# kepengxu/RealCamNet

Hardware: AMD Instinct MI355X
Metric: megapixels/sec RAW->sRGB at 4K (higher is better)
Workload: dtype bf16; 1 GPU; cfg3: 3840x2160 Bayer mosaic -> unshuffle+pad16 -> LiteISPNet_GFM_LSC_GMA -> sRGB 3840x2160, 8 frames/GPU, bf16 storage / fp32 accumulate; frames_per_gpu=8, global_frames=8, parallelism=frame-shard x1, collective=none

## Files before the change

### include/realcam_hip.h

```cpp
#ifndef REALCAM_HIP_H
#define REALCAM_HIP_H

#include <stddef.h>
#include <stdint.h>

#ifdef __cplusplus
extern "C" {
#endif

#define RC_ABI_VERSION 15

typedef enum rc_status {
    RC_OK = 0,
    RC_ERR_INVALID = -1,
    RC_ERR_HIP = -2,
    RC_ERR_UNSUPPORTED = -3
} rc_status;

typedef enum rc_dtype { RC_F32 = 0, RC_BF16 = 1, RC_U16 = 2 ,
                        RC_F16 = 3  } rc_dtype;

typedef enum rc_act { RC_ACT_NONE = 0, RC_ACT_RELU = 1, RC_ACT_LEAKY = 2 ,
                      RC_ACT_GELU = 3 ,
                      RC_ACT_RELU_POST = 4  } rc_act;

typedef enum rc_out_mode {
    RC_OUT_NHWC = 0,
    RC_OUT_PIXEL_SHUFFLE2 = 1,
    RC_OUT_NCHW = 2,
    RC_OUT_PIXEL_SHUFFLE2_NCHW = 3,
    RC_OUT_NHWC_DWT = 4
} rc_out_mode;

int rc_abi_version(void);
const char* rc_last_error(void);
const char* rc_build_info(void);
int rc_device_arch(char* buf, size_t buflen);

int rc_bayer_unshuffle(const void* d_mosaic, int in_dtype, void* d_packed, int out_dtype,
                       int batch, int h, int w, int hp, int wp, void* stream);

int rc_raw_ingest(const void* d_mosaic, int in_dtype, void* d_packed, void* d_cond, int out_dtype, int batch, int h, int w,
                  int hp, int wp, int cond_h, int cond_w, float black_level, float white_level, void* stream);

typedef enum rc_raw_storage {
    RC_RAW_F32 = 0, RC_RAW_BF16 = 1, RC_RAW_U16 = 2, RC_RAW_F16 = 3,
    RC_RAW_U8 = 4,
    RC_RAW_MIPI10 = 5,
    RC_RAW_MIPI12 = 6
} rc_raw_storage;

typedef enum rc_cfa { RC_CFA_RGGB = 0, RC_CFA_BGGR = 1, RC_CFA_GRBG = 2, RC_CFA_GBRG = 3 } rc_cfa;

typedef struct rc_raw_format {
    int storage;
    int cfa;
    int line_bytes;
    int width;
    float black[4];
    float white;
    int reserved[4];
} rc_raw_format;
size_t rc_raw_format_size(void);

int rc_raw_ingest_fmt(const void* d_src, const rc_raw_format* fmt, void* d_packed, void* d_cond, int out_dtype, int batch, int h, int w,
                      int hp, int wp, int cond_h, int cond_w, void* stream);

int rc_rgb_encode(const void* d_src, int src_dtype, void* d_dst, int out_bits, int batch, int H, int W, int h, int w, void* stream);

typedef enum rc_yuv_layout {
    RC_YUV_NV12 = 0,
    RC_YUV_P010 = 1,
    RC_YUV_I420 = 2
} rc_yuv_layout;
typedef enum rc_yuv_matrix { RC_MATRIX_BT601 = 0, RC_MATRIX_BT709 = 1, RC_MATRIX_BT2020 = 2  } rc_yuv_matrix;
typedef enum rc_yuv_range { RC_RANGE_LIMITED = 0, RC_RANGE_FULL = 1 } rc_yuv_range;
typedef enum rc_chroma_siting { RC_SITING_LEFT = 0 ,
                                RC_SITING_CENTER = 1  } rc_chroma_siting;

#define RC_YUV_KR_KB {{0.299, 0.114}, {0.2126, 0.0722}, {0.2627, 0.0593}}

typedef struct rc_out_format {
    int layout;
    int matrix;
    int range;
    int siting;
    int pitch;
    int rows;
    int chroma_offset[2];
    int reserved[4];
} rc_out_format;
size_t rc_out_format_size(void);

size_t rc_yuv_frame_bytes(const rc_out_format* fmt, int h, int w);

int rc_yuv_encode(const void* d_src, int src_dtype, const rc_out_format* fmt, void* d_dst, int batch, int H, int W, int h, int w, void* stream);

typedef enum rc_resize_filter {
    RC_FILTER_AREA = 0,
    RC_FILTER_BILINEAR = 1
} rc_resize_filter;
#define RC_RESIZE_MAX_TAPS 20
#define RC_RESIZE_MAX_RATIO 8

int rc_resize_taps(int filter, int n, int off, int m, int* first, float* weights, int* taps);

int rc_resize(const void* d_src, int src_dtype, void* d_dst, int dst_dtype, int batch, int H, int W, int h, int w, const int* d_first_y,
              const float* d_wy, int taps_y, const int* d_first_x, const float* d_wx, int taps_x, void* stream);

#define RC_LUT3D_MIN_SIZE 2
#define RC_LUT3D_MAX_SIZE 65

int rc_lut3d(const void* d_src, int src_dtype, void* d_dst, int dst_dtype, const float* d_lut, int n, int batch, int H, int W, int h, int w, void* stream);

typedef enum rc_warp_interp {
    RC_WARP_BILINEAR = 0,
    RC_WARP_BICUBIC = 1
} rc_warp_interp;
typedef enum rc_warp_border {
    RC_WARP_CLAMP = 0,
    RC_WARP_CONSTANT = 1
} rc_warp_border;
#define RC_WARP_MIN_CELL_LOG2 3
#define RC_WARP_MAX_CELL_LOG2 6
#define RC_WARP_MAX_DIM 8388608

int rc_warp(const void* d_src, int src_dtype, void* d_dst, int dst_dtype, const float* d_mesh, int mesh_batch, int cell_log2, int interp,
            int border, float fill_r, float fill_g, float fill_b, int batch, int H, int W, int h, int w, int oh, int ow, void* stream);

int rc_nchw_to_nhwc(const void* d_src, int src_dtype, void* d_dst, int dst_dtype,
                    int batch, int c, int h, int w, int hp, int wp, void* stream);
int rc_nhwc_to_nchw(const void* d_src, int src_dtype, void* d_dst, int dst_dtype,
                    int batch, int c, int H, int W, int h, int w, void* stream);

typedef struct rc_conv_desc {
    int32_t batch, height, width;
    int32_t cin, cout, ksize;
    int32_t dtype;
    const void* in0;
    const void* in1;
    const float* in_gate;
    void* in_store;
    const void* wpacked;
    const float* bias;
    const float* film_scale;
    const float* film_shift;
    int32_t act;
    float act_slope;
    const void* mul_plus1;
    const void* residual;
    void* out;
    int32_t out_mode;
    int32_t out_dtype;
    int32_t out_h, out_w;
    float* chan_sums;
    int32_t src_h, src_w;
    const float* out_scale;
    int32_t chan_sums_slots;
    int32_t cout_tile;
    int32_t algo;
} rc_conv_desc;

size_t rc_conv_packed_bytes(int cin, int cout, int ksize, int dtype, int out_mode);
int rc_conv_pack_weights(const float* w_oihw_host, int cin, int cout, int ksize, int dtype,
                         int out_mode, void* dst_host);
int rc_conv_packed_cout(int cin, int cout, int ksize, int dtype, int out_mode);
int rc_conv_pack_bias(const float* bias_host, int cin, int cout, int ksize, int dtype, int out_mode,
                      float* dst_host);
size_t rc_conv_packed_bytes_ct(int cin, int cout, int ksize, int dtype, int out_mode, int cout_tile);
int rc_conv_packed_cout_ct(int cin, int cout, int ksize, int dtype, int out_mode, int cout_tile);
int rc_conv_pack_weights_ct(const float* w_oihw_host, int cin, int cout, int ksize, int dtype, int out_mode, int cout_tile, void* dst_host);
int rc_conv_pack_bias_ct(const float* bias_host, int cin, int cout, int ksize, int dtype, int out_mode, int cout_tile, float* dst_host);
size_t rc_wino_packed_bytes(int cin, int cout, int dtype);
int rc_wino_pack_weights(const float* w_oihw_host, int cin, int cout, int dtype, void* dst_host);
int rc_conv_sum_tiles(int height, int width);
int rc_conv_sum_slots(const rc_conv_desc* d);
int rc_conv2d(const rc_conv_desc* desc, void* stream);
size_t rc_conv_desc_size(void);

int rc_tail_fold_weights(const float* w1_host, const float* b1_host, const float* w2_host, const float* b2_host, int c, int o,
                         float* wc_host, float* bc_host);
int rc_tail_ring_gather(const void* d_x, void* d_rows, void* d_cols, int dtype, int batch, int H, int W, int c, void* stream);
int rc_tail_ring_scatter(const void* d_rows_out, const void* d_cols_out, void* d_out, int dtype, int batch, int c_out, int H, int W,
                         int out_h, int out_w, void* stream);

typedef struct rc_conv_pair_desc {
    int32_t batch, height, width, channels;
    int32_t dtype;
    const void* in0;
    const void* in1;
    const float* in_gate;
    void* in_store;
    const void* w1; const float* b1;
    const float* film_scale;
    const float* film_shift;
    int32_t act1;
    float act1_slope;
    const void* w2; const float* b2;
    const void* residual;
    void* out;
    float* chan_sums;
} rc_conv_pair_desc;
int rc_conv_pair(const rc_conv_pair_desc* desc, void* stream);
int rc_conv_pair_sum_slots(int height, int width);
size_t rc_conv_pair_desc_size(void);

int rc_pointwise_chain48(const void* d_x, int cin0, const void* d_w0packed, const float* d_b0, const void* const* d_wpacked,
                         const float* const* d_bias, int n_mid, float slope, void* d_out, int dtype, long long pixels,
                         void* stream);

size_t rc_lsc_packed_bytes(int c, int n_mid, int has_head);
int rc_lsc_pack(const float* w0, const float* b0, int cin0, const float* const* wmid, const float* const* bmid, int n_mid,
                const float* whead, const float* bhead, int raw_c, int c, void* dst);
int rc_lsc_chain(const void* d_x, int cin0, const void* d_blob, int c, int n_mid, float slope, const void* d_raw, int raw_c,
                 void* d_out, int batch, int H, int W, void* stream);

int rc_ca_gate(float* d_sums, int batch, int n_tiles, int c, int cr, float inv_hw,
               const float* d_w0, const float* d_b0, const float* d_w1, const float* d_b1,
               float* d_gate, void* stream);

size_t rc_ca_gate_ahead_scratch_floats(int batch, int c);
int rc_ca_gate_ahead(float* d_sums, int batch, int n_tiles, int c, int cr, const void* d_t, int dtype, int H, int W,
                     const float* d_w2t, const float* d_b2, const float* d_w0, const float* d_b0, const float* d_w1, const float* d_b1,
                     float* d_scratch, float* d_gate, void* stream);

int rc_channel_sums_slots(int n_pix);
int rc_channel_sums(const void* d_x, int dtype, int batch, int n_pix, int c, float* d_sums, void* stream);

int rc_gate_residual(const void* d_r, const float* d_gate, const void* d_x, void* d_y, int dtype,
                     int batch, int n_pix, int c, void* stream);

int rc_film_apply(const void* d_x, const float* d_scale, const float* d_shift, void* d_y, int dtype, int batch, int n_pix, int c, void* stream);

int rc_sigmoid_gate_add(const void* d_a, const void* d_b, const void* d_identity, void* d_y, int dtype, long long n_elems,
                        void* stream);

int rc_subsample2(const void* d_src, void* d_dst, int dtype, int batch, int H, int W, int c, void* stream);
int rc_upsample_bilinear2(const void* d_src, void* d_dst, int dtype, int batch, int H, int W, int c, void* stream);
int rc_sft_apply(const void* d_x, const void* d_scale, const void* d_shift, const void* d_identity, void* d_y, int dtype,
                 long long n_elems, void* stream);
int rc_space_to_depth2(const void* d_src, void* d_dst, int dtype, int batch, int H, int W, int c, void* stream);
int rc_pixel_shuffle2(const void* d_src, void* d_dst, int dtype, int batch, int H, int W, int c_out, void* stream);
int rc_pixel_shuffle2_nchw(const void* d_src, void* d_dst, int dtype, int batch, int H, int W, int c_out, void* stream);
int rc_square(const void* d_x, void* d_y, int dtype, long long n_elems, void* stream);
int rc_gdn_apply(const void* d_x, const void* d_norm, const void* d_identity, void* d_y, int dtype, int inverse, long long n_elems,
                 void* stream);

int rc_entropy_bottleneck(const void* d_z, const float* d_params, const float* d_medians, void* d_z_hat, float* d_likelihood,
                          int dtype, long long n_pix, int channels, float likelihood_bound, void* stream);
int rc_gaussian_conditional(const void* d_y, const void* d_scale, const void* d_mu, void* d_y_hat, float* d_likelihood, int dtype,
                            long long n_elems, float scale_bound, float likelihood_bound, void* stream);
// ... 139 lines not shown
```

### realcamnet_amd/LiteISP.py

```python
from __future__ import annotations

from typing import Optional, Sequence

import torch
import torch.nn as nn

from . import networks as N
from . import ops
from .groupmix import GMA_Block, SUPPORTED_DTYPES
from ._lib import RC_OUT_NCHW, RC_OUT_PIXEL_SHUFFLE2
from .out_format import OutFormat
from .resize import Output


def color_block(in_filters, out_filters, normalization=False):
    layers = [N.Conv2d(in_filters, out_filters, 1, stride=1, padding=0),
              nn.AvgPool2d(3, stride=2, padding=1, count_include_pad=True),
              nn.LeakyReLU(0.2)]
    if normalization:
        layers.append(nn.InstanceNorm2d(out_filters, affine=True))
    return layers


def pad_to_multiple_of_16(x):
# ... 256 lines not shown
def _emit(y, bits, outs):
    if outs is None:
        return _encode(y, bits)
    res = []
    for o in outs:
        t = y if o.warp is None else ops.warp(y, o.warp)
        t = t if o.resize is None else ops.resize(t, o.resize)
        if o.look is not None:
            t = ops.lut3d(t, o.look)
        res.append(_encode(t, _out_bits(o.format)))
    return res


class _DwtUNet(nn.Module):

    output_dtype: Optional[torch.dtype] = None
    cond_from_raw = False

    def _build(self, ch_1, ch_2, ch_3, cond_c=None, lsc=False, nf=None, n_blocks=4):
        if cond_c is not None:
            self.classifier = Color_Condition_GFM(in_channels=4, out_c=cond_c)
        self.head = N.seq(N.conv(4, ch_1, mode='C'))
        if lsc:
            self.lsc = Lens_Shading_Correction(in_channels=2, out_c=ch_1, nf=ch_1)

        def gfm(i, c):
            if cond_c is not None:
                setattr(self, f"encoder_modulation{i}", N.seq(Res_GFM(in_nc=c, chan=c, cond_c=cond_c, out_nc=c, nf=nf[i - 1])))

        gfm(1, ch_1)
        self.down1 = N.seq(N.conv(ch_1, ch_1, mode='C'), N.RCAGroup(in_channels=ch_1, out_channels=ch_1, nb=n_blocks),
                           N.conv(ch_1, ch_1, mode='C'), N.DWTForward(ch_1))
        gfm(2, ch_1 * 4)
        self.down2 = N.seq(N.conv(ch_1 * 4, ch_1, mode='C'), N.RCAGroup(in_channels=ch_1, out_channels=ch_1, nb=n_blocks),
                           N.DWTForward(ch_1))
        gfm(3, ch_1 * 4)
        self.down3 = N.seq(N.conv(ch_1 * 4, ch_2, mode='C'), N.RCAGroup(in_channels=ch_2, out_channels=ch_2, nb=n_blocks),
                           N.DWTForward(ch_2))
        gfm(4, ch_2 * 4)
        self.middle = N.seq(N.conv(ch_2 * 4, ch_3, mode='C'), N.RCAGroup(in_channels=ch_3, out_channels=ch_3, nb=n_blocks),
                            N.RCAGroup(in_channels=ch_3, out_channels=ch_3, nb=n_blocks), N.conv(ch_3, ch_2 * 4, mode='C'))
        self.up3 = N.seq(N.DWTInverse(ch_2 * 4), N.RCAGroup(in_channels=ch_2, out_channels=ch_2, nb=n_blocks),
                         N.conv(ch_2, ch_1 * 4, mode='C'))
        self.up2 = N.seq(N.DWTInverse(ch_1 * 4), N.RCAGroup(in_channels=ch_1, out_channels=ch_1, nb=n_blocks),
                         N.conv(ch_1, ch_1 * 4, mode='C'))
        self.up1 = N.seq(N.DWTInverse(ch_1 * 4), N.RCAGroup(in_channels=ch_1, out_channels=ch_1, nb=n_blocks),
                         N.conv(ch_1, ch_1, mode='C'))
        self.tail = N.seq(N.conv(ch_1, ch_1 * 4, mode='C'), nn.PixelShuffle(upscale_factor=2), N.conv(ch_1, 3, mode='C'))

    def _act_dtype(self) -> torch.dtype:
        return self.head.weight.dtype

    def _refine_d1(self, d1):
        return d1

    def _check(self, raw):
        if self.training:
            raise RuntimeError("realcamnet_amd is an inference path: call .eval() first")
        if raw.dim() != 4 or raw.shape[1] != 4:
            raise ValueError(f"raw must be (B,4,H,W), got {tuple(raw.shape)}")
        if raw.shape[2] % 8 or raw.shape[3] % 8:
            raise ValueError(f"packed RAW H,W must be multiples of 8 (3 Haar levels), got {raw.shape[2]}x{raw.shape[3]}; "
                             "use forward_mosaic()/pad_to_multiple_of_16 for other sizes")

    def _front(self, a, cond, coord_nhwc):
        def head():
            if not hasattr(self, "lsc"):
                return self.head._nhwc(a)
            h = ops.lsc_chain(self.lsc, coord_nhwc, self.head, a)
            return h if h is not None else self.head._nhwc(a, mul_plus1=self.lsc._nhwc(coord_nhwc))

        if not hasattr(self, "classifier"):
            return head(), None
        cond = ops._req(cond, "cond")
        vec, h = ops.fork_join(lambda: self.classifier._vec(cond), head, [cond])
        return h, vec

    def _trunk(self, h, vec, crop_hw=None):
        mod = (lambda i, t: getattr(self, f"encoder_modulation{i}")._nhwc((t, vec))[0]) if vec is not None else (lambda i, t: t)
        h = mod(1, h)
        d1 = self._refine_d1(self.down1._nhwc(h))
        d2 = self.down2._nhwc(mod(2, d1))
        d3 = self.down3._nhwc(mod(3, d2))
        m = self.middle._nhwc(mod(4, d3), residual=d3)
        u3 = self.up3._nhwc(m, residual=d2)
        u2 = self.up2._nhwc(u3, residual=d1)
        u1 = self.up1._nhwc(u2, residual=h)
        if ops.tail_fold_ok(u1, self.tail[0], self.tail[2]):
            return ops.tail_fold(u1, self.tail[0], self.tail[2], crop_hw=crop_hw, out_dtype=self.output_dtype)
        t = self.tail[0]._nhwc(u1, out_mode=RC_OUT_PIXEL_SHUFFLE2)
        return self.tail[2]._nhwc(t, out_mode=RC_OUT_NCHW, crop_hw=crop_hw, out_dtype=self.output_dtype)

    def forward(self, x: Sequence[torch.Tensor]):
        raw = x if isinstance(x, torch.Tensor) else x[0]
        self._check(raw)
        dt = self._act_dtype()
        coord_nhwc = None
        if hasattr(self, "lsc"):
            coord = x[2]
            if coord.shape[0] != raw.shape[0] or coord.shape[1] != 2 or coord.shape[2:] != raw.shape[2:]:
                raise ValueError(f"coord must be (B,2,H,W) matching raw, got {tuple(coord.shape)}")
            coord_nhwc = ops.to_nhwc(coord, dtype=dt)
        cond = (raw if self.cond_from_raw else x[1]) if hasattr(self, "classifier") else None
        h, vec = self._front(ops.to_nhwc(raw, dtype=dt), cond, coord_nhwc)
        return self._trunk(h, vec)

    def forward_mosaic(self, mosaic, cond=None, coord=None, pad_to: int = 16, black_level: float = 0.0, white_level: float = 1.0,
                       cond_hw=(256, 256), raw_format=None, out_format=None, outputs=None):
        if self.training:
            raise RuntimeError("realcamnet_amd is an inference path: call .eval() first")
        bits = _out_bits(out_format)
        dt = self._act_dtype()
        mh, mw = _mosaic_hw(mosaic, raw_format)
        outs = _plan_outputs(outputs, out_format, (mh, mw))
        a, cond = _ingest(self, mosaic, cond, dt, pad_to, black_level, white_level, cond_hw, raw_format)
        b, hp, wp, _ = a.shape
        co = None
        if hasattr(self, "lsc"):
            if coord is None or coord.shape[-2:] != (mh // 2, mw // 2):
                raise ValueError("coord must be at packed resolution (h, w)")
            co = ops.to_nhwc(coord, dtype=dt, pad_hw=(hp, wp))
        if hasattr(self, "classifier") and self.cond_from_raw:
            cond = ops.to_nchw(a)
        h, vec = self._front(a, cond, co)
        return _emit(self._trunk(h, vec, crop_hw=(mh, mw)), bits, outs)


class LiteISPNet(_DwtUNet):

    def __init__(self):
        super().__init__()
        self._build(64, 128, 128)


class LiteISPNet_GFM_LSC(_DwtUNet):

    def __init__(self):
        super().__init__()
        self._build(48, 128, 128, cond_c=32, lsc=True, nf=(48, 48, 48, 128))


class LiteISPNet_LSC(_DwtUNet):

    def __init__(self):
        super().__init__()
        self._build(48, 128, 128, lsc=True)


class LiteISPNet_GFM(_DwtUNet):

    def __init__(self):
        super().__init__()
        self._build(64, 128, 128, cond_c=64, nf=(64, 64, 64, 128))


class LiteISPNet_GFMresize(_DwtUNet):
    cond_from_raw = True

    def __init__(self):
        super().__init__()
        self._build(64, 128, 128, cond_c=32, nf=(128, 256, 256, 512))


class _StridedUNet(nn.Module):

    output_dtype: Optional[torch.dtype] = None

    cond_from_raw = False
    coord_in_intro = False
    skips = True
# ... 270 lines not shown
```

### realcamnet_amd/_lib.py

```python
from __future__ import annotations

import ctypes as C
import os
import re
from pathlib import Path

PKG = Path(__file__).resolve().parent
LIB_PATH = Path(os.environ["RC_HIP_LIB"]) if os.environ.get("RC_HIP_LIB") else PKG / "librealcam_hip.so"
HEADER = PKG.parent / "include" / "realcam_hip.h"

RC_F32, RC_BF16, RC_U16, RC_F16 = 0, 1, 2, 3
RC_ACT_NONE, RC_ACT_RELU, RC_ACT_LEAKY, RC_ACT_GELU, RC_ACT_RELU_POST = 0, 1, 2, 3, 4
RC_OUT_NHWC, RC_OUT_PIXEL_SHUFFLE2, RC_OUT_NCHW, RC_OUT_PIXEL_SHUFFLE2_NCHW, RC_OUT_NHWC_DWT = 0, 1, 2, 3, 4
ABI_VERSION = 15
RC_RAW_F32, RC_RAW_BF16, RC_RAW_U16, RC_RAW_F16, RC_RAW_U8, RC_RAW_MIPI10, RC_RAW_MIPI12 = 0, 1, 2, 3, 4, 5, 6
RC_CFA_RGGB, RC_CFA_BGGR, RC_CFA_GRBG, RC_CFA_GBRG = 0, 1, 2, 3
RC_YUV_NV12, RC_YUV_P010, RC_YUV_I420 = 0, 1, 2
RC_MATRIX_BT601, RC_MATRIX_BT709, RC_MATRIX_BT2020 = 0, 1, 2
RC_RANGE_LIMITED, RC_RANGE_FULL = 0, 1
RC_SITING_LEFT, RC_SITING_CENTER = 0, 1
RC_FILTER_AREA, RC_FILTER_BILINEAR = 0, 1
RC_RESIZE_MAX_TAPS, RC_RESIZE_MAX_RATIO = 20, 8
RC_LUT3D_MIN_SIZE, RC_LUT3D_MAX_SIZE = 2, 65
RC_WARP_BILINEAR, RC_WARP_BICUBIC = 0, 1
RC_WARP_CLAMP, RC_WARP_CONSTANT = 0, 1
RC_WARP_MIN_CELL_LOG2, RC_WARP_MAX_CELL_LOG2, RC_WARP_MAX_DIM = 3, 6, 1 << 23


class ConvDesc(C.Structure):
    _fields_ = [
        ("batch", C.c_int32), ("height", C.c_int32), ("width", C.c_int32),
        ("cin", C.c_int32), ("cout", C.c_int32), ("ksize", C.c_int32),
        ("dtype", C.c_int32),
        ("in0", C.c_void_p), ("in1", C.c_void_p), ("in_gate", C.c_void_p), ("in_store", C.c_void_p),
        ("wpacked", C.c_void_p), ("bias", C.c_void_p),
        ("film_scale", C.c_void_p), ("film_shift", C.c_void_p),
        ("act", C.c_int32), ("act_slope", C.c_float),
        ("mul_plus1", C.c_void_p), ("residual", C.c_void_p),
        ("out", C.c_void_p), ("out_mode", C.c_int32), ("out_dtype", C.c_int32),
        ("out_h", C.c_int32), ("out_w", C.c_int32),
        ("chan_sums", C.c_void_p),
        ("src_h", C.c_int32), ("src_w", C.c_int32),
        ("out_scale", C.c_void_p),
        ("chan_sums_slots", C.c_int32), ("cout_tile", C.c_int32),
        ("algo", C.c_int32),
    ]


class ConvPairDesc(C.Structure):
    _fields_ = [
        ("batch", C.c_int32), ("height", C.c_int32), ("width", C.c_int32), ("channels", C.c_int32),
        ("dtype", C.c_int32),
        ("in0", C.c_void_p), ("in1", C.c_void_p), ("in_gate", C.c_void_p), ("in_store", C.c_void_p),
        ("w1", C.c_void_p), ("b1", C.c_void_p),
        ("film_scale", C.c_void_p), ("film_shift", C.c_void_p),
        ("act1", C.c_int32), ("act1_slope", C.c_float),
        ("w2", C.c_void_p), ("b2", C.c_void_p),
        ("residual", C.c_void_p), ("out", C.c_void_p), ("chan_sums", C.c_void_p),
    ]


class RawFormatDesc(C.Structure):
    _fields_ = [
        ("storage", C.c_int32), ("cfa", C.c_int32), ("line_bytes", C.c_int32), ("width", C.c_int32),
        ("black", C.c_float * 4), ("white", C.c_float), ("reserved", C.c_int32 * 4),
    ]


class OutFormatDesc(C.Structure):
    _fields_ = [
        ("layout", C.c_int32), ("matrix", C.c_int32), ("range", C.c_int32), ("siting", C.c_int32),
        ("pitch", C.c_int32), ("rows", C.c_int32), ("chroma_offset", C.c_int32 * 2), ("reserved", C.c_int32 * 4),
    ]


def declared_symbols() -> list[str]:
    text = HEADER.read_text()
    text = re.sub(r"/\*.*?\*/", "", text, flags=re.S)
    return sorted(set(re.findall(r"\b(rc_[a-z0-9_]+)\s*\(", text)))


_P, _I, _F, _SZ = C.c_void_p, C.c_int, C.c_float, C.c_size_t
_SIGS = {
    "rc_abi_version": (C.c_int, []),
    "rc_last_error": (C.c_char_p, []),
    "rc_build_info": (C.c_char_p, []),
    "rc_device_arch": (C.c_int, [C.c_char_p, _SZ]),
    "rc_bayer_unshuffle": (C.c_int, [_P, _I, _P, _I, _I, _I, _I, _I, _I, _P]),
    "rc_raw_ingest": (C.c_int, [_P, _I, _P, _P, _I, _I, _I, _I, _I, _I, _I, _I, _F, _F, _P]),
    "rc_raw_format_size": (_SZ, []),
    "rc_raw_ingest_fmt": (C.c_int, [_P, C.POINTER(RawFormatDesc), _P, _P, _I, _I, _I, _I, _I, _I, _I, _I, _P]),
    "rc_rgb_encode": (C.c_int, [_P, _I, _P, _I, _I, _I, _I, _I, _I, _P]),
    "rc_out_format_size": (_SZ, []),
    "rc_yuv_frame_bytes": (_SZ, [C.POINTER(OutFormatDesc), _I, _I]),
    "rc_yuv_encode": (C.c_int, [_P, _I, C.POINTER(OutFormatDesc), _P, _I, _I, _I, _I, _I, _P]),
    "rc_resize_taps": (C.c_int, [_I, _I, _I, _I, _P, _P, C.POINTER(C.c_int)]),
    "rc_resize": (C.c_int, [_P, _I, _P, _I, _I, _I, _I, _I, _I, _P, _P, _I, _P, _P, _I, _P]),
    "rc_lut3d": (C.c_int, [_P, _I, _P, _I, _P, _I, _I, _I, _I, _I, _I, _P]),
    "rc_warp": (C.c_int, [_P, _I, _P, _I, _P, _I, _I, _I, _I, _F, _F, _F, _I, _I, _I, _I, _I, _I, _I, _P]),
    "rc_nchw_to_nhwc": (C.c_int, [_P, _I, _P, _I, _I, _I, _I, _I, _I, _I, _P]),
    "rc_nhwc_to_nchw": (C.c_int, [_P, _I, _P, _I, _I, _I, _I, _I, _I, _I, _P]),
    "rc_conv_packed_bytes": (_SZ, [_I, _I, _I, _I, _I]),
    "rc_conv_pack_weights": (C.c_int, [_P, _I, _I, _I, _I, _I, _P]),
    "rc_conv_packed_cout": (C.c_int, [_I, _I, _I, _I, _I]),
    "rc_conv_pack_bias": (C.c_int, [_P, _I, _I, _I, _I, _I, _P]),
    "rc_conv_packed_bytes_ct": (_SZ, [_I, _I, _I, _I, _I, _I]),
    "rc_wino_packed_bytes": (_SZ, [_I, _I, _I]),
    "rc_wino_pack_weights": (C.c_int, [_P, _I, _I, _I, _P]),
    "rc_conv_packed_cout_ct": (C.c_int, [_I, _I, _I, _I, _I, _I]),
    "rc_conv_pack_weights_ct": (C.c_int, [_P, _I, _I, _I, _I, _I, _I, _P]),
    "rc_conv_pack_bias_ct": (C.c_int, [_P, _I, _I, _I, _I, _I, _I, _P]),
    "rc_conv_sum_tiles": (C.c_int, [_I, _I]),
    "rc_conv_sum_slots": (C.c_int, [_P]),
    "rc_conv2d": (C.c_int, [C.POINTER(ConvDesc), _P]),
    "rc_conv_desc_size": (_SZ, []),
    "rc_tail_fold_weights": (C.c_int, [_P, _P, _P, _P, _I, _I, _P, _P]),
    "rc_tail_ring_gather": (C.c_int, [_P, _P, _P, _I, _I, _I, _I, _I, _P]),
    "rc_tail_ring_scatter": (C.c_int, [_P, _P, _P, _I, _I, _I, _I, _I, _I, _I, _P]),
    "rc_debug_stream_create_masked": (C.c_int, [_I, C.POINTER(C.c_void_p)]),
    "rc_debug_hbm_probe": (C.c_int, [_P, _P, C.c_size_t, _I, _I, _I, _I, _I, C.POINTER(C.c_double)]),
    "rc_debug_mfma_peak": (C.c_int, [_I, _I, C.POINTER(C.c_double), C.POINTER(C.c_double)]),
    "rc_debug_mfma_peak32": (C.c_int, [_I, _I, C.POINTER(C.c_double), C.POINTER(C.c_double)]),
    "rc_debug_poison_lds": (C.c_int, [C.c_uint, _P]),
    "rc_pointwise_chain48": (C.c_int, [_P, _I, _P, _P, C.POINTER(C.c_void_p), C.POINTER(C.c_void_p), _I, _F, _P, _I, C.c_longlong, _P]),
    "rc_lsc_packed_bytes": (C.c_size_t, [_I, _I, _I]),
    "rc_lsc_pack": (C.c_int, [_P, _P, _I, C.POINTER(C.c_void_p), C.POINTER(C.c_void_p), _I, _P, _P, _I, _I, _P]),
    "rc_lsc_chain": (C.c_int, [_P, _I, _P, _I, _I, _F, _P, _I, _P, _I, _I, _I, _P]),
    "rc_film_apply": (C.c_int, [_P, _P, _P, _P, _I, _I, _I, _I, _P]),
    "rc_sigmoid_gate_add": (C.c_int, [_P, _P, _P, _P, _I, C.c_longlong, _P]),
    "rc_subsample2": (C.c_int, [_P, _P, _I, _I, _I, _I, _I, _P]),
    "rc_entropy_bottleneck": (C.c_int, [_P, _P, _P, _P, _P, _I, C.c_longlong, _I, C.c_float, _P]),
    "rc_gaussian_conditional": (C.c_int, [_P, _P, _P, _P, _P, _I, C.c_longlong, C.c_float, C.c_float, _P]),
    "rc_tanh_half_add": (C.c_int, [_P, _P, _P, _I, C.c_longlong, _P]),
    "rc_upsample_bilinear2": (C.c_int, [_P, _P, _I, _I, _I, _I, _I, _P]),
    "rc_sft_apply": (C.c_int, [_P, _P, _P, _P, _P, _I, C.c_longlong, _P]),
    "rc_space_to_depth2": (C.c_int, [_P, _P, _I, _I, _I, _I, _I, _P]),
    "rc_pixel_shuffle2": (C.c_int, [_P, _P, _I, _I, _I, _I, _I, _P]),
    "rc_pixel_shuffle2_nchw": (C.c_int, [_P, _P, _I, _I, _I, _I, _I, _P]),
    "rc_square": (C.c_int, [_P, _P, _I, C.c_longlong, _P]),
    "rc_gdn_apply": (C.c_int, [_P, _P, _P, _P, _I, _I, C.c_longlong, _P]),
    "rc_channel_copy": (C.c_int, [_P, _I, _I, _P, _I, _I, _I, C.c_longlong, _I, _P]),
    "rc_channel_concat": (C.c_int, [C.POINTER(C.c_void_p), C.POINTER(C.c_int), _I, _P, C.c_longlong, _I, _P]),
    "rc_window_attention": (C.c_int, [_P, _P, _P, _I, _I, _I, _I, _I, _I, _I, _I, _P]),
    "rc_window_attention_planar8": (C.c_int, [_P, _P, _P, _I, _I, _I, _I, _I, _I, _I, _I, _P]),
    "rc_window_attention_planar8_ok": (C.c_int, [_I, _I, _I, _I, _I, _I]),
    "rc_conv_pair": (C.c_int, [C.POINTER(ConvPairDesc), _P]),
    "rc_conv_pair_sum_slots": (C.c_int, [_I, _I]),
    "rc_conv_pair_desc_size": (_SZ, []),
    "rc_ca_gate": (C.c_int, [_P, _I, _I, _I, _I, _F, _P, _P, _P, _P, _P, _P]),
    "rc_ca_gate_ahead_scratch_floats": (_SZ, [_I, _I]),
    "rc_ca_gate_ahead": (C.c_int, [_P, _I, _I, _I, _I, _P, _I, _I, _I, _P, _P, _P, _P, _P, _P, _P, _P, _P]),
    "rc_gate_residual": (C.c_int, [_P, _P, _P, _P, _I, _I, _I, _I, _P]),
    "rc_channel_sums_slots": (C.c_int, [_I]),
    "rc_channel_sums": (C.c_int, [_P, _I, _I, _I, _I, _P, _P]),
    "rc_dwt_forward": (C.c_int, [_P, _P, _P, _I, _I, _I, _I, _I, _I, _P]),
    "rc_dwt_inverse": (C.c_int, [_P, _P, _P, _I, _I, _I, _I, _I, _I, _P]),
    "rc_color_block": (C.c_int, [_P, _I, _P, _I, _I, _I, _I, _I, _P, _P, _P, _P, _P, _P, _P]),
    "rc_instance_stats": (C.c_int, [_P, _P, _P, _I, _I, _I, _F, _P]),
    "rc_instance_norm": (C.c_int, [_P, _P, _P, _P, _P, _P, _I, _I, _I, _P]),
    "rc_color_head": (C.c_int, [_P, _P, _I, _I, _I, _I, _P, _P, _P]),
    "rc_gfm_vector": (C.c_int, [_P, _I, _I, _I, _I, _P, _P, _P, _P, _P, _P]),
    "rc_dwconv2d": (C.c_int, [_P, _I, _I, _P, _I, _I, _I, _I, _I, _I, _I, _I, _P, _I, _P, _I, _I, _I, _I, _I, _P, _P]),
    "rc_layernorm": (C.c_int, [_P, _P, _I, C.c_longlong, _I, _P, _P, _F, _P]),
    "rc_gma_pointwise": (C.c_int, [_P, _P, _P, _I, _I, _I, _I, _P, _P, _I, C.c_longlong, _I, _P, _P, _P, _P, _P, _P, _P]),
    "rc_chain_packed_bytes": (_SZ, [_I, _I]),
    "rc_chain_packed_rows": (C.c_int, [_I]),
    "rc_chain_pack_weights": (C.c_int, [_P, _I, _I, _P]),
    "rc_chain_pack_bias": (C.c_int, [_P, _I, _P]),
    "rc_gma_ln_qkv": (C.c_int, [_P, _P, C.c_longlong, _P, _P, _P, _P, _F, _P]),
    "rc_gma_tail": (C.c_int, [_P, _P, _P, _P, _P, _P, _I, _I, _P, _P, _P, _P, _F, _P, _P, _P, _P, _P, _P, _P, _I, _P, _P]),
    "rc_gma_aggregate": (C.c_int, [_P, _P, _P, _I, _I, _I, _P, _P, _P, _P, _P, _P, _P, _P, _P, _P, _P, _P]),
    "rc_chain_pack_weights_natural": (C.c_int, [_P, _I, _I, _P]),
    "rc_gma_toeplitz_bytes": (_SZ, []),
    "rc_gma_toeplitz_pack": (C.c_int, [_P, _P, _P, _P, _P]),
    "rc_dw_toeplitz_pack": (C.c_int, [_P, _I, _I, _P]),
    "rc_gma_in_cpe": (C.c_int, [_P, _P, _P, _P, _P, _P, _I, _I, _I, _P]),
    "rc_gma_qkv_aggregate": (C.c_int, [_P, _P, _P, _P, _P, _F, _P, _P, _I, _I, _I, _P, _P, _P, _P, _P, _P, _P, _P, _P]),
    "rc_cat_linear": (C.c_int, [_P, _P, _P, _P, _P, C.c_longlong, _I, _P, _P, _P]),
    "rc_gdn_chain": (C.c_int, [_P, _P, _P, C.c_longlong, _I, _P, _P, _I, _P]),
    "rc_ln_linear": (C.c_int, [_P, _P, C.c_longlong, _I, _I, _P, _P, _P, _P, _F, _P]),
    "rc_ln_linear_planar8": (C.c_int, [_P, _P, C.c_longlong, _I, _I, _P, _P, _P, _P, _F, _P]),
    "rc_ln_mlp": (C.c_int, [_P, _P, C.c_longlong, _I, _P, _P, _P, _P, _P, _P, _F, _P]),
    "rc_gma_kv_mfma_blocks": (C.c_int, [_I]),
    "rc_gma_kv_mfma_scratch_bytes": (C.c_size_t, [_I, _I]),
    "rc_gma_kv_mfma": (C.c_int, [_P, _I, _I, _F, _P, _P, _P, _P]),
    "rc_gma_crpe": (C.c_int, [_P, _P, _I, _I, _I, _P, _P, _P, _P, _P, _P]),
    "rc_gma_kv_blocks": (C.c_int, [_I]),
    "rc_gma_kv_scratch_bytes": (_SZ, [_I, _I, _I, _I]),
# ... 74 lines not shown
```

### realcamnet_amd/csrc/conv.hip

```cpp
#include <mutex>
#include <vector>

#include "conv32_kernel.hpp"

namespace rc {

struct ConvPlan {
    int ck = 0, nt = 0, unit = 0, upt = 0, nu = 0, steps = 0;
    int n_chunks = 0, n_ct = 0, cout_packed = 0;
    int m32 = 0;
};

static int g_persist_on = 1;
extern int g_dw3_seg16;
extern int g_dec_lds;
extern int g_pw_grid_cap;
static int g_pss = 0;
static int g_poison = 0;
static int g_thin = 2;
static int g_auto = 1;
static int g_sums_compact = 1;
static int g_conv32 = 0;

static bool make_plan(int cin, int cout, int ksize, int dtype, int out_mode, ConvPlan* p, int cout_tile = 0) {
    if (cin < 1 || cout < 1 || (ksize != 1 && ksize != 3 && ksize != 2 && ksize != 5)) return false;
    if (dtype != RC_F32 && dtype != RC_BF16 && dtype != RC_F16) return false;
    const bool h16 = dtype != RC_F32;
    if (ksize == 5 && (cout > 16 || out_mode == RC_OUT_PIXEL_SHUFFLE2 || (h16 ? (cin % 48 != 0 && cin % 32 != 0) : cin % 16 != 0))) return false;
    if (out_mode == RC_OUT_PIXEL_SHUFFLE2_NCHW && cout % 4 != 0) return false;
    if (ksize == 2 && (dtype != RC_BF16 || cin % 16 != 0 || out_mode != RC_OUT_NHWC || (cin % 48 == 0 && cin % 64 != 0))) return false;
    p->unit = dtype == RC_F32 ? 4 : 8;
    if (ksize == 5) p->ck = h16 ? (cin % 48 == 0 ? 48 : 32) : 16;
    else if (h16) {
        if (cin <= 8) p->ck = 8;
        else if (ksize == 1 && cin % 80 == 0 && cin % 64 != 0) p->ck = 80;
        else if (ksize >= 2 && cin % 64 == 0 && cin > 64) p->ck = 32;
        else if (cin % 64 == 0) p->ck = 64;
        else if (cin % 48 == 0) p->ck = 48;
        else if (ksize == 3 && cin == 32) p->ck = 32;
        else if (ksize == 3 && cin % 32 == 0 && cin > 64) p->ck = 32;
        else p->ck = 16;
    } else {
        p->ck = cin <= 4 ? 4 : 16;
    }
    if (out_mode == RC_OUT_PIXEL_SHUFFLE2) {
        if (cout % 4 != 0) return false;
        const int cps = cout / 4;
        if (cps % 64 == 0 && !(cps % 48 == 0 && h16 && cin == 48)) p->nt = 4;
        else if (cps % 48 == 0) p->nt = 3;
        else if (cps % 64 == 0) p->nt = 4;
        else if (cps % 16 == 0) p->nt = 1;
        else return false;
    } else if (cout % 48 == 0 && h16 && cin == 48) p->nt = 3;
    else if (h16 && ksize == 3 && cin == 32 && cout == 32) p->nt = 2;
    else if (ksize == 1 && cout % 80 == 0) p->nt = 5;
    else if (cout % 64 == 0) p->nt = 4;
    else if (cout % 48 == 0) p->nt = 3;
    else if (h16 && ksize == 3 && p->ck == 32 && cout % 32 == 0) p->nt = 2;
    else p->nt = 1;
    if (cout_tile != 0) {
        if (cout_tile < 16 || cout_tile > 80 || cout_tile % 16 != 0 || ksize == 5 || ksize == 2 || out_mode == RC_OUT_PIXEL_SHUFFLE2 || out_mode == RC_OUT_PIXEL_SHUFFLE2_NCHW) return false;
        p->nt = cout_tile / 16;
    }
    p->m32 = 0;
    if (cout_tile == 0 && dtype == RC_BF16 && ksize == 3 && g_conv32 != 0 && cout <= kPersistMaxCout && out_mode != RC_OUT_NCHW && out_mode != RC_OUT_PIXEL_SHUFFLE2_NCHW) {
        const int cw = out_mode == RC_OUT_PIXEL_SHUFFLE2 ? cout / 4 : cout;
        const bool all = g_conv32 != 4;
        if (all && p->ck == 32 && cin % 32 == 0 && (out_mode == RC_OUT_PIXEL_SHUFFLE2 ? cw % 32 == 0 : cw % 64 == 0)) { p->m32 = 1; p->nt = 2; p->ck = (g_conv32 == 1 && out_mode == RC_OUT_NHWC) ? 16 : 32; }
        else if (cin == 48 && (out_mode == RC_OUT_PIXEL_SHUFFLE2 ? (all && cw % 48 == 0) : cw % 96 == 0)) { p->m32 = 1; p->nt = 3; p->ck = 48; }
    }
    if (p->m32) {
        p->upt = p->ck / p->unit;
        p->nu = 9 * p->upt;
        p->steps = 9 * (p->ck / 16);
        p->n_chunks = cin / p->ck;
        p->n_ct = cout / (32 * p->nt);
        p->cout_packed = cout;
        return true;
    }
    p->upt = p->ck / p->unit;
    p->nu = ksize * ksize * p->upt;
    p->steps = unit_map_steps(p->upt, ksize * ksize);
    p->n_chunks = ceil_div(cin, p->ck);
    p->n_ct = ceil_div(cout, 16 * p->nt);
    p->cout_packed = p->n_ct * 16 * p->nt;
    return true;
}

static int packed_to_cout(const ConvPlan& p, int cout, int out_mode, int j) {
    if (p.m32) return c32_packed_to_cout(p.nt, out_mode, j);
    if (out_mode == RC_OUT_PIXEL_SHUFFLE2) {
        const int tile = 16 * p.nt;
        const int ct = j / tile, within = j % tile;
        const int cb = ct >> 2, sub = ct & 3;
        return 4 * (cb * tile + within) + sub;
    }
    return j < cout ? j : -1;
}

int wino_conv(const rc_conv_desc* d, hipStream_t stream);
int wino_sum_slots(int H, int W, int cout);
void wino_set_nnt(int v);
int wino_get_nnt();
bool wino_supported(const rc_conv_desc* d, std::string* why);

static int g_dbg_flags = 0;
static int g_pair_impl = 0;
static long long* g_dbg_ptr = nullptr;
static std::mutex g_prof_mu;
static bool g_prof_on = false;
struct ProfRec { hipEvent_t e0, e1; double flops, bytes; int cin, cout, ksize; };
static std::vector<ProfRec> g_prof;

long long* conv_dbg_ptr() { return g_dbg_ptr; }
int conv_pair_impl() { return g_pair_impl; }

void conv_prof_begin(double flops, hipStream_t stream, void** token, double bytes, int cin, int cout, int ksize) {
    *token = nullptr;
    { std::lock_guard<std::mutex> lk(g_prof_mu); if (!g_prof_on) return; }
    ProfRec* rec = new ProfRec{};
    rec->flops = flops; rec->bytes = bytes; rec->cin = cin; rec->cout = cout; rec->ksize = ksize;
    if (hipEventCreate(&rec->e0) != hipSuccess || hipEventCreate(&rec->e1) != hipSuccess) { delete rec; return; }
    (void)hipEventRecord(rec->e0, stream);
    *token = rec;
}
void conv_prof_end(void* token, hipStream_t stream) {
    if (!token) return;
    ProfRec* rec = static_cast<ProfRec*>(token);
    (void)hipEventRecord(rec->e1, stream);
    std::lock_guard<std::mutex> lk(g_prof_mu);
    g_prof.push_back(*rec);
    delete rec;
}

}

using namespace rc;

extern "C" {

size_t rc_conv_packed_bytes_ct(int cin, int cout, int ksize, int dtype, int out_mode, int cout_tile) {
    ConvPlan p;
    if (!make_plan(cin, cout, ksize, dtype, out_mode, &p, cout_tile)) { set_error("rc_conv_packed_bytes: bad shape"); return 0; }
    return (size_t)p.n_ct * p.n_chunks * p.steps * p.nt * 1024;
}
size_t rc_conv_packed_bytes(int cin, int cout, int ksize, int dtype, int out_mode) { return rc_conv_packed_bytes_ct(cin, cout, ksize, dtype, out_mode, 0); }

int rc_conv_packed_cout_ct(int cin, int cout, int ksize, int dtype, int out_mode, int cout_tile) {
    ConvPlan p;
    if (!make_plan(cin, cout, ksize, dtype, out_mode, &p, cout_tile)) return fail(RC_ERR_INVALID, "rc_conv_packed_cout: bad shape");
    return p.cout_packed;
}
int rc_conv_packed_cout(int cin, int cout, int ksize, int dtype, int out_mode) { return rc_conv_packed_cout_ct(cin, cout, ksize, dtype, out_mode, 0); }

int rc_conv_pack_weights(const float* w, int cin, int cout, int ksize, int dtype, int out_mode, void* dst) {
    return rc_conv_pack_weights_ct(w, cin, cout, ksize, dtype, out_mode, 0, dst);
}
int rc_conv_pack_bias(const float* bias, int cin, int cout, int ksize, int dtype, int out_mode, float* dst) {
    return rc_conv_pack_bias_ct(bias, cin, cout, ksize, dtype, out_mode, 0, dst);
}

int rc_conv_pack_weights_ct(const float* w, int cin, int cout, int ksize, int dtype, int out_mode, int cout_tile, void* dst) {
    ConvPlan p;
    RC_REQUIRE(w && dst, "rc_conv_pack_weights: null pointer");
    RC_REQUIRE(make_plan(cin, cout, ksize, dtype, out_mode, &p, cout_tile), "rc_conv_pack_weights: bad shape");
    const int kk = ksize * ksize;
    char* out = static_cast<char*>(dst);
    if (p.m32) {
        const int spt = p.ck / 16;
        for (int ct = 0; ct < p.n_ct; ++ct)
            for (int chunk = 0; chunk < p.n_chunks; ++chunk)
                for (int s = 0; s < p.steps; ++s)
                    for (int t = 0; t < p.nt; ++t)
                        for (int lane = 0; lane < 64; ++lane) {
                            const int m = lane & 31, kg = lane >> 5;
                            const int c = 16 * ((m >> 2) & 1) + (m & 3) + 4 * (m >> 3);
                            const int co = packed_to_cout(p, cout, out_mode, ct * 32 * p.nt + 32 * t + c);
                            const int tap = s / spt, ci0 = chunk * p.ck + (2 * (s % spt) + kg) * 8;
                            for (int e = 0; e < 8; ++e) {
                                *reinterpret_cast<uint16_t*>(out) = host_f32_to_bf16(w[((size_t)co * cin + ci0 + e) * kk + tap]);
                                out += 2;
                            }
                        }
        return RC_OK;
    }
    for (int ct = 0; ct < p.n_ct; ++ct)
        for (int chunk = 0; chunk < p.n_chunks; ++chunk)
            for (int s = 0; s < p.steps; ++s)
                for (int nt = 0; nt < p.nt; ++nt)
                    for (int lane = 0; lane < 64; ++lane) {
                        const int m = lane & 15, qk = lane >> 4;
                        int tap = 0, cu = 0;
                        const bool live = unit_map(p.upt, kk, s, qk, tap, cu);
                        const int j = ct * 16 * p.nt + (m >> 2) * (4 * p.nt) + nt * 4 + (m & 3);
                        const int co = packed_to_cout(p, cout, out_mode, j);
                        for (int e = 0; e < p.unit; ++e) {
                            float val = 0.f;
                            if (live && co >= 0 && co < cout) {
                                const int ci = chunk * p.ck + cu * p.unit + e;
                                if (ci < cin) val = w[((size_t)co * cin + ci) * kk + tap];
                            }
                            if (dtype == RC_F32) {
                                *reinterpret_cast<float*>(out) = val; out += 4;
                            } else {
                                *reinterpret_cast<uint16_t*>(out) = host_f32_to_h16(val, dtype); out += 2;
                            }
                        }
                    }
    return RC_OK;
}

int rc_conv_pack_bias_ct(const float* bias, int cin, int cout, int ksize, int dtype, int out_mode, int cout_tile, float* dst) {
    ConvPlan p;
    RC_REQUIRE(dst, "rc_conv_pack_bias: null pointer");
    RC_REQUIRE(make_plan(cin, cout, ksize, dtype, out_mode, &p, cout_tile), "rc_conv_pack_bias: bad shape");
    for (int j = 0; j < p.cout_packed; ++j) {
        const int co = packed_to_cout(p, cout, out_mode, j);
        dst[j] = (bias && co >= 0 && co < cout) ? bias[co] : 0.f;
    }
    return RC_OK;
}

size_t rc_conv_desc_size(void) { return sizeof(rc_conv_desc); }

int rc_tail_fold_weights(const float* w1, const float* b1, const float* w2, const float* b2, int c, int o, float* wc, float* bc) {
    RC_REQUIRE(w1 && w2 && wc && bc && c >= 1 && o >= 1, "rc_tail_fold_weights: bad arguments");
    std::vector<double> acc((size_t)4 * o * c * 25, 0.0), bacc((size_t)4 * o, 0.0);
    for (int oo = 0; oo < o; ++oo)
        for (int i = 0; i < 2; ++i)
            for (int j = 0; j < 2; ++j) {
                const int row = oo * 4 + 2 * i + j;
                bacc[row] = b2 ? (double)b2[oo] : 0.0;
                for (int dy = 0; dy < 3; ++dy)
                    for (int dx = 0; dx < 3; ++dx) {
                        const int a = i + dy - 1, b = j + dx - 1;
                        const int fy = a < 0 ? -1 : a >> 1, ii = a & 1, fx = b < 0 ? -1 : b >> 1, jj = b & 1;
                        for (int cc = 0; cc < c; ++cc) {
                            const int m = 4 * cc + 2 * ii + jj;
                            const double v2 = w2[(((size_t)oo * c + cc) * 3 + dy) * 3 + dx];
                            if (b1) bacc[row] += v2 * (double)b1[m];
                            for (int k = 0; k < c; ++k)
                                for (int ey = 0; ey < 3; ++ey)
                                    for (int ex = 0; ex < 3; ++ex)
                                        acc[(((size_t)row * c + k) * 5 + (fy + ey + 1)) * 5 + (fx + ex + 1)] += v2 * (double)w1[(((size_t)m * c + k) * 3 + ey) * 3 + ex];
                        }
                    }
            }
    for (size_t n = 0; n < acc.size(); ++n) wc[n] = (float)acc[n];
    for (size_t n = 0; n < bacc.size(); ++n) bc[n] = (float)bacc[n];
    return RC_OK;
}

int rc_conv_sum_tiles(int height, int width) { return 4 * ceil_div(height, kTH) * ceil_div(width, kTW); }

int rc_debug_set(const char* key, int value) {
    RC_REQUIRE(key != nullptr, "rc_debug_set: null key");
    if (std::string(key) == "persist") { g_persist_on = value < 0 ? 0 : (value > 3 ? 3 : value); return RC_OK; }
    if (std::string(key) == "conv_flags") { g_dbg_flags = value; return RC_OK; }
    if (std::string(key) == "pair_impl") { g_pair_impl = value < 0 || value > 2 ? 0 : value; return RC_OK; }
    if (std::string(key) == "dec_lds") { g_dec_lds = value != 0; return RC_OK; }
    if (std::string(key) == "dw3_seg16") { g_dw3_seg16 = value != 0; return RC_OK; }
    if (std::string(key) == "pss") { g_pss = value != 0; return RC_OK; }
    if (std::string(key) == "sums_compact") { g_sums_compact = value != 0; return RC_OK; }
    if (std::string(key) == "persist_auto") { g_auto = value < 0 ? 0 : (value > 2 ? 2 : value); return RC_OK; }
    if (std::string(key) == "thin") { g_thin = value < 0 ? 0 : (value > 2 ? 2 : value); return RC_OK; }
    if (std::string(key) == "lds_poison") { g_poison = value != 0; return RC_OK; }
    if (std::string(key) == "conv32") { g_conv32 = value < 0 ? 0 : (value > 4 ? 4 : value); return RC_OK; }
    if (std::string(key) == "wino_nnt") { wino_set_nnt(value); return RC_OK; }
    if (std::string(key) == "pw_grid_cap") { g_pw_grid_cap = value <= 0 || value > (1 << 22) ? (1 << 22) : value; return RC_OK; }
    return fail(RC_ERR_INVALID, std::string("rc_debug_set: unknown key ") + key);
}

int rc_debug_get(const char* key) {
    if (key == nullptr) return -1;
    if (std::string(key) == "persist") return g_persist_on;
    if (std::string(key) == "conv32") return g_conv32;
    if (std::string(key) == "conv_flags") return g_dbg_flags;
    if (std::string(key) == "pss") return g_pss;
    if (std::string(key) == "sums_compact") return g_sums_compact;
    if (std::string(key) == "persist_auto") return g_auto;
    if (std::string(key) == "thin") return g_thin;
    if (std::string(key) == "lds_poison") return g_poison;
    if (std::string(key) == "wino_nnt") return wino_get_nnt();
    if (std::string(key) == "pw_grid_cap") return g_pw_grid_cap;
    return -1;
}

int rc_debug_set_ptr(const char* key, void* p) {
    RC_REQUIRE(key != nullptr, "rc_debug_set_ptr: null key");
    if (std::string(key) == "conv_phase_timing") { g_dbg_ptr = static_cast<long long*>(p); return RC_OK; }
    return fail(RC_ERR_INVALID, std::string("rc_debug_set_ptr: unknown key ") + key);
}

int rc_prof_enable(int on) {
    std::lock_guard<std::mutex> lk(g_prof_mu);
    for (auto& r : g_prof) { (void)hipEventDestroy(r.e0); (void)hipEventDestroy(r.e1); }
    g_prof.clear();
    g_prof_on = on != 0;
    return RC_OK;
}

int rc_prof_collect(int64_t* n_launches, double* total_ms, double* total_flops) {
    std::lock_guard<std::mutex> lk(g_prof_mu);
    double ms = 0.0, fl = 0.0;
    for (auto& r : g_prof) {
        RC_HIP_CHECK(hipEventSynchronize(r.e1));
        float t = 0.f;
        RC_HIP_CHECK(hipEventElapsedTime(&t, r.e0, r.e1));
        ms += t; fl += r.flops;
    }
    if (n_launches) *n_launches = (int64_t)g_prof.size();
    if (total_ms) *total_ms = ms;
    if (total_flops) *total_flops = fl;
    return RC_OK;
}

int rc_prof_collect_rows(rc_prof_row* rows, int max_rows, int* n_rows) {
    RC_REQUIRE(rows != nullptr && n_rows != nullptr && max_rows >= 1, "rc_prof_collect_rows: bad arguments");
    std::lock_guard<std::mutex> lk(g_prof_mu);
    int n = 0;
    for (auto& r : g_prof) {
        RC_HIP_CHECK(hipEventSynchronize(r.e1));
        float t = 0.f;
        RC_HIP_CHECK(hipEventElapsedTime(&t, r.e0, r.e1));
        int i = 0;
        while (i < n && !(rows[i].cin == r.cin && rows[i].cout == r.cout && rows[i].ksize == r.ksize)) ++i;
        if (i == n) {
            if (n == max_rows) continue;
            rows[n] = rc_prof_row{r.cin, r.cout, r.ksize, 0, 0.0, 0.0, 0.0};
            ++n;
        }
        rows[i].launches += 1; rows[i].ms += t; rows[i].flops += r.flops; rows[i].bytes += r.bytes;
    }
    *n_rows = n;
    return RC_OK;
}

static int conv_build_args(const rc_conv_desc* d, ConvPlan& p, ConvArgs& a, size_t& es_out) {
    RC_REQUIRE(d != nullptr, "rc_conv2d: null desc");
    const bool dwt = d->out_mode == RC_OUT_NHWC_DWT;
    RC_REQUIRE(make_plan(d->cin, d->cout, d->ksize, d->dtype, dwt ? (int)RC_OUT_NHWC : d->out_mode, &p, d->cout_tile), "rc_conv2d: unsupported cin/cout/ksize/dtype/cout_tile");
    RC_REQUIRE(d->batch >= 1 && d->height >= 1 && d->width >= 1, "rc_conv2d: empty tensor");
    RC_REQUIRE(d->batch <= 65535, "rc_conv2d: batch > 65535");
    RC_REQUIRE(d->in0 && d->wpacked && d->out, "rc_conv2d: null in0/wpacked/out");
    RC_REQUIRE(d->out_mode >= RC_OUT_NHWC && d->out_mode <= RC_OUT_NHWC_DWT, "rc_conv2d: bad out_mode");
    if (dwt) {
        RC_REQUIRE(d->height % 2 == 0 && d->width % 2 == 0, "rc_conv2d: RC_OUT_NHWC_DWT needs even height and width");
        RC_REQUIRE(d->out_dtype == d->dtype && reinterpret_cast<uintptr_t>(d->out) % 16 == 0, "rc_conv2d: RC_OUT_NHWC_DWT: out_dtype must equal dtype, out 16-byte aligned");
        RC_REQUIRE(!d->mul_plus1 && !d->film_scale && !d->out_scale && !d->chan_sums && !d->in_gate && !d->in1 && !d->in_store && !d->src_h && !d->src_w && !d->cout_tile,
                   "rc_conv2d: RC_OUT_NHWC_DWT excludes mul_plus1 / film / out_scale / chan_sums / gated input / src_h / cout_tile");
        if (d->dtype == RC_F32 || d->ksize != 3 || p.m32 || !(d->act == RC_ACT_NONE || ((d->act == RC_ACT_RELU || d->act == RC_ACT_LEAKY) && !d->residual)))
            return fail(RC_ERR_UNSUPPORTED, "rc_conv2d: RC_OUT_NHWC_DWT is a bf16 / fp16 3x3 form with act NONE / RELU / LEAKY, or act NONE + residual");
    }
    RC_REQUIRE(d->act >= RC_ACT_NONE && d->act <= RC_ACT_RELU_POST, "rc_conv2d: bad act");
    RC_REQUIRE(d->act != RC_ACT_RELU_POST || (d->residual != nullptr && d->mul_plus1 == nullptr && d->film_scale == nullptr && d->chan_sums == nullptr),
               "rc_conv2d: RC_ACT_RELU_POST is relu(conv + residual): needs residual, excludes film / mul_plus1 / chan_sums");
    if (d->in_gate) RC_REQUIRE(d->in1 != nullptr, "rc_conv2d: in_gate needs in1 (the skip tensor)");
    RC_REQUIRE((d->film_scale == nullptr) == (d->film_shift == nullptr), "rc_conv2d: film_scale/film_shift must come together");
    const bool full_tiles = d->cout == p.cout_packed;
    if (d->mul_plus1 || d->residual)
        RC_REQUIRE((full_tiles || d->cout % 4 == 0) && (d->out_mode == RC_OUT_NHWC || (dwt && !d->mul_plus1)), "rc_conv2d: mul_plus1/residual need cout % 4 == 0 and RC_OUT_NHWC (residual: or RC_OUT_NHWC_DWT)");
    if (d->chan_sums) RC_REQUIRE(d->out_mode == RC_OUT_NHWC, "rc_conv2d: chan_sums needs RC_OUT_NHWC");
    if (d->out_scale) {
        RC_REQUIRE(d->out_mode == RC_OUT_NHWC && !p.m32, "rc_conv2d: out_scale needs RC_OUT_NHWC and a layer outside the 32x32x16 forms");
        RC_REQUIRE(reinterpret_cast<uintptr_t>(d->out_scale) % 4 == 0, "rc_conv2d: out_scale must be 4-byte aligned");
    }
    const size_t es = dtype_size(d->dtype);
    const int planar16 = d->dtype == RC_F16 ? RC_F16 : RC_BF16;
    if (dwt) {
    } else if (d->out_mode == RC_OUT_NHWC) {
        RC_REQUIRE(d->out_dtype == d->dtype, "rc_conv2d: out_dtype must equal dtype for RC_OUT_NHWC");
        RC_REQUIRE(!full_tiles || (d->cout * es) % 8 == 0, "rc_conv2d: cout*elem_size must be a multiple of 8 bytes for RC_OUT_NHWC");
        RC_REQUIRE(reinterpret_cast<uintptr_t>(d->out) % 16 == 0, "rc_conv2d: out must be 16-byte aligned");
        if (p.nt == 4 && d->dtype != RC_F32) RC_REQUIRE(d->cout % 8 == 0, "rc_conv2d: cout % 8");
    } else if (d->out_mode == RC_OUT_PIXEL_SHUFFLE2) {
        RC_REQUIRE(d->out_dtype == d->dtype, "rc_conv2d: out_dtype must equal dtype for RC_OUT_PIXEL_SHUFFLE2");
        RC_REQUIRE(full_tiles && ((d->cout / 4) * es) % 8 == 0, "rc_conv2d: pixel-shuffle store needs (cout/4)*elem_size % 8 == 0");
        RC_REQUIRE(!d->film_scale, "rc_conv2d: film not supported with pixel-shuffle store");
        RC_REQUIRE(reinterpret_cast<uintptr_t>(d->out) % 16 == 0, "rc_conv2d: out must be 16-byte aligned");
    } else if (d->out_mode == RC_OUT_PIXEL_SHUFFLE2_NCHW) {
        RC_REQUIRE(d->out_h >= 1 && d->out_h <= 2 * d->height && d->out_w >= 1 && d->out_w <= 2 * d->width, "rc_conv2d: bad pixel-shuffle NCHW crop");
        RC_REQUIRE(d->out_dtype == RC_F32 || d->out_dtype == planar16, "rc_conv2d: bad out_dtype");
        RC_REQUIRE(!d->chan_sums, "rc_conv2d: chan_sums needs RC_OUT_NHWC");
        RC_REQUIRE((double)d->out_h * d->out_w * (d->cout / 4) * 4.0 < 2147483647.0, "rc_conv2d: one output image must be < 2 GiB");
    } else {
        RC_REQUIRE(d->out_h >= 1 && d->out_h <= d->height && d->out_w >= 1 && d->out_w <= d->width, "rc_conv2d: bad NCHW crop");
        RC_REQUIRE(d->out_dtype == RC_F32 || d->out_dtype == planar16, "rc_conv2d: bad out_dtype");
    }
    {
        const double lim = 2147483647.0;
        RC_REQUIRE((double)d->height * d->width * d->cin * es < lim, "rc_conv2d: one input image must be < 2 GiB");
        RC_REQUIRE((double)d->height * d->width * d->cout * 4.0 < lim, "rc_conv2d: one output image must be < 2 GiB");
    }
    const bool fold = d->src_h != 0 || d->src_w != 0;
    if (fold) {
        RC_REQUIRE(d->ksize == 2 && d->cin % 4 == 0 && (d->cin / 4) % p.ck == 0, "rc_conv2d: src_h/src_w need ksize 2 and cin / 4 a whole number of Cin chunks");
        RC_REQUIRE(d->src_h >= 1 && d->src_w >= 1 && d->height == (d->src_h + 1) / 2 && d->width == (d->src_w + 1) / 2,
                   "rc_conv2d: height/width must be ceil(src_h / 2), ceil(src_w / 2)");
        RC_REQUIRE(d->in_gate == nullptr && d->in1 == nullptr && d->in_store == nullptr, "rc_conv2d: src_h/src_w exclude the gated input");
        RC_REQUIRE(reinterpret_cast<uintptr_t>(d->in0) % 16 == 0, "rc_conv2d: src_h/src_w need a 16-byte aligned in0 (the scalar staging path does not gather)");
        RC_REQUIRE((double)d->src_h * d->src_w * (d->cin / 4) * es < 2147483647.0, "rc_conv2d: one input image must be < 2 GiB");
    }
    if (d->residual) RC_REQUIRE(reinterpret_cast<uintptr_t>(d->residual) % 16 == 0, "rc_conv2d: residual must be 16-byte aligned");
    if (d->mul_plus1) RC_REQUIRE(reinterpret_cast<uintptr_t>(d->mul_plus1) % 16 == 0, "rc_conv2d: mul_plus1 must be 16-byte aligned");

    a = ConvArgs{};
    a.batch = d->batch; a.H = d->height; a.W = d->width; a.cin = d->cin; a.cout = d->cout;
    a.n_chunks = p.n_chunks; a.n_ct = p.n_ct;
    a.tiles_x = ceil_div(d->width, kTW); a.tiles_y = ceil_div(d->height, kTH);
    if (p.m32) RC_REQUIRE(!d->film_scale || (reinterpret_cast<uintptr_t>(d->film_scale) % 16 == 0 && reinterpret_cast<uintptr_t>(d->film_shift) % 16 == 0),
                          "rc_conv2d: film vectors must be 16-byte aligned");
    auto aligned16 = [](const void* q) { return q == nullptr || reinterpret_cast<uintptr_t>(q) % 16 == 0; };
    a.cin_vec_ok = (d->cin % p.unit == 0) && aligned16(d->in0) && aligned16(d->in1) && aligned16(d->in_store) &&
                   (d->in_gate == nullptr || reinterpret_cast<uintptr_t>(d->in_gate) % 4 == 0);
    a.cin_chunk_ok = d->cin % p.ck == 0;
    a.fold2 = fold ? 1 : 0; a.src_H = d->src_h; a.src_W = d->src_w; a.cfold = d->cin / 4;
    a.in0 = d->in0; a.in1 = d->in1; a.in_gate = d->in_gate; a.in_store = d->in_store;
    a.wpacked = d->wpacked; a.bias = d->bias;
    a.film_scale = d->film_scale; a.film_shift = d->film_shift;
    a.act = d->act; a.act_slope = d->act_slope;
    a.mul_plus1 = d->mul_plus1; a.residual = d->residual; a.out_scale = d->out_scale;
    a.out = d->out; a.out_mode = d->out_mode; a.out_dtype = d->out_dtype; a.out_h = d->out_h; a.out_w = d->out_w;
    a.chan_sums = d->chan_sums; a.cout_packed = p.cout_packed;
    a.sum_slots = d->chan_sums_slots > 0 ? d->chan_sums_slots : 4 * ceil_div(d->height, kTH) * ceil_div(d->width, kTW);
    a.sums_compact = 0; a.query = nullptr; a.sums_compact_ok = g_sums_compact;
    {
        int key = (d->act == RC_ACT_RELU ? 1 : 0) | (d->act == RC_ACT_LEAKY ? 2 : 0) | (d->film_scale ? 4 : 0) |
                  (d->mul_plus1 ? 8 : 0) | (d->residual ? 16 : 0) | (d->chan_sums ? 32 : 0) | (d->out_scale ? 64 : 0);
        bool fast = full_tiles && d->out_mode != RC_OUT_NCHW && d->out_mode != RC_OUT_PIXEL_SHUFFLE2_NCHW && d->act != RC_ACT_GELU && d->act != RC_ACT_RELU_POST;
        if (d->act == RC_ACT_LEAKY) fast = fast && d->act_slope >= 0.f && d->act_slope <= 1.f;
        if (d->film_scale)
            fast = fast && d->cout % 4 == 0 && reinterpret_cast<uintptr_t>(d->film_scale) % 16 == 0 && reinterpret_cast<uintptr_t>(d->film_shift) % 16 == 0;
        if (d->out_scale) fast = fast && d->cout % 4 == 0 && reinterpret_cast<uintptr_t>(d->out_scale) % 16 == 0;
        switch (key) { case 0: case 1: case 2: case 16: case 32: case 8: case 6: case 33: case 34: case 80: break; default: fast = false; }
        a.ep_key = fast ? key : -1;
        a.pss = g_pss && d->out_mode == RC_OUT_PIXEL_SHUFFLE2 && !p.m32 && p.n_chunks == 1 && p.n_ct == 4 && d->cout == 4 * 16 * p.nt &&
                d->dtype == RC_BF16 && d->in_gate == nullptr && fast && (key == 0 || key == 1 || key == 2);
    }
    {
        const int num_cus = device_cu_count();
        a.num_cus = num_cus;
        a.persist_ok = g_persist_on;
        a.auto_impl = g_auto;
        a.thin = g_thin;
        a.dbg = g_dbg_ptr;
        a.dbg_flags = g_dbg_flags;
        a.td = make_tile_decode(a.tiles_x, a.tiles_y, kBandRows);
        a.td_wsm = make_tile_decode(a.tiles_x, (a.H + kWsmTH - 1) / kWsmTH, kBandRows);
        a.div_n_ct = make_magic(a.n_ct);
    }
    es_out = es;
    return RC_OK;
// ... 44 lines not shown
```

### realcamnet_amd/csrc/conv_dispatch.hip

```cpp
#include "conv_kernel.hpp"
namespace rc {
int conv_bf16_k3_ck8(int nt, const ConvArgs& a, hipStream_t s);
int conv_bf16_k3_ck16(int nt, const ConvArgs& a, hipStream_t s);
int conv_bf16_k3_ck32(int nt, const ConvArgs& a, hipStream_t s);
int conv_bf16_k3_ck48(int nt, const ConvArgs& a, hipStream_t s);
int conv_bf16_k3_ck64(int nt, const ConvArgs& a, hipStream_t s);
int conv_bf16_k5_ck48(int nt, const ConvArgs& a, hipStream_t s);
int conv_bf16_k5_ck32(int nt, const ConvArgs& a, hipStream_t s);
int conv_f32_k5_ck16(int nt, const ConvArgs& a, hipStream_t s);
int conv_bf16_k2_ck16(int nt, const ConvArgs& a, hipStream_t s);
int conv_bf16_k2_ck32(int nt, const ConvArgs& a, hipStream_t s);
int conv_bf16_k2_ck64(int nt, const ConvArgs& a, hipStream_t s);
int conv_bf16_k1_ck8(int nt, const ConvArgs& a, hipStream_t s);
int conv_bf16_k1_ck16(int nt, const ConvArgs& a, hipStream_t s);
int conv_bf16_k1_ck48(int nt, const ConvArgs& a, hipStream_t s);
int conv_bf16_k1_ck64(int nt, const ConvArgs& a, hipStream_t s);
int conv_bf16_k1_ck80(int nt, const ConvArgs& a, hipStream_t s);
int conv_f32_k3_ck4(int nt, const ConvArgs& a, hipStream_t s);
int conv_f32_k3_ck16(int nt, const ConvArgs& a, hipStream_t s);
int conv_f32_k1_ck4(int nt, const ConvArgs& a, hipStream_t s);
int conv_f32_k1_ck16(int nt, const ConvArgs& a, hipStream_t s);
int conv_f16_k3_ck8(int nt, const ConvArgs& a, hipStream_t s);
int conv_f16_k3_ck16(int nt, const ConvArgs& a, hipStream_t s);
int conv_f16_k3_ck32(int nt, const ConvArgs& a, hipStream_t s);
int conv_f16_k3_ck48(int nt, const ConvArgs& a, hipStream_t s);
int conv_f16_k3_ck64(int nt, const ConvArgs& a, hipStream_t s);
int conv_f16_k5_ck48(int nt, const ConvArgs& a, hipStream_t s);
int conv_f16_k5_ck32(int nt, const ConvArgs& a, hipStream_t s);
int conv_f16_k1_ck8(int nt, const ConvArgs& a, hipStream_t s);
int conv_f16_k1_ck16(int nt, const ConvArgs& a, hipStream_t s);
int conv_f16_k1_ck48(int nt, const ConvArgs& a, hipStream_t s);
int conv_f16_k1_ck64(int nt, const ConvArgs& a, hipStream_t s);

int dispatch_conv(int dtype, int ksize, int ck, int nt, const ConvArgs& a, hipStream_t s) {
    if (dtype == RC_F16) {
        if (ksize == 3 && ck == 8) return conv_f16_k3_ck8(nt, a, s);
        if (ksize == 3 && ck == 16) return conv_f16_k3_ck16(nt, a, s);
        if (ksize == 3 && ck == 32) return conv_f16_k3_ck32(nt, a, s);
        if (ksize == 3 && ck == 48) return conv_f16_k3_ck48(nt, a, s);
        if (ksize == 3 && ck == 64) return conv_f16_k3_ck64(nt, a, s);
        if (ksize == 5 && ck == 48) return conv_f16_k5_ck48(nt, a, s);
        if (ksize == 5 && ck == 32) return conv_f16_k5_ck32(nt, a, s);
        if (ksize == 1 && ck == 8) return conv_f16_k1_ck8(nt, a, s);
        if (ksize == 1 && ck == 16) return conv_f16_k1_ck16(nt, a, s);
        if (ksize == 1 && ck == 48) return conv_f16_k1_ck48(nt, a, s);
        if (ksize == 1 && ck == 64) return conv_f16_k1_ck64(nt, a, s);
        return fail(RC_ERR_UNSUPPORTED, "conv: no fp16 kernel instantiation for this (ksize, chunk width)");
    }
    const bool bf16 = dtype == RC_BF16;
    if (bf16 && ksize == 3 && ck == 8) return conv_bf16_k3_ck8(nt, a, s);
    if (bf16 && ksize == 3 && ck == 16) return conv_bf16_k3_ck16(nt, a, s);
    if (bf16 && ksize == 3 && ck == 32) return conv_bf16_k3_ck32(nt, a, s);
    if (bf16 && ksize == 3 && ck == 48) return conv_bf16_k3_ck48(nt, a, s);
    if (bf16 && ksize == 3 && ck == 64) return conv_bf16_k3_ck64(nt, a, s);
    if (bf16 && ksize == 5 && ck == 48) return conv_bf16_k5_ck48(nt, a, s);
    if (bf16 && ksize == 5 && ck == 32) return conv_bf16_k5_ck32(nt, a, s);
    if (!bf16 && ksize == 5 && ck == 16) return conv_f32_k5_ck16(nt, a, s);
    if (bf16 && ksize == 2 && ck == 16) return conv_bf16_k2_ck16(nt, a, s);
    if (bf16 && ksize == 2 && ck == 32) return conv_bf16_k2_ck32(nt, a, s);
    if (bf16 && ksize == 2 && ck == 64) return conv_bf16_k2_ck64(nt, a, s);
    if (bf16 && ksize == 1 && ck == 8) return conv_bf16_k1_ck8(nt, a, s);
    if (bf16 && ksize == 1 && ck == 16) return conv_bf16_k1_ck16(nt, a, s);
    if (bf16 && ksize == 1 && ck == 48) return conv_bf16_k1_ck48(nt, a, s);
    if (bf16 && ksize == 1 && ck == 64) return conv_bf16_k1_ck64(nt, a, s);
    if (bf16 && ksize == 1 && ck == 80) return conv_bf16_k1_ck80(nt, a, s);
    if (!bf16 && ksize == 3 && ck == 4) return conv_f32_k3_ck4(nt, a, s);
    if (!bf16 && ksize == 3 && ck == 16) return conv_f32_k3_ck16(nt, a, s);
    if (!bf16 && ksize == 1 && ck == 4) return conv_f32_k1_ck4(nt, a, s);
    if (!bf16 && ksize == 1 && ck == 16) return conv_f32_k1_ck16(nt, a, s);
    return fail(RC_ERR_UNSUPPORTED, "conv: no kernel instantiation for this (dtype, ksize, chunk width)");
}
}
```

### realcamnet_amd/csrc/conv_kernel.hpp

```cpp
#pragma once
#include "common.hpp"

namespace rc {

struct MagicDiv { unsigned m, sh; };
inline MagicDiv make_magic(int d) {
    if (d <= 1) return MagicDiv{0u, 0u};
    int L = 0;
    while ((2 << L) <= d) ++L;
    const unsigned long long m = ((1ull << (31 + L)) + (unsigned long long)d - 1) / (unsigned long long)d;
    return MagicDiv{(unsigned)m, (unsigned)(L - 1)};
}
__device__ __forceinline__ int magic_div(int n, const MagicDiv& d) {
    return d.m ? (int)(__umulhi((unsigned)n, d.m) >> d.sh) : n;
}
struct TileDecode { MagicDiv sp_total, band, last_rows; };
inline TileDecode make_tile_decode(int tiles_x, int tiles_y, int band_rows) {
    return TileDecode{make_magic(tiles_x * tiles_y), make_magic(band_rows * tiles_x), make_magic(tiles_y % band_rows ? tiles_y % band_rows : 1)};
}

struct ConvArgs {
    int batch, H, W, cin, cout;
    int n_chunks, n_ct, tiles_x, tiles_y;
    int cin_vec_ok;
    int cin_chunk_ok;
    const void* in0; const void* in1; const float* in_gate; void* in_store;
    const void* wpacked; const float* bias;
    const float* film_scale; const float* film_shift;
    int act; float act_slope;
    const void* mul_plus1; const void* residual;
    const float* out_scale;
    void* out; int out_mode; int out_dtype; int out_h, out_w;
    float* chan_sums; int cout_packed;
    int sum_slots;
    int sums_compact_ok;
    int sums_compact;
    int* query;
    int num_cus; int persist_ok;
    int ep_key;
    TileDecode td, td_wsm;
    MagicDiv div_n_ct;
    int w_resident;
    int pss;
    int auto_impl;
    int thin;
    int fold2, src_H, src_W, cfold;
    long long* dbg;
    int dbg_flags;
};

constexpr int kTH = 8, kTW = 32, kThreads = 256;

constexpr int pix_stride_bytes(int ck_bytes) {
    int s = (ck_bytes + 15) / 16 * 16;
    while (s % 64 != 32) s += 16;
    return s;
}

__host__ __device__ constexpr int unit_map_steps(int upt, int taps) {
    return upt == 6 ? taps + (taps + 1) / 2 : (taps * upt + 3) / 4;
}
__host__ __device__ constexpr bool unit_map(int upt, int taps, int s, int q, int& tap, int& cu) {
    if (upt == 6) {
        if (s < taps) { tap = s; cu = q; return true; }
        tap = 2 * (s - taps) + (q >> 1); cu = 4 + (q & 1);
        return tap < taps;
    }
    const int u = 4 * s + q;
    tap = u / upt; cu = u % upt;
    return u < taps * upt;
}

template <typename T, int CK_, int NT_, int KS_, int TH_ = kTH>
struct ConvCfg {
    using elem = T;
    static constexpr int CK = CK_, NT = NT_, KS = KS_, TH = TH_;
    static constexpr int UNIT = 16 / (int)sizeof(T);
    static_assert(CK % UNIT == 0, "CK must be a whole number of 16-byte units");
    static constexpr int UPT = CK / UNIT;
    static constexpr int TAPS = KS * KS;
    static constexpr int STEPS = unit_map_steps(UPT, TAPS);
    static constexpr int HALO = KS / 2;
    static constexpr int THH = TH + 2 * HALO, TWH = kTW + 2 * HALO;
    static constexpr int SPIX = pix_stride_bytes(CK * (int)sizeof(T));
    static constexpr int IN_BYTES = THH * TWH * SPIX;
    static constexpr int G_RAW = (80 * 1024 - IN_BYTES) / (NT * 1024);
    static constexpr int G_CAP = G_RAW < 1 ? 1 : (G_RAW > STEPS ? STEPS : G_RAW);
    static constexpr int NSUB = (STEPS + G_CAP - 1) / G_CAP;
    static constexpr int G = (STEPS + NSUB - 1) / NSUB;
    static constexpr int W_BYTES = G * NT * 1024;
    static constexpr int COUT_TILE = 16 * NT;
    static constexpr int LDS_BYTES = IN_BYTES + W_BYTES;
    static constexpr size_t CHUNK_W_BYTES = (size_t)STEPS * NT * 1024;
};

constexpr int kOOB = (int)0x80000000;

typedef unsigned int u32x4_t __attribute__((ext_vector_type(4)));
typedef unsigned int u32x2_t __attribute__((ext_vector_type(2)));

__device__ __forceinline__ __amdgpu_buffer_rsrc_t make_rsrc(const void* p, unsigned bytes) {
    return __builtin_amdgcn_make_buffer_rsrc(const_cast<void*>(p), 0, (int)bytes, 0x00020000);
}
__device__ __forceinline__ uint4 buf_load16(__amdgpu_buffer_rsrc_t r, int voff, int soff) {
    const u32x4_t v = __builtin_amdgcn_raw_buffer_load_b128(r, voff, soff, 0);
    return make_uint4(v.x, v.y, v.z, v.w);
}
__device__ __forceinline__ void buf_store16(__amdgpu_buffer_rsrc_t r, int voff, int soff, const uint4& v) {
    __builtin_amdgcn_raw_buffer_store_b128(u32x4_t{v.x, v.y, v.z, v.w}, r, voff, soff, 0);
}

template <typename T> struct Mma;
template <> struct Mma<bf16_t> {
    __device__ static __forceinline__ void run(const uint4& w, const uint4& x, f32x4& acc) {
        acc = __builtin_amdgcn_mfma_f32_16x16x32_bf16(__builtin_bit_cast(bf16x8, w), __builtin_bit_cast(bf16x8, x), acc, 0, 0, 0);
    }
};
template <> struct Mma<f16_t> {
    __device__ static __forceinline__ void run(const uint4& w, const uint4& x, f32x4& acc) {
        acc = __builtin_amdgcn_mfma_f32_16x16x32_f16(__builtin_bit_cast(f16x8, w), __builtin_bit_cast(f16x8, x), acc, 0, 0, 0);
    }
};
template <> struct Mma<float> {
    __device__ static __forceinline__ void run(const uint4& w, const uint4& x, f32x4& acc) {
        acc = __builtin_amdgcn_mfma_f32_16x16x4f32(__uint_as_float(w.x), __uint_as_float(x.x), acc, 0, 0, 0);
        acc = __builtin_amdgcn_mfma_f32_16x16x4f32(__uint_as_float(w.y), __uint_as_float(x.y), acc, 0, 0, 0);
        acc = __builtin_amdgcn_mfma_f32_16x16x4f32(__uint_as_float(w.z), __uint_as_float(x.z), acc, 0, 0, 0);
        acc = __builtin_amdgcn_mfma_f32_16x16x4f32(__uint_as_float(w.w), __uint_as_float(x.w), acc, 0, 0, 0);
    }
};

__device__ __forceinline__ unsigned pack_bf16x2(float lo, float hi) {
    return Vec16<bf16_t>::rne2(lo, hi);
}
template <typename T> __device__ __forceinline__ unsigned pack16x2(float lo, float hi) {
    return Vec16<T>::rne2(lo, hi);
}

template <typename TT, int NV, bool PK_RELU>
__device__ __forceinline__ void buf_store_row(__amdgpu_buffer_rsrc_t r, int voff, const float* v) {
    if constexpr (sizeof(TT) == 4) {
        static_assert(!PK_RELU, "packed ReLU is a bf16 form");
#pragma unroll
        for (int i = 0; i < NV; i += 4)
            __builtin_amdgcn_raw_buffer_store_b128(u32x4_t{__float_as_uint(v[i]), __float_as_uint(v[i + 1]), __float_as_uint(v[i + 2]), __float_as_uint(v[i + 3])},
                                                   r, voff + 4 * i, 0, 0);
    } else {
        unsigned w[NV / 2];
#pragma unroll
        for (int i = 0; i < NV / 2; ++i) {
            w[i] = pack16x2<TT>(v[2 * i], v[2 * i + 1]);
            if constexpr (PK_RELU) {
                typedef short s16x2 __attribute__((ext_vector_type(2)));
                const s16x2 z = {0, 0};
                w[i] = __builtin_bit_cast(unsigned, __builtin_elementwise_max(__builtin_bit_cast(s16x2, w[i]), z));
            }
        }
        constexpr int NQ = NV / 8;
#pragma unroll
        for (int i = 0; i < NQ; ++i)
            __builtin_amdgcn_raw_buffer_store_b128(u32x4_t{w[4 * i], w[4 * i + 1], w[4 * i + 2], w[4 * i + 3]}, r, voff + 16 * i, 0, 0);
        if constexpr (NV % 8 != 0)
            __builtin_amdgcn_raw_buffer_store_b64(u32x2_t{w[4 * NQ], w[4 * NQ + 1]}, r, voff + 16 * NQ, 0, 0);
    }
}

template <typename TT, int NV>
__device__ __forceinline__ void buf_load_row(__amdgpu_buffer_rsrc_t r, int voff, float* v) {
    if constexpr (sizeof(TT) == 4) {
#pragma unroll
        for (int i = 0; i < NV; i += 4) {
            const u32x4_t t = __builtin_amdgcn_raw_buffer_load_b128(r, voff + 4 * i, 0, 0);
            v[i] = __uint_as_float(t.x); v[i + 1] = __uint_as_float(t.y); v[i + 2] = __uint_as_float(t.z); v[i + 3] = __uint_as_float(t.w);
        }
    } else {
#pragma unroll
        for (int i = 0; i < NV; i += 4) {
            const u32x2_t p = __builtin_amdgcn_raw_buffer_load_b64(r, voff + 2 * i, 0, 0);
            v[i] = lo16<TT>(p.x); v[i + 1] = hi16<TT>(p.x);
            v[i + 2] = lo16<TT>(p.y); v[i + 3] = hi16<TT>(p.y);
        }
    }
// ... 662 lines not shown
                }
            }
            if constexpr ((F & EP_SUMS) != 0) {
#pragma unroll
                for (int e = 0; e < NV; ++e) run[e] += valid ? v[e] : 0.f;
            }
            const int oo = (valid && !(a.dbg_flags & 1)) ? (((gy + p) * a.W + gx) * a.cout + jbase) * ES : kOOB;
            buf_store_row<T, NV, PK_RELU>(r_out, oo, v);
        }
        if constexpr ((F & EP_SUMS) != 0) {
            if (flush) {
                write_chan_sums(a, b, slot, n, jbase, run, false);
#pragma unroll
                for (int e = 0; e < NV; ++e) run[e] = 0.f;
            }
        }
    }

    template <int F>
    __device__ static __forceinline__ void epilogue_dwt(const ConvArgs& a, int b, int y0, int x0, int tid, f32x4 (&acc)[4][NT], char* st,
                                                        const unsigned (&rp)[(F & EP_RES) ? 4 : 1][(F & EP_RES) ? NV / 2 : 1]) {
        static_assert(ES == 2 && NV % 4 == 0 && (F == 0 || F == EP_RELU || F == EP_LEAKY || F == EP_RES), "bf16; plain / ReLU / LeakyReLU / + residual");
        typedef float f32x2 __attribute__((ext_vector_type(2)));
        const int lane = tid & 63, wave = tid >> 6, q = lane >> 4, n = lane & 15;
        constexpr int REC = Cfg::COUT_TILE * 2 + 8, ROW = kTW * REC;
        const float inf = __builtin_inff();
#pragma unroll
        for (int pt = 0; pt < 4; ++pt) {
            float v[NV];
#pragma unroll
            for (int nt = 0; nt < NT; ++nt)
#pragma unroll
                for (int r = 0; r < 4; ++r) v[nt * 4 + r] = acc[pt][nt][r];
            if constexpr ((F & EP_RELU) != 0) {
#pragma unroll
                for (int e = 0; e < NV; ++e) v[e] = __builtin_amdgcn_fmed3f(v[e], 0.f, inf);
            }
            if constexpr ((F & EP_LEAKY) != 0) {
#pragma unroll
                for (int e = 0; e < NV; ++e) v[e] = __builtin_amdgcn_fmed3f(v[e], v[e] * a.act_slope, inf);
            }
            if constexpr ((F & EP_RES) != 0) {
#pragma unroll
                for (int i = 0; i < NV / 2; ++i) {
                    v[2 * i] += lo16<T>(rp[pt][i]);
                    v[2 * i + 1] += hi16<T>(rp[pt][i]);
                }
            }
            char* dst = st + (pt >> 1) * ROW + (16 * (pt & 1) + n) * REC + q * (NV * 2);
#pragma unroll
            for (int i = 0; i < NV / 4; ++i)
                *reinterpret_cast<uint2*>(dst + 8 * i) = make_uint2(pack16x2<T>(v[4 * i], v[4 * i + 1]), pack16x2<T>(v[4 * i + 2], v[4 * i + 3]));
        }
        __builtin_amdgcn_fence(__ATOMIC_RELEASE, "wavefront");
        __builtin_amdgcn_wave_barrier();
        f32x2 in[4][NV / 2];
        const char* src = st + (2 * n) * REC + q * (NV * 2);
#pragma unroll
        for (int t = 0; t < 4; ++t)
#pragma unroll
            for (int i = 0; i < NV / 4; ++i) {
                const uint2 w = *reinterpret_cast<const uint2*>(src + (t >> 1) * ROW + (t & 1) * REC + 8 * i);
                in[t][2 * i] = f32x2{lo16<T>(w.x), hi16<T>(w.x)} * 0.5f;
                in[t][2 * i + 1] = f32x2{lo16<T>(w.y), hi16<T>(w.y)} * 0.5f;
            }
        __builtin_amdgcn_fence(__ATOMIC_RELEASE, "wavefront");
        __builtin_amdgcn_wave_barrier();
        unsigned o[2 * NV];
#pragma unroll
        for (int p = 0; p < NV / 2; ++p) {
            const f32x2 sab = in[0][p] + in[1][p], dab = in[0][p] - in[1][p];
            const f32x2 k0 = (sab + in[2][p]) + in[3][p], k1 = (sab - in[2][p]) - in[3][p];
            const f32x2 k2 = (dab + in[2][p]) - in[3][p], k3 = (dab - in[2][p]) + in[3][p];
            o[4 * p] = pack16x2<T>(k0.x, k1.x); o[4 * p + 1] = pack16x2<T>(k2.x, k3.x);
            o[4 * p + 2] = pack16x2<T>(k0.y, k1.y); o[4 * p + 3] = pack16x2<T>(k2.y, k3.y);
        }
        const int Hh = a.H >> 1, Wh = a.W >> 1, oy = (y0 >> 1) + wave, ox = (x0 >> 1) + n;
        const size_t img_out = (size_t)a.H * a.W * a.cout;
        const __amdgpu_buffer_rsrc_t r_out = make_rsrc(static_cast<T*>(a.out) + (size_t)b * img_out, (unsigned)(img_out * ES));
        const int oo = (oy < Hh && ox < Wh && !(a.dbg_flags & 1)) ? ((oy * Wh + ox) * (4 * a.cout) + 4 * q * NV) * ES : kOOB;
#pragma unroll
        for (int i = 0; i < NV / 2; ++i)
            __builtin_amdgcn_raw_buffer_store_b128(u32x4_t{o[4 * i], o[4 * i + 1], o[4 * i + 2], o[4 * i + 3]}, r_out, oo, 16 * i, 0);
    }

    __device__ static __forceinline__ void epilogue_generic(const ConvArgs& a, int b, int y0, int x0, int sp, int ct, int tid,
                                                            f32x4 (&acc)[4][NT]) {
        const int lane = tid & 63, wave = tid >> 6, q = lane >> 4, n = lane & 15;
        const int jbase = ct * Cfg::COUT_TILE + q * NV;
        float fs[NV], ft[NV];
        const bool film = a.film_scale != nullptr;
        if (film) {
#pragma unroll
            for (int e = 0; e < NV; ++e) {
                const bool in = jbase + e < a.cout;
                fs[e] = in ? a.film_scale[(size_t)b * a.cout + jbase + e] : 0.f;
                ft[e] = in ? a.film_shift[(size_t)b * a.cout + jbase + e] : 0.f;
            }
        }
        const int gy_w = y0 + 2 * wave, gx_l = x0 + n;
        float csum[NV];
#pragma unroll
        for (int e = 0; e < NV; ++e) csum[e] = 0.f;

        const size_t img_out = (size_t)a.H * a.W * a.cout;
        const unsigned img_bytes_out = (unsigned)(img_out * ES);
        __amdgpu_buffer_rsrc_t r_out;
        if (a.out_mode == RC_OUT_NCHW || a.out_mode == RC_OUT_PIXEL_SHUFFLE2_NCHW) {
            const size_t plane = (size_t)a.out_h * a.out_w;
            const int osz = a.out_dtype == RC_F32 ? 4 : 2;
            const int planes = a.out_mode == RC_OUT_NCHW ? a.cout : a.cout >> 2;
            r_out = make_rsrc(static_cast<char*>(a.out) + (size_t)b * planes * plane * osz, (unsigned)(planes * plane * osz));
        } else {
            r_out = make_rsrc(static_cast<T*>(a.out) + (size_t)b * img_out, img_bytes_out);
        }
        const bool full = a.cout == a.cout_packed;

#pragma unroll
        for (int pt = 0; pt < 4; ++pt) {
            const int gy = gy_w + (pt >> 1);
            const int gx = gx_l + (pt & 1) * 16;
            const bool valid = gy < a.H && gx < a.W;
            float v[NV];
#pragma unroll
            for (int nt = 0; nt < NT; ++nt)
#pragma unroll
                for (int r = 0; r < 4; ++r) v[nt * 4 + r] = acc[pt][nt][r];
            if (film) {
#pragma unroll
                for (int e = 0; e < NV; ++e) v[e] = v[e] * fs[e] + ft[e] + v[e];
            }
            if (a.act == RC_ACT_RELU) {
#pragma unroll
                for (int e = 0; e < NV; ++e) v[e] = __builtin_amdgcn_fmed3f(v[e], 0.f, __builtin_inff());
            } else if (a.act == RC_ACT_LEAKY) {
#pragma unroll
                for (int e = 0; e < NV; ++e) v[e] = v[e] > 0.f ? v[e] : v[e] * a.act_slope;
            } else if (a.act == RC_ACT_GELU) {
#pragma unroll
                for (int e = 0; e < NV; ++e) v[e] = gelu_erf_f32(v[e]);
            }
            const int pix_off = valid ? ((gy * a.W + gx) * a.cout + jbase) * ES : kOOB;
            if (a.mul_plus1 != nullptr) {
                float m[NV];
                const __amdgpu_buffer_rsrc_t r_mul = make_rsrc(static_cast<const T*>(a.mul_plus1) + (size_t)b * img_out, img_bytes_out);
                buf_load_row<T, NV>(r_mul, pix_off, m);
#pragma unroll
                for (int e = 0; e < NV; ++e) v[e] = v[e] * (m[e] + 1.f);
            }
            if (a.out_scale != nullptr) {
#pragma unroll
                for (int e = 0; e < NV; ++e) v[e] *= (jbase + e < a.cout) ? a.out_scale[(size_t)b * a.cout + jbase + e] : 0.f;
            }
            if (a.residual != nullptr) {
                float m[NV];
                const __amdgpu_buffer_rsrc_t r_res = make_rsrc(static_cast<const T*>(a.residual) + (size_t)b * img_out, img_bytes_out);
                buf_load_row<T, NV>(r_res, pix_off, m);
#pragma unroll
                for (int e = 0; e < NV; ++e) v[e] += m[e];
                if (a.act == RC_ACT_RELU_POST) {
#pragma unroll
                    for (int e = 0; e < NV; ++e) v[e] = __builtin_amdgcn_fmed3f(v[e], 0.f, __builtin_inff());
                }
            }
            if (a.chan_sums != nullptr) {
#pragma unroll
// ... 60 lines not shown

template <class Cfg, bool GATED, bool FAST>
__global__ __launch_bounds__(kThreads, 2) void conv_mfma_kernel(const ConvArgs a) {
    using D = ConvDev<Cfg>;
    using T = typename Cfg::elem;
    constexpr int NT = Cfg::NT, STEPS = Cfg::STEPS, G = Cfg::G, NSUB = Cfg::NSUB, NV = 4 * NT;

    extern __shared__ __attribute__((aligned(16))) char smem[];
    char* s_w = smem;
    char* s_in = smem + Cfg::W_BYTES;

    const int tid = threadIdx.x, lane = tid & 63, wave = tid >> 6;
    const int q = lane >> 4, n = lane & 15;
    const int ct = blockIdx.x % a.n_ct;
    const int sp = blockIdx.x / a.n_ct;
    const int tx = sp % a.tiles_x, ty = sp / a.tiles_x;
    const int b = blockIdx.y;
    const int y0 = ty * kTH, x0 = tx * kTW;

    typename D::LaneOff lo;
    D::lane_offsets(q, lo);
    const int lane_x = ((2 * wave) * D::TWH + n) * D::SPIX;
    const int lane_w = lane * 16;

    f32x4 acc[4][NT];
#pragma unroll
    for (int nt = 0; nt < NT; ++nt) {
        f32x4 bv = f32x4{0.f, 0.f, 0.f, 0.f};
        if (a.bias) {
            const float4 t4 = *reinterpret_cast<const float4*>(a.bias + ct * Cfg::COUT_TILE + q * NV + nt * 4);
            bv = f32x4{t4.x, t4.y, t4.z, t4.w};
        }
#pragma unroll
        for (int pt = 0; pt < 4; ++pt) acc[pt][nt] = bv;
    }

    ConvArgs aa = a;
    if (ct != 0) aa.in_store = nullptr;
    const typename D::TileSrc ts = D::tile_src(aa, b, y0, x0);
    typename D::TileOffs to;
    D::tile_offsets(aa, tid, to);
    const char* wbase = static_cast<const char*>(a.wpacked) + (size_t)ct * a.n_chunks * Cfg::CHUNK_W_BYTES;

    for (int chunk = 0; chunk < a.n_chunks; ++chunk) {
        if (chunk > 0) __syncthreads();
        const char* wchunk = wbase + (size_t)chunk * Cfg::CHUNK_W_BYTES;
        D::dma_weights(wchunk, s_w, (STEPS < G ? STEPS : G) * NT, wave, lane_w);
        if (a.cin_vec_ok) {
            uint4 r0[D::NI], r1[GATED ? D::NI : 1];
            float gv[GATED ? D::UNIT : 1];
            D::template load_tile<GATED>(aa, ts, to, b, chunk, tid, r0, r1, gv);
            D::template commit_tile<GATED>(aa, ts, to, chunk, tid, r0, r1, gv, s_in);
        } else {
            D::stage_tile_scalar(aa, b, y0, x0, chunk, tid, s_in, static_cast<T*>(aa.in_store));
        }
        __syncthreads();
        D::template mma_steps<0, G, 0>(s_in, s_w, lane_x, lane_w, q, lo, acc);
        if constexpr (NSUB > 1) {
            __syncthreads();
            D::dma_weights(wchunk + (size_t)G * NT * 1024, s_w, ((STEPS - G) < G ? (STEPS - G) : G) * NT, wave, lane_w);
            __syncthreads();
            D::template mma_steps<G, G, G>(s_in, s_w, lane_x, lane_w, q, lo, acc);
        }
        if constexpr (NSUB > 2) {
            __syncthreads();
            D::dma_weights(wchunk + (size_t)2 * G * NT * 1024, s_w, ((STEPS - 2 * G) < G ? (STEPS - 2 * G) : G) * NT, wave, lane_w);
            __syncthreads();
            D::template mma_steps<2 * G, G, 2 * G>(s_in, s_w, lane_x, lane_w, q, lo, acc);
        }
        static_assert(NSUB <= 3, "add another weight sub-stage");
    }
    D::template epilogue<FAST>(a, b, y0, x0, sp, ct, tid, acc);
}

constexpr int kPersistMaxCout = 512;
template <class Cfg>
constexpr int persist_bias_slots() { return Cfg::KS == 5 ? 64 : kPersistMaxCout; }
template <class Cfg>
constexpr int persist_lds_bytes_c() { return Cfg::IN_BYTES + (int)Cfg::CHUNK_W_BYTES + persist_bias_slots<Cfg>() * 4; }

template <class Cfg>
constexpr int persist_blocks_per_cu() { return Cfg::NT <= 2 && persist_lds_bytes_c<Cfg>() * 3 <= 160 * 1024 ? 3 : 2; }

template <class Cfg, bool GATED, bool FAST>
__global__ __launch_bounds__(kThreads, persist_blocks_per_cu<Cfg>()) void conv_mfma_persist_kernel(const ConvArgs a) {
    using D = ConvDev<Cfg>;
    constexpr int NT = Cfg::NT, STEPS = Cfg::STEPS, NV = 4 * NT;

    const int w_copies = a.w_resident ? a.n_ct : 1;
    extern __shared__ __attribute__((aligned(16))) char smem[];
    char* s_w = smem;
    float* s_bias = reinterpret_cast<float*>(smem + w_copies * Cfg::CHUNK_W_BYTES);
    char* s_in = smem + w_copies * Cfg::CHUNK_W_BYTES + persist_bias_slots<Cfg>() * 4;

    const int tid = threadIdx.x, lane = tid & 63, wave = tid >> 6;
    const int q = lane >> 4, n = lane & 15;
    typename D::LaneOff lo;
    D::lane_offsets(q, lo);
    const int lane_x = ((2 * wave) * D::TWH + n) * D::SPIX;
    const int lane_w = lane * 16;

    const int sp_total = a.tiles_x * a.tiles_y;
    const int n_tiles = sp_total * a.batch;
    const int n_ct = a.n_ct;
    const int slots = gridDim.x >> 3;
    const int pos = (blockIdx.x & 7) * slots + (blockIdx.x >> 3);

    if (n_ct == 1 || a.w_resident) D::dma_weights(static_cast<const char*>(a.wpacked), s_w, STEPS * NT * w_copies, wave, lane_w);
    for (int i = tid; i < a.cout_packed; i += kThreads) s_bias[i] = a.bias ? a.bias[i] : 0.f;

    uint4 r0[D::NI], r1[GATED ? D::NI : 1];
    float gv[GATED ? D::UNIT : 1];
    typename D::TileOffs to;
    D::tile_offsets(a, tid, to);
    int tile = pos < n_tiles ? pos : -1;
    int b = 0, sp = 0, y0 = 0, x0 = 0;
    typename D::TileSrc ts;
    if (tile >= 0) {
        b = magic_div(tile, a.td.sp_total);
        int ty, tx;
        band_decode(tile - b * sp_total, a.tiles_x, a.tiles_y, a.td, ty, tx);
        sp = ty * a.tiles_x + tx; y0 = ty * kTH; x0 = tx * kTW;
        ts = D::tile_src(a, b, y0, x0);
        if (a.cin_vec_ok) {
            D::template load_gate<GATED>(a, b, 0, tid, gv);
            if (ts.interior) D::template load_tile_interior<GATED>(a, ts, to, 0, r0, r1);
        }
    }
    float run[NV];
#pragma unroll
    for (int e = 0; e < NV; ++e) run[e] = 0.f;
    int covered = 0;
    constexpr bool BORDER_PRE = !GATED && Cfg::KS == 3 && (NT == 3 || NT == 4) && sizeof(typename Cfg::elem) == 2;
    bool first_tile = true;
    while (tile >= 0) {
        __syncthreads();
        if (a.cin_vec_ok && !ts.interior && (!BORDER_PRE || first_tile || (a.dbg_flags & 16))) D::template load_tile_border<GATED>(a, ts, 0, tid, r0, r1);
        first_tile = false;
        if (a.cin_vec_ok) D::template commit_tile<GATED>(a, ts, to, 0, tid, r0, r1, gv, s_in);
        else D::stage_tile_scalar(a, b, y0, x0, 0, tid, s_in, static_cast<typename Cfg::elem*>(a.in_store));
        constexpr bool RUN_SUMS = FAST && sizeof(typename Cfg::elem) == 2 && NT >= 3;
        const int cb = b, csp = sp, cy0 = y0, cx0 = x0;
        const int next = tile + (int)gridDim.x;
        tile = next < n_tiles ? next : -1;
        if constexpr (RUN_SUMS) {
            const bool will_flush = tile < 0 || magic_div(tile, a.td.sp_total) != cb;
            if ((a.ep_key == D::EP_SUMS || a.ep_key == (D::EP_RELU | D::EP_SUMS)) && n_ct == 1) {
                if (!a.sums_compact) { if (!will_flush) D::zero_sum_slots(a, cb, csp, tid); }
                else if (will_flush) {
                    for (int bb = covered; bb < cb; ++bb) D::zero_slots4(a, bb, 4 * D::compact_residue(pos, bb, sp_total, (int)gridDim.x), tid);
                    covered = cb + 1;
                }
            }
        }

        for (int ct = 0; ct < n_ct; ++ct) {
            if (n_ct > 1 && !a.w_resident) {
                if (ct > 0) __syncthreads();
                D::dma_weights(static_cast<const char*>(a.wpacked) + (size_t)ct * Cfg::CHUNK_W_BYTES, s_w, STEPS * NT, wave, lane_w);
            }
            if (ct == 0 || !a.w_resident) __syncthreads();
            if (ct == n_ct - 1 && tile >= 0) {
                b = magic_div(tile, a.td.sp_total);
                int ty, tx;
                band_decode(tile - b * sp_total, a.tiles_x, a.tiles_y, a.td, ty, tx);
                sp = ty * a.tiles_x + tx; y0 = ty * kTH; x0 = tx * kTW;
                ts = D::tile_src(a, b, y0, x0);
                if (a.cin_vec_ok) {
                    D::template load_gate<GATED>(a, b, 0, tid, gv);
                    if (ts.interior) D::template load_tile_interior<GATED>(a, ts, to, 0, r0, r1);
                    else if constexpr (BORDER_PRE) { if (!(a.dbg_flags & 16)) D::template load_tile_border<GATED>(a, ts, 0, tid, r0, r1); }
                }
            }
            f32x4 acc[4][NT];
#pragma unroll
            for (int nt = 0; nt < NT; ++nt) {
                const float4 t4 = *reinterpret_cast<const float4*>(s_bias + ct * Cfg::COUT_TILE + q * NV + nt * 4);
#pragma unroll
                for (int pt = 0; pt < 4; ++pt) acc[pt][nt] = f32x4{t4.x, t4.y, t4.z, t4.w};
            }
            constexpr bool RESPRE = FAST && !GATED && sizeof(typename Cfg::elem) == 2 && NT <= 3;
            [[maybe_unused]] unsigned rpre[RESPRE ? 4 : 1][RESPRE ? D::NRH : 1];
            bool res_pre = false;
            if constexpr (RESPRE) {
                if ((a.ep_key == D::EP_RES || a.ep_key == (D::EP_GATE | D::EP_RES)) && a.out_mode == RC_OUT_NHWC) {
                    res_pre = true;
                    D::res_prefetch(a, cb, cy0, cx0, ct, tid, rpre);
                }
            }
            D::template mma_steps<0, STEPS, 0, (!GATED && NT < 5)>(s_in, a.w_resident ? s_w + ct * (int)Cfg::CHUNK_W_BYTES : s_w, lane_x, lane_w, q, lo, acc);
            if constexpr (FAST && sizeof(typename Cfg::elem) == 2) {
                const int rslot = a.sums_compact ? 4 * D::compact_residue(pos, cb, sp_total, (int)gridDim.x) : -1;
                if (RUN_SUMS && a.ep_key == D::EP_SUMS && n_ct == 1)
                    D::template epilogue_fast_impl<D::EP_SUMS, RUN_SUMS>(a, cb, cy0, cx0, csp, ct, tid, acc, run, tile < 0 || b != cb, rslot);
                else if (RUN_SUMS && a.ep_key == (D::EP_RELU | D::EP_SUMS) && n_ct == 1)
                    D::template epilogue_fast_impl<D::EP_RELU | D::EP_SUMS, RUN_SUMS>(a, cb, cy0, cx0, csp, ct, tid, acc, run, tile < 0 || b != cb, rslot);
                else if (res_pre) {
                    if constexpr (RESPRE) {
                        D::epilogue_res_pre(a, cb, cy0, cx0, ct, tid, acc, rpre, a.ep_key == (D::EP_GATE | D::EP_RES) ? a.out_scale + (size_t)cb * a.cout : nullptr);
                    }
                } else D::template epilogue<FAST>(a, cb, cy0, cx0, csp, ct, tid, acc);
            } else D::template epilogue<FAST>(a, cb, cy0, cx0, csp, ct, tid, acc);
        }
    }
    if constexpr (FAST && sizeof(typename Cfg::elem) == 2 && NT >= 3) {
        if (a.sums_compact && (a.ep_key == D::EP_SUMS || a.ep_key == (D::EP_RELU | D::EP_SUMS)) && n_ct == 1)
            for (int bb = covered; bb < a.batch; ++bb) D::zero_slots4(a, bb, 4 * D::compact_residue(pos, bb, sp_total, (int)gridDim.x), tid);
    }
}

constexpr int kWsThreads = 512;

template <class Cfg, bool GATED, bool FAST>
__global__ __launch_bounds__(kWsThreads) void conv_mfma_ws_kernel(const ConvArgs a) {
    using D = ConvDev<Cfg>;
    constexpr int NT = Cfg::NT, STEPS = Cfg::STEPS, NV = 4 * NT;

    extern __shared__ __attribute__((aligned(16))) char smem[];
    char* s_w = smem;
    float* s_bias = reinterpret_cast<float*>(smem + Cfg::CHUNK_W_BYTES);
    char* s_buf0 = smem + Cfg::CHUNK_W_BYTES + 16 * Cfg::NT * 4;
    char* s_buf1 = s_buf0 + Cfg::IN_BYTES;

    const int tid = threadIdx.x, lane = tid & 63;
    const int wave8 = __builtin_amdgcn_readfirstlane(tid >> 6);
    const bool loader = wave8 >= 4;
    const int rtid = tid & 255, wave = wave8 & 3;
    const int q = lane >> 4, n = lane & 15;

    const int sp_total = a.tiles_x * a.tiles_y;
    const int n_tiles = sp_total * a.batch;
    const int slots = gridDim.x >> 3;
    const int pos = (blockIdx.x & 7) * slots + (blockIdx.x >> 3);
    const int stride = (int)gridDim.x;
    const int my_tiles = pos < n_tiles ? (n_tiles - pos + stride - 1) / stride : 0;

    for (int kb = wave8; kb < STEPS * NT; kb += kWsThreads / 64)
        __builtin_amdgcn_global_load_lds((const __attribute__((address_space(1))) void*)(static_cast<const char*>(a.wpacked) + kb * 1024 + lane * 16),
                                         (__attribute__((address_space(3))) void*)(s_w + kb * 1024), 16, 0, 0);
    for (int i = tid; i < a.cout_packed; i += kWsThreads) s_bias[i] = a.bias ? a.bias[i] : 0.f;

    auto decode = [&](int tile, int& b, int& sp, int& y0, int& x0) {
        b = magic_div(tile, a.td.sp_total);
        int ty, tx;
        band_decode(tile - b * sp_total, a.tiles_x, a.tiles_y, a.td, ty, tx);
        sp = ty * a.tiles_x + tx; y0 = ty * kTH; x0 = tx * kTW;
    };

    if (loader) {
        uint4 r0[D::NI], r1[GATED ? D::NI : 1];
        float gv[GATED ? D::UNIT : 1];
        typename D::TileSrc ts;
        typename D::TileOffs to;
        D::tile_offsets(a, rtid, to);
        int b, sp, y0, x0;
        if (my_tiles > 0) {
            decode(pos, b, sp, y0, x0);
            ts = D::tile_src(a, b, y0, x0);
            D::template load_tile<GATED>(a, ts, to, b, 0, rtid, r0, r1, gv);
            D::template commit_tile<GATED>(a, ts, to, 0, rtid, r0, r1, gv, s_buf0);
        }
        if (my_tiles > 1) {
            decode(pos + stride, b, sp, y0, x0);
            ts = D::tile_src(a, b, y0, x0);
            D::template load_tile<GATED>(a, ts, to, b, 0, rtid, r0, r1, gv);
        }
        __syncthreads();
        const bool rec = a.dbg != nullptr && blockIdx.x == 8 && wave8 == 4 && lane == 0;
        for (int k = 0; k < my_tiles; ++k) {
            const long long tl0 = rec ? (long long)__builtin_amdgcn_s_memtime() : 0;
            if (k + 1 < my_tiles) {
                D::template commit_tile<GATED>(a, ts, to, 0, rtid, r0, r1, gv, ((k + 1) & 1) ? s_buf1 : s_buf0);
                if (k + 2 < my_tiles) {
                    decode(pos + (k + 2) * stride, b, sp, y0, x0);
// ... 128 lines not shown
        __syncthreads();
        for (int g = 0; g < my_stages; ++g) {
            const int wsoff_g = wsoff;
            dma(WA, WB, wsoff_g);
            if (g + 1 < my_stages) issue_a();
            __syncthreads();
            if (g + 1 < my_stages) {
                if (need_wa()) dma(0, WA, wsoff);
                commit_a();
            }
            __syncthreads();
        }
    } else {
        const int wave = wave12;
        typename D::LaneOff lo;
        D::lane_offsets(q, lo);
        const int lane_x = ((2 * wave) * D::TWH + n) * D::SPIX;
        const int lane_w = lane * 16;
        __syncthreads();
        int g = 0;
        for (int k = 0; k < my_units; ++k) {
            int b, ty, tx, ct0;
            decode(pos + k * stride, b, ty, tx, ct0);
            const int ty8 = 2 * ty + (wave >> 2);
            for (int ct = ct0; ct < ct0 + cts_per_unit; ++ct) {
                f32x4 acc[4][NT];
#pragma unroll
                for (int nt = 0; nt < NT; ++nt) {
                    const float4 t4 = *reinterpret_cast<const float4*>(s_bias + ct * Cfg::COUT_TILE + q * NV + nt * 4);
#pragma unroll
                    for (int pt = 0; pt < 4; ++pt) acc[pt][nt] = f32x4{t4.x, t4.y, t4.z, t4.w};
                }
                auto run_chunks = [&](auto PH, int c0, int c1) {
                    constexpr int ph = decltype(PH)::value;
                    for (int c = c0; c < c1; ++c, ++g) {
                        const char* s_in = s_in0 + (one_chunk ? (k & 1) : (g & 1)) * Cfg::IN_BYTES;
                        if constexpr (ph == 3) { if (!(a.dbg_flags & 2)) D::template mma_steps<0, SA, 0, true>(s_in, s_w, lane_x, lane_w, q, lo, acc); }
                        else if constexpr (ph == 2) D::template mma_steps<1, 1, 0, false>(s_in, s_w, lane_x, lane_w, q, lo, acc);
                        __syncthreads();
                        if constexpr ((ph & 1) != 0) { if (!(a.dbg_flags & 2)) D::template mma_steps<SA, STEPS - SA, 0, true>(s_in, s_w, lane_x, lane_w, q, lo, acc); }
                        else D::template mma_steps<3, 1, 0, false>(s_in, s_w, lane_x, lane_w, q, lo, acc);
                        if (c + 1 < n_chunks) __syncthreads();
                    }
                };
                if constexpr (FOLD_SKIP) {
                    const int cpp = D::folded(a) ? n_chunks >> 2 : 0;
                    run_chunks(std::integral_constant<int, 0>{}, 0, cpp);
                    run_chunks(std::integral_constant<int, 1>{}, cpp, 2 * cpp);
                    run_chunks(std::integral_constant<int, 2>{}, 2 * cpp, 3 * cpp);
                    run_chunks(std::integral_constant<int, 3>{}, 3 * cpp, n_chunks);
                } else {
                    run_chunks(std::integral_constant<int, 3>{}, 0, n_chunks);
                }
                if (ty8 < a.tiles_y)
                    D8::template epilogue<FAST>(a, b, ty8 * kTH, tx * kTW, ty8 * a.tiles_x + tx, ct, tid & 255, acc);
                __syncthreads();
            }
        }
    }
}

template <class Cfg8>
struct WstCfg : WsmCfg<Cfg8> {
    using B = WsmCfg<Cfg8>;
    static constexpr int SPIX = B::CK * (int)sizeof(typename B::elem);
    static constexpr int N_PIECES = B::THH * B::TWH * B::UPT;
    static constexpr int N_DMA = (N_PIECES + 63) / 64;
    static constexpr int IN_BYTES = N_DMA * 1024;
};
template <class Cfg>
constexpr int wst_form() {
    if (!(sizeof(typename Cfg::elem) == 2 && (Cfg::KS == 2 || Cfg::KS == 3) && (Cfg::UPT == 2 || Cfg::UPT == 4) && Cfg::STEPS >= 2)) return 0;
    const int w = (int)Cfg::CHUNK_W_BYTES, in = WstCfg<Cfg>::IN_BYTES, fixed = 2 * w + kPersistMaxCout * 4;
    if (w <= 20 * 1024 && fixed + 3 * in <= 160 * 1024) return 3;
    if (w <= 36 * 1024 && fixed + 2 * in <= 160 * 1024) return 2;
    return 0;
}
template <class Cfg>
constexpr int wst_lds_bytes() { return 2 * (int)Cfg::CHUNK_W_BYTES + kPersistMaxCout * 4 + (wst_form<Cfg>() == 3 ? 3 : 2) * WstCfg<Cfg>::IN_BYTES; }
template <class Cfg>
constexpr bool wst_eligible() { return wst_form<Cfg>() != 0; }
constexpr int waitcnt_vm(int n) { return (n & 15) | ((n >> 4) << 14) | 0x0F70; }

template <class Cfg8, bool FAST>
__global__ __launch_bounds__(kWsmThreads) void conv_mfma_wst_kernel(const ConvArgs a) {
#if defined(__HIP_DEVICE_COMPILE__)
    using Cfg = WstCfg<Cfg8>;
    using D = ConvDev<Cfg>;
    using D8 = ConvDev<Cfg8>;
    constexpr int NT = Cfg::NT, STEPS = Cfg::STEPS, NV = 4 * NT, WALL = (int)Cfg::CHUNK_W_BYTES, UPT = Cfg::UPT, TWH = Cfg::TWH, ES = 2;
    constexpr int N_DMA = Cfg::N_DMA, NDW = (N_DMA + 3) / 4;
    constexpr int NBUF = wst_form<Cfg8>() == 3 ? 3 : 2;
    constexpr bool FOLD_SKIP = Cfg::KS == 2 && UPT == 4 && STEPS == 4;

    extern __shared__ __attribute__((aligned(16))) char smem[];
    char* s_w = smem;
    float* s_bias = reinterpret_cast<float*>(smem + 2 * WALL);
    char* s_in0 = smem + 2 * WALL + kPersistMaxCout * 4;

    const int tid = threadIdx.x, lane = tid & 63;
    const int wave12 = __builtin_amdgcn_readfirstlane(tid >> 6);
    const bool loader = wave12 >= 8;
    const int q = lane >> 4, n = lane & 15;

    const int tiles_y = (a.H + kWsmTH - 1) / kWsmTH;
    const int sp_total = a.tiles_x * tiles_y;
    const int n_tiles = sp_total * a.batch;
    const int n_chunks = a.n_chunks, n_ct = a.n_ct;
    const bool one_chunk = n_chunks == 1;
    const int n_units = one_chunk ? n_tiles : n_tiles * n_ct;
    const int cts_per_unit = one_chunk ? n_ct : 1;
    const int slots = gridDim.x >> 3;
    const int pos = (blockIdx.x & 7) * slots + (blockIdx.x >> 3);
    const int stride = (int)gridDim.x;
    const int my_units = pos < n_units ? (n_units - pos + stride - 1) / stride : 0;
    const int my_stages = my_units * cts_per_unit * n_chunks;

    for (int i = tid; i < a.cout_packed; i += kWsmThreads) s_bias[i] = a.bias ? a.bias[i] : 0.f;

    auto decode = [&](int unit, int& b, int& ty, int& tx, int& ct0) {
        int tile = unit;
        ct0 = 0;
        if (!one_chunk) { tile = magic_div(unit, a.div_n_ct); ct0 = unit - tile * n_ct; }
        b = magic_div(tile, a.td_wsm.sp_total);
        band_decode(tile - b * sp_total, a.tiles_x, tiles_y, a.td_wsm, ty, tx);
    };

    if (loader && NBUF == 2) {
        if constexpr (NBUF == 2) {
            const int rtid = tid - kWsmCompute, w4 = wave12 - 8;
            uint4 r0[D::NI], r1[1];
            float gv[1];
            typename D::TileSrc ts;
            typename D::TileOffs to;
            D::tile_offsets(a, rtid, to);
            int k_unit = 0, cti = 0, chunk = 0, gi = 0, ct = 0;
            int b = 0, ty = 0, tx = 0, ct0 = 0;
            auto fetch = [&]() {
                if (gi < my_stages) {
                    if (chunk == 0) {
                        if (cti == 0) decode(pos + k_unit * stride, b, ty, tx, ct0);
                        ct = ct0 + cti;
                        ts = D::tile_src(a, b, ty * kWsmTH, tx * kTW);
                    }
                    const int goff = (ct * n_chunks + chunk) * WALL;
                    for (int kb = w4; kb < WALL / 1024; kb += 4)
                        __builtin_amdgcn_global_load_lds((const __attribute__((address_space(1))) void*)(static_cast<const char*>(a.wpacked) + goff + kb * 1024 + lane * 16),
                                                         (__attribute__((address_space(3))) void*)(s_w + (gi & 1) * WALL + kb * 1024), 16, 0, 0);
                    if (!one_chunk || cti == 0) {
                        D::template load_tile<false>(a, ts, to, b, chunk, rtid, r0, r1, gv);
                        D::template commit_tile<false>(a, ts, to, chunk, rtid, r0, r1, gv, s_in0 + (one_chunk ? (k_unit & 1) : (gi & 1)) * Cfg::IN_BYTES);
                    }
                }
                ++gi;
                if (++chunk == n_chunks) { chunk = 0; if (++cti == cts_per_unit) { cti = 0; ++k_unit; } }
            };
            fetch();
            __syncthreads();
            for (int g = 0; g < my_stages; ++g) {
                fetch();
                __syncthreads();
            }
        }
    } else if (loader) {
        const int w4 = wave12 - 8;
        int lc[NDW];
#pragma unroll
        for (int r = 0; r < NDW; ++r) {
            const int P = (w4 + 4 * r) * 64 + lane, pix = P / UPT, v = P - pix * UPT, py = pix / TWH, px = pix - py * TWH;
            const int o = D::folded(a) ? ((2 * py * a.src_W + 2 * px) * a.cfold + v * Cfg::UNIT) * ES : ((py * a.W + px) * a.cin + v * Cfg::UNIT) * ES;
            lc[r] = P < Cfg::N_PIECES ? o : kOOB;
        }
        typename D::TileSrc ts;
        int k_unit = 0, cti = 0, chunk = 0, gi = 0, gb3 = 0, kb3 = 0;
        int b = 0, ty = 0, tx = 0, ct0 = 0;
        const int n_mine = (N_DMA - w4 + 3) / 4;
        auto issue = [&]() -> int {
            const bool tile = gi < my_stages && (!one_chunk || cti == 0);
            char* dst = s_in0 + (one_chunk ? kb3 : gb3) * Cfg::IN_BYTES;
            int in_flight = 0;
            if (tile && chunk == 0) {
                decode(pos + k_unit * stride, b, ty, tx, ct0);
                ts = D::tile_src(a, b, ty * kWsmTH, tx * kTW);
            }
            if (tile && ts.interior) {
                const int soff = ts.soff + D::chunk_soff(a, chunk);
#pragma unroll
                for (int r = 0; r < NDW; ++r) {
                    const int inst = w4 + 4 * r;
                    if (inst < N_DMA)
                        __builtin_amdgcn_raw_ptr_buffer_load_lds(ts.r0, (__attribute__((address_space(3))) void*)(dst + inst * 1024), 16, lc[r], soff, 0, 0);
                }
                in_flight = n_mine;
            } else if (tile) {
                int ln = lane;
                asm volatile("" : "+v"(ln));
#pragma unroll
                for (int r = 0; r < NDW; ++r) {
                    const int inst = w4 + 4 * r, P = inst * 64 + ln, pix = P / UPT, v = P - pix * UPT;
                    if (inst < N_DMA) {
                        bool center;
// ... 2 lines not shown
                    }
                }
            }
            ++gi; gb3 = gb3 == 2 ? 0 : gb3 + 1;
            if (++chunk == n_chunks) { chunk = 0; if (++cti == cts_per_unit) { cti = 0; ++k_unit; kb3 = kb3 == 2 ? 0 : kb3 + 1; } }
            return in_flight;
        };
        int wi = 0, wk = 0, wcti = 0, wchunk = 0, wct0 = 0;
        auto issue_w = [&]() {
            if (wi < my_stages) {
                if (wchunk == 0 && wcti == 0) { int b_, ty_, tx_; decode(pos + wk * stride, b_, ty_, tx_, wct0); }
                const int goff = ((wct0 + wcti) * n_chunks + wchunk) * WALL;
                int ph = 3;
                if constexpr (FOLD_SKIP) ph = D::folded(a) ? D::fold_phase(a, wchunk * Cfg::CK) : 3;
                for (int kb = w4; kb < WALL / 1024; kb += 4) {
                    if constexpr (FOLD_SKIP) {
                        const int st = kb / NT;
                        if (!(st == 3 || ph == 3 || (ph == 1 && st == 2) || (ph == 2 && st == 1))) continue;
                    }
                    __builtin_amdgcn_global_load_lds((const __attribute__((address_space(1))) void*)(static_cast<const char*>(a.wpacked) + goff + kb * 1024 + lane * 16),
                                                     (__attribute__((address_space(3))) void*)(s_w + (wi & 1) * WALL + kb * 1024), 16, 0, 0);
                }
            }
            ++wi;
            if (++wchunk == n_chunks) { wchunk = 0; if (++wcti == cts_per_unit) { wcti = 0; ++wk; } }
        };
        issue_w();
        issue();
        issue();
        __syncthreads();
        for (int g = 0; g < my_stages; ++g) {
            issue_w();
            const int nfl = issue();
            if (nfl == NDW) __builtin_amdgcn_s_waitcnt(waitcnt_vm(NDW));
            else if (NDW > 1 && nfl == NDW - 1) __builtin_amdgcn_s_waitcnt(waitcnt_vm(NDW > 1 ? NDW - 1 : 0));
            else __builtin_amdgcn_s_waitcnt(waitcnt_vm(0));
            __builtin_amdgcn_s_barrier();
        }
        __builtin_amdgcn_s_waitcnt(waitcnt_vm(0));
    } else {
        const int wave = wave12;
        typename D::LaneOff lo;
        D::lane_offsets(q, lo);
        const int lane_x = ((2 * wave) * D::TWH + n) * D::SPIX;
        const int lane_w = lane * 16;
        __syncthreads();
        int g = 0, gb3 = 0, kb3 = 0;
        for (int k = 0; k < my_units; ++k) {
            int b, ty, tx, ct0;
            decode(pos + k * stride, b, ty, tx, ct0);
            const int ty8 = 2 * ty + (wave >> 2);
            for (int ct = ct0; ct < ct0 + cts_per_unit; ++ct) {
                f32x4 acc[4][NT];
#pragma unroll
                for (int nt = 0; nt < NT; ++nt) {
                    const float4 t4 = *reinterpret_cast<const float4*>(s_bias + ct * Cfg::COUT_TILE + q * NV + nt * 4);
#pragma unroll
                    for (int pt = 0; pt < 4; ++pt) acc[pt][nt] = f32x4{t4.x, t4.y, t4.z, t4.w};
                }
                auto run_chunks = [&](auto PH, int c0, int c1) {
                    constexpr int ph = decltype(PH)::value;
                    for (int c = c0; c < c1; ++c, ++g) {
                        const char* s_in = s_in0 + (one_chunk ? kb3 : gb3) * Cfg::IN_BYTES;
                        const char* s_wg = s_w + (g & 1) * WALL;
                        if constexpr (ph == 3) D::template mma_steps<0, STEPS, 0, true>(s_in, s_wg, lane_x, lane_w, q, lo, acc);
                        else if constexpr (ph == 1) D::template mma_steps<2, 2, 0, true>(s_in, s_wg, lane_x, lane_w, q, lo, acc);
                        else {
                            if constexpr (ph == 2) D::template mma_steps<1, 1, 0, false>(s_in, s_wg, lane_x, lane_w, q, lo, acc);
                            D::template mma_steps<3, 1, 0, false>(s_in, s_wg, lane_x, lane_w, q, lo, acc);
                        }
                        gb3 = gb3 == NBUF - 1 ? 0 : gb3 + 1;
                        if (c + 1 < n_chunks) __syncthreads();
                    }
                };
                if constexpr (FOLD_SKIP) {
                    const int cpp = D::folded(a) ? n_chunks >> 2 : 0;
                    run_chunks(std::integral_constant<int, 0>{}, 0, cpp);
                    run_chunks(std::integral_constant<int, 1>{}, cpp, 2 * cpp);
                    run_chunks(std::integral_constant<int, 2>{}, 2 * cpp, 3 * cpp);
                    run_chunks(std::integral_constant<int, 3>{}, 3 * cpp, n_chunks);
                } else {
                    run_chunks(std::integral_constant<int, 3>{}, 0, n_chunks);
                }
                if (ty8 < a.tiles_y)
                    D8::template epilogue<FAST>(a, b, ty8 * kTH, tx * kTW, ty8 * a.tiles_x + tx, ct, tid & 255, acc);
                __syncthreads();
            }
            kb3 = kb3 == NBUF - 1 ? 0 : kb3 + 1;
        }
    }
#endif
}

template <class Cfg>
constexpr int pss_lds_bytes() { return (int)Cfg::CHUNK_W_BYTES + kPersistMaxCout * 4 + WsmCfg<Cfg>::IN_BYTES + kWsmTH * kTW * Cfg::COUT_TILE * 2; }

template <class Cfg8>
__global__ __launch_bounds__(kWsmThreads) void conv_mfma_pss_kernel(const ConvArgs a) {
    using Cfg = WsmCfg<Cfg8>;
    using D = ConvDev<Cfg>;
    using T = typename Cfg::elem;
    static_assert(sizeof(T) == 2, "bf16 form");
    constexpr int NT = Cfg::NT, STEPS = Cfg::STEPS, NV = 4 * NT, NH = NV / 2;
    constexpr int SA = (STEPS + 1) / 2;
    constexpr int WA = SA * NT * 1024, WB = (STEPS - SA) * NT * 1024, WALL = (int)Cfg::CHUNK_W_BYTES;
    constexpr int NWA = (WA / 16 + kThreads - 1) / kThreads, NWB = (WB / 16 + kThreads - 1) / kThreads;
    constexpr int PXB = Cfg::COUT_TILE * 2, ROWB = kTW * PXB, OUTB = kWsmTH * ROWB;
    constexpr int UPP = PXB / 16, UPR = kTW * UPP;
    constexpr int NDR = OUTB / 16 / kThreads;
    static_assert(STEPS >= 2 && WA + WB == WALL && OUTB % (16 * kThreads) == 0 && NDR % 2 == 0 && PXB % 16 == 0, "pss shapes");

    extern __shared__ __attribute__((aligned(16))) char smem[];
    char* s_w = smem;
    float* s_bias = reinterpret_cast<float*>(smem + WALL);
    char* s_in = smem + WALL + kPersistMaxCout * 4;
    char* s_out = s_in + Cfg::IN_BYTES;

    const int tid = threadIdx.x, lane = tid & 63;
    const int wave12 = __builtin_amdgcn_readfirstlane(tid >> 6);
    const bool loader = wave12 >= 8;
    const int q = lane >> 4, n = lane & 15;

    const int tiles_y = (a.H + kWsmTH - 1) / kWsmTH;
    const int sp_total = a.tiles_x * tiles_y;
    const int n_tiles = sp_total * a.batch;
    constexpr int n_ct = 4;
    const int slots = gridDim.x >> 3;
    const int pos = (blockIdx.x & 7) * slots + (blockIdx.x >> 3);
    const int stride = (int)gridDim.x;
    const int my_units = pos < n_tiles ? (n_tiles - pos + stride - 1) / stride : 0;
    const int my_stages = my_units * n_ct;
    const int cps = a.cout >> 2;

    for (int i = tid; i < a.cout_packed; i += kWsmThreads) s_bias[i] = a.bias ? a.bias[i] : 0.f;

    auto decode = [&](int unit, int& b, int& ty, int& tx) {
        b = magic_div(unit, a.td_wsm.sp_total);
        band_decode(unit - b * sp_total, a.tiles_x, tiles_y, a.td_wsm, ty, tx);
    };

    if (loader) {
        const int rtid = tid - kWsmCompute;
        uint4 r0[D::NI], r1[1], wra[NWA], wrb[NWB];
        float gv[1];
        typename D::TileSrc ts;
        typename D::TileOffs to;
        D::tile_offsets(a, rtid, to);
        int lt = rtid;
        auto woa = [&](int k) { return (k * kThreads + lt) * 16 < WA ? (k * kThreads + lt) * 16 : kOOB; };
        auto wob = [&](int k) { return (k * kThreads + lt) * 16 < WB ? WA + (k * kThreads + lt) * 16 : kOOB; };
        const __amdgpu_buffer_rsrc_t r_w = make_rsrc(a.wpacked, (unsigned)((size_t)n_ct * WALL));
        const size_t img_out = (size_t)a.H * a.W * a.cout;

        int b = 0, ty = 0, tx = 0;
        int d_b = 0, d_y0 = 0, d_x0 = 0, d_ct = 0;
        int wsoff = 0;
        auto issue_tile = [&](int k) {
            decode(pos + k * stride, b, ty, tx);
            ts = D::tile_src(a, b, ty * kWsmTH, tx * kTW);
            D::template load_tile<false>(a, ts, to, b, 0, rtid, r0, r1, gv);
        };
        auto issue_wa = [&](int ct) {
            wsoff = ct * WALL;
#pragma unroll
            for (int k = 0; k < NWA; ++k) wra[k] = buf_load16(r_w, woa(k), wsoff);
        };
        auto issue_wb = [&]() {
#pragma unroll
            for (int k = 0; k < NWB; ++k) wrb[k] = buf_load16(r_w, wob(k), wsoff);
        };
        auto commit_tile = [&]() { D::template commit_tile<false>(a, ts, to, 0, rtid, r0, r1, gv, s_in); };
        auto commit_wa = [&]() {
#pragma unroll
            for (int k = 0; k < NWA; ++k)
                if (woa(k) != kOOB) *reinterpret_cast<uint4*>(s_w + woa(k)) = wra[k];
// ... 378 lines not shown
    for (int e = 0; e < (MODE == 1 ? NV : 1); ++e) run[e] = 0.f;
    [[maybe_unused]] int covered = 0;

    while (cu_ >= 0) {
#pragma unroll
        for (int k = 0; k < NI; ++k) {
            const int row0 = (8 * k) / TWH, thr = (row0 + 1) * TWH - 8 * k;
            const int pix = 8 * k + j8;
            const int px = pix - TWH * (row0 + ((thr < 8 && j8 >= thr) ? 1 : 0));
            *reinterpret_cast<uint4*>(s_my + pix * kA64PXB + ((cu ^ (px & 7)) * 16)) = r[k];
        }
        const int gy = cty8 * kTH + 2 * wv, gx0 = ctx * kTW + 16 * chalf, sp = cty8 * a.tiles_x + ctx;
        int nb = cb, nty8 = cty8, ntx = ctx, nu = cu_;
        const int nhalf = chalf ^ 1;
        if (chalf == 1) nu = decode(cu_ + stride, nb, nty8, ntx);
        unsigned rpre[MODE == 2 ? 2 : 1][MODE == 2 ? D::NRH : 1];
        if constexpr (MODE == 2) D::sub_res_prefetch(a, cb, gy, gx0, lane, rpre);
        issue(nu >= 0, nb, nty8, ntx, nhalf);

        f32x4 acc[2][NT];
#pragma unroll
        for (int nt = 0; nt < NT; ++nt) {
            const float4 t4 = *reinterpret_cast<const float4*>(s_bias + q * NV + nt * 4);
            acc[0][nt] = f32x4{t4.x, t4.y, t4.z, t4.w};
            acc[1][nt] = f32x4{t4.x, t4.y, t4.z, t4.w};
        }
        if (!(a.dbg_flags & 2)) {
            uint4 wfa[NT], xfa[2], wfb[NT], xfb[2];
#pragma unroll
            for (int nt = 0; nt < NT; ++nt) wfa[nt] = *reinterpret_cast<const uint4*>(s_w + nt * 1024 + lane_w);
            xfa[0] = *reinterpret_cast<const uint4*>(s_my + xo[0][0]);
            xfa[1] = *reinterpret_cast<const uint4*>(s_my + xo[0][0] + kA64ROWB);
#pragma unroll
            for (int s = 0; s < STEPS; s += 2) {
                a64_step<T, 0, true, NT>(s, s_my, s_w, lane_w, xo, wfa, xfa, wfb, xfb, acc);
                if (s + 2 < STEPS) a64_step<T, 0, true, NT>(s + 1, s_my, s_w, lane_w, xo, wfb, xfb, wfa, xfa, acc);
                else a64_step<T, 0, false, NT>(s + 1, s_my, s_w, lane_w, xo, wfb, xfb, wfa, xfa, acc);
            }
        }

        if constexpr (MODE == 1) {
            const bool last = chalf == 1;
            const bool flush = last && (nu < 0 || nb != cb);
            int slot = 4 * sp + wv;
            if (!a.sums_compact) {
                if (last && !flush) D::zero_slot1(a, cb, slot, lane);
            } else if (flush) {
                for (int bb = covered; bb < cb; ++bb) D::zero_slot1(a, bb, 4 * D::compact_residue(pos, bb, sp_total, stride) + wv, lane);
                covered = cb + 1;
                slot = 4 * D::compact_residue(pos, cb, sp_total, stride) + wv;
            }
            const unsigned none[1][1] = {{0u}};
            if (a.ep_key == EP_SUMS) D::template epilogue_sub<EP_SUMS, 1>(a, cb, gy, gx0, slot, lane, acc, run, flush, none, nullptr);
            else if (a.ep_key == (EP_RELU | EP_SUMS)) D::template epilogue_sub<EP_RELU | EP_SUMS, 1>(a, cb, gy, gx0, slot, lane, acc, run, flush, none, nullptr);
            else D::template epilogue_sub<EP_LEAKY | EP_SUMS, 1>(a, cb, gy, gx0, slot, lane, acc, run, flush, none, nullptr);
        } else if constexpr (MODE == 2) {
            float none[1] = {0.f};
            if (gated_out) D::template epilogue_sub<EP_GATE | EP_RES, 2>(a, cb, gy, gx0, 0, lane, acc, none, false, rpre, s_gate + cb * a.cout);
            else D::template epilogue_sub<EP_RES, 2>(a, cb, gy, gx0, 0, lane, acc, none, false, rpre, nullptr);
        } else {
            float none[1] = {0.f};
            const unsigned nonr[1][1] = {{0u}};
            if (a.ep_key == EP_RELU) D::template epilogue_sub<EP_RELU, 1>(a, cb, gy, gx0, 0, lane, acc, none, false, nonr, nullptr);
            else if (a.ep_key == EP_LEAKY) D::template epilogue_sub<EP_LEAKY, 1>(a, cb, gy, gx0, 0, lane, acc, none, false, nonr, nullptr);
            else D::template epilogue_sub<0, 1>(a, cb, gy, gx0, 0, lane, acc, none, false, nonr, nullptr);
        }
        cu_ = nu; cb = nb; cty8 = nty8; ctx = ntx; chalf = nhalf;
    }
    if constexpr (MODE == 1) {
        if (a.sums_compact)
            for (int bb = covered; bb < a.batch; ++bb) D::zero_slot1(a, bb, 4 * D::compact_residue(pos, bb, sp_total, stride) + wv, lane);
    }
}

template <class Cfg>
constexpr int ws_lds_bytes() { return 2 * Cfg::IN_BYTES + (int)Cfg::CHUNK_W_BYTES + 16 * Cfg::NT * 4; }

template <class Cfg>
constexpr int persist_lds_bytes() { return persist_lds_bytes_c<Cfg>(); }

template <class Cfg, bool FAST>
int launch_wst(const ConvArgs& a, int grid, hipStream_t stream) {
    return launch_lds<&conv_mfma_wst_kernel<Cfg, FAST>>(dim3((unsigned)grid), dim3(kWsmThreads), wst_lds_bytes<Cfg>(), stream, a);
}

template <class Cfg, bool GATED, bool FAST>
int launch_conv_g(const ConvArgs& a, hipStream_t stream) {
    constexpr int P_LDS = persist_lds_bytes<Cfg>();
    constexpr bool P_OK = P_LDS <= 80 * 1024;
    const int n_tiles = a.tiles_x * a.tiles_y * a.batch;
    const int legacy_slots = 4 * a.tiles_x * a.tiles_y;
    auto report = [&](int kind, int slots) -> bool {
        if (a.query == nullptr) return false;
        a.query[0] = kind; a.query[1] = slots;
        return true;
    };
    auto sums_mode = [&](int compact_slots, int& compact) -> int {
        compact = 0;
        if (a.chan_sums == nullptr || a.sum_slots == legacy_slots) return RC_OK;
        if (compact_slots > 0 && a.sum_slots == compact_slots) { compact = 1; return RC_OK; }
        return fail(RC_ERR_INVALID, "rc_conv2d: chan_sums_slots matches neither layout of the kernel this launch takes (ask rc_conv_sum_slots)");
    };
    if (a.out_mode == RC_OUT_NHWC_DWT) {
        if constexpr (!GATED && FAST && auto_eligible<Cfg>()) {
            using DD = ConvDev<Cfg>;
            static_assert(StripCfg<Cfg>::IN_BYTES >= 2 * kTW * (Cfg::COUT_TILE * 2 + 8), "the strip's output fits its own halo strip");
            if ((a.ep_key == 0 || a.ep_key == DD::EP_RELU || a.ep_key == DD::EP_LEAKY || a.ep_key == DD::EP_RES) && a.n_chunks == 1 && a.n_ct == 1 && a.cout == Cfg::COUT_TILE &&
                a.cin_vec_ok && a.cin_chunk_ok && n_tiles < (1 << 24)) {
                if (report(0, legacy_slots)) return RC_OK;
                constexpr int A_LDS = auto_lds_bytes<Cfg>();
                const int n_items = a.tiles_x * ((a.H + kWsmTH - 1) / kWsmTH) * a.batch;
                const dim3 grid((unsigned)persistent_grid(a.num_cus, n_items));
                if (a.ep_key == DD::EP_RES) return launch_lds<&conv_mfma_auto_kernel<Cfg, 2>>(grid, dim3(kAutoThreads), A_LDS, stream, a);
                return launch_lds<&conv_mfma_auto_kernel<Cfg, 0>>(grid, dim3(kAutoThreads), A_LDS, stream, a);
            }
        }
        return fail(RC_ERR_UNSUPPORTED, "rc_conv2d: RC_OUT_NHWC_DWT needs a bf16 / fp16 3x3 layer of one Cin chunk and one 32- or 48-wide cout tile (cin == cout == 32 or 48), 16-byte aligned operands");
    }
    constexpr int WS_LDS = ws_lds_bytes<Cfg>();
    if constexpr (WS_LDS <= 150 * 1024) {
        const bool ws_auto = GATED || Cfg::NT == 5 || Cfg::CK == 80;
        if (a.n_chunks == 1 && a.n_ct == 1 && a.cin_vec_ok && (a.persist_ok == 2 || (a.persist_ok == 1 && ws_auto)) && n_tiles < (1 << 24)) {
            if (report(0, legacy_slots)) return RC_OK;
            { int c_; if (int e_ = sums_mode(0, c_)) return e_; }
            return launch_lds<&conv_mfma_ws_kernel<Cfg, GATED, FAST>>(dim3((unsigned)persistent_grid(a.num_cus, n_tiles)), dim3(kWsThreads), WS_LDS, stream, a);
        }
    }
    if constexpr (!GATED && FAST && dtype_of<typename Cfg::elem>::value == RC_BF16 && Cfg::KS == 3 && Cfg::STEPS >= 2 && pss_lds_bytes<Cfg>() <= 160 * 1024 &&
                  (kWsmTH * kTW * Cfg::COUT_TILE * 2) % (16 * kThreads * 2) == 0) {
        if (a.pss && a.n_chunks == 1 && a.n_ct == 4 && a.cin_vec_ok && a.cin_chunk_ok && a.persist_ok && n_tiles < (1 << 24)) {
            if (report(0, legacy_slots)) return RC_OK;
            constexpr int PSS_LDS = pss_lds_bytes<Cfg>();
            const int n_items = a.tiles_x * ((a.H + kWsmTH - 1) / kWsmTH) * a.batch;
            return launch_lds<&conv_mfma_pss_kernel<Cfg>>(dim3((unsigned)persistent_grid(a.num_cus, n_items)), dim3(kWsmThreads), PSS_LDS, stream, a);
        }
    }
    constexpr int WSM_LDS = wsm_lds_bytes<Cfg>();
    if constexpr (!GATED && WSM_LDS <= 160 * 1024 && Cfg::KS >= 2 && Cfg::STEPS >= 2 && sizeof(typename Cfg::elem) == 2) {
        const bool res_pre_form = FAST && !GATED && sizeof(typename Cfg::elem) == 2 && Cfg::NT <= 3 && a.ep_key == ConvDev<Cfg>::EP_RES && a.out_mode == RC_OUT_NHWC;
        if ((a.n_chunks > 1 || (a.n_ct > 1 && a.persist_ok != 3 && !(P_OK && res_pre_form))) && a.cin_vec_ok && a.cin_chunk_ok && a.persist_ok && a.cout_packed <= kPersistMaxCout &&
            n_tiles < (1 << 24)) {
            if (report(0, legacy_slots)) return RC_OK;
            { int c_; if (int e_ = sums_mode(0, c_)) return e_; }
            const int n_items = a.tiles_x * ((a.H + kWsmTH - 1) / kWsmTH) * a.batch * (a.n_chunks > 1 ? a.n_ct : 1);
            const int grid = persistent_grid(a.num_cus, n_items);
            if constexpr ((FAST || Cfg::NT <= 3) && wst_eligible<Cfg>()) {
                if (a.thin >= (wst_form<Cfg>() == 3 ? 1 : 2)) return launch_wst<Cfg, FAST>(a, grid, stream);
            }
            return launch_lds<&conv_mfma_wsm_kernel<Cfg, GATED, FAST>>(dim3((unsigned)grid), dim3(kWsmThreads), WSM_LDS, stream, a);
        }
    }
    if constexpr (!GATED && FAST && auto64_eligible<Cfg>()) {
        using DD = ConvDev<Cfg>;
        const int k7 = a.ep_key;
        const bool key_ok = k7 == 0 || k7 == DD::EP_RELU || k7 == DD::EP_LEAKY || k7 == DD::EP_SUMS || k7 == (DD::EP_RELU | DD::EP_SUMS) || k7 == (DD::EP_LEAKY | DD::EP_SUMS) ||
                            k7 == DD::EP_RES || (k7 == (DD::EP_GATE | DD::EP_RES) && a.batch * a.cout <= kAutoGate);
        if (a.auto_impl && key_ok && a.n_chunks == 1 && a.n_ct == 1 && a.cout == Cfg::COUT_TILE && a.cin_vec_ok && a.persist_ok && a.out_mode == RC_OUT_NHWC && n_tiles < (1 << 24)) {
            constexpr int A_LDS = auto64_lds_bytes<Cfg>();
            static_assert(A_LDS <= 160 * 1024, "kernel 7 LDS");
            const int grid = persistent_grid(a.num_cus, (n_tiles + 1) / 2);
            const int cslots = ((k7 & DD::EP_SUMS) && a.sums_compact_ok && grid * 8 < legacy_slots) ? grid * 8 : 0;
            if (report(7, cslots ? cslots : legacy_slots)) return RC_OK;
            ConvArgs aa = a;
            if (int e_ = sums_mode(cslots, aa.sums_compact)) return e_;
            if (k7 & DD::EP_SUMS) return launch_lds<&conv_mfma_auto64_kernel<Cfg, 1>>(dim3((unsigned)grid), dim3(kAutoThreads), A_LDS, stream, aa);
            if (k7 & DD::EP_RES) return launch_lds<&conv_mfma_auto64_kernel<Cfg, 2>>(dim3((unsigned)grid), dim3(kAutoThreads), A_LDS, stream, aa);
// ... 56 lines not shown
```

### realcamnet_amd/networks.py

```python
from __future__ import annotations

from collections import OrderedDict

import torch
import torch.nn as nn

from . import ops
from ._lib import RC_OUT_NHWC, RC_OUT_PIXEL_SHUFFLE2


def _is_act(m) -> bool:
    return isinstance(m, (nn.ReLU, nn.LeakyReLU)) or (isinstance(m, nn.GELU) and m.approximate == "none")


def _act_args(m):
    if isinstance(m, nn.ReLU):
        return dict(act="relu")
    if isinstance(m, nn.GELU):
        return dict(act="gelu")
    return dict(act="leaky", slope=float(m.negative_slope))


class HipModule(nn.Module):

    def forward(self, x):
        a = ops.to_nhwc(x)
        return ops.to_nchw(self._nhwc(a))

    def _nhwc(self, a):
        raise NotImplementedError


class Conv2d(nn.Conv2d):

    def forward(self, x):
        return ops.to_nchw(self._nhwc(ops.to_nhwc(x)))

    def _nhwc(self, a, **fuse):
        if ops.is_down2x2(self):
            return ops.conv2x2s2(a, self, **fuse)
        if tuple(self.stride) == (2, 2) and ops.is_stride2(self):
            return ops.conv_stride2(a, self, **fuse)
        return ops.conv2d(a, self, **fuse)


class Sequential(nn.Sequential):

    def forward(self, x):
        if isinstance(x, (tuple, list)):
            a = (ops.to_nhwc(x[0]), *x[1:])
            y = self._nhwc(a)
            return (ops.to_nchw(y[0]), *y[1:])
        return ops.to_nchw(self._nhwc(ops.to_nhwc(x)))

    def _nhwc(self, a, residual=None):
        mods = list(self)
        i, n = 0, len(mods)
        while i < n:
            m = mods[i]
            if isinstance(m, Conv2d):
                kw = {}
                j = i + 1
                if j < n and _is_act(mods[j]):
                    kw.update(_act_args(mods[j]))
                    j += 1
                shuffle_after = False
                if j < n and isinstance(mods[j], nn.PixelShuffle):
                    if mods[j].upscale_factor != 2:
                        raise NotImplementedError("PixelShuffle: only upscale_factor=2 is on the hot path")
                    if (m.out_channels // 4) % 16 == 0:
                        kw["out_mode"] = RC_OUT_PIXEL_SHUFFLE2
                    else:
                        shuffle_after = True
                    j += 1
                if (j < n and isinstance(mods[j], DWTForward) and "out_mode" not in kw and not shuffle_after and
                        ops.conv_dwt_ok(a, m, mods[j], kw.get("act"), kw.get("slope", 0.0))):
                    kw["out_mode"] = ops.RC_OUT_NHWC_DWT
                    j += 1
                if j == n and residual is not None and kw.get("out_mode", RC_OUT_NHWC) == RC_OUT_NHWC and not shuffle_after:
                    kw["residual"], residual = residual, None
                a = m._nhwc(a, **kw)
                if shuffle_after:
                    a = ops.pixel_shuffle2(a)
                i = j
                continue
            if isinstance(m, RCAGroup) and i + 1 < n and isinstance(mods[i + 1], DWTForward) and not isinstance(a, (tuple, list)):
                a = m._nhwc(a, dwt=mods[i + 1])
                i += 2
                continue
            if isinstance(m, (nn.Dropout, nn.Identity)):
                i += 1
                continue
            if not hasattr(m, "_nhwc"):
                raise NotImplementedError(f"{type(m).__name__} has no HIP implementation on this path")
            a = m._nhwc(a)
            i += 1
        if residual is not None:
            raise NotImplementedError("trailing residual could not be fused (sequence does not end in a conv)")
        return a


def seq(*args):
    if len(args) == 1:
        args = args[0]
    if isinstance(args, nn.Module):
        return args
    if isinstance(args, OrderedDict):
        return Sequential(OrderedDict((k, seq(v)) for k, v in args.items()))
    assert isinstance(args, (list, tuple))
    return Sequential(*[seq(i) for i in args])


_UNSUPPORTED = "XTBIiSP34UuMA"


def conv(in_channels=64, out_channels=64, kernel_size=3, stride=1, padding=1, output_padding=0, dilation=1,
         groups=1, bias=True, padding_mode='zeros', mode='CBR'):
    L = []
    for t in mode:
        if t == 'C':
            L.append(Conv2d(in_channels=in_channels, out_channels=out_channels, kernel_size=kernel_size,
                            stride=stride, padding=padding, dilation=dilation, groups=groups, bias=bias,
                            padding_mode=padding_mode))
        elif t == 'R':
            L.append(nn.ReLU(inplace=True))
        elif t == 'r':
            L.append(nn.ReLU(inplace=False))
        elif t == 'L':
            L.append(nn.LeakyReLU(negative_slope=1e-1, inplace=True))
        elif t == 'l':
            L.append(nn.LeakyReLU(negative_slope=1e-1, inplace=False))
        elif t == '2':
            L.append(nn.PixelShuffle(upscale_factor=2))
        elif t in _UNSUPPORTED:
            raise NotImplementedError(f"conv mode '{t}' is not on the RAW->sRGB hot path (SURVEY.md section 8); no HIP kernel")
        else:
            raise NotImplementedError('Undefined type: {}'.format(t))
    return seq(*L)


_HAAR = [[[[0.5, 0.5], [0.5, 0.5]]],
         [[[0.5, 0.5], [-0.5, -0.5]]],
         [[[0.5, -0.5], [0.5, -0.5]]],
         [[[0.5, -0.5], [-0.5, 0.5]]]]


class DWTForward(nn.Conv2d):

    def __init__(self, in_channels=64):
        super().__init__(in_channels, in_channels * 4, 2, 2, groups=in_channels, bias=False)
        w = torch.tensor(_HAAR, dtype=torch.get_default_dtype()).repeat(in_channels, 1, 1, 1)
        self.weight.data.copy_(w)
        self.requires_grad_(False)

    def forward(self, x):
        return ops.to_nchw(self._nhwc(ops.to_nhwc(x)))

    def _nhwc(self, a):
        return ops.dwt_forward(a, self)


class DWTInverse(nn.ConvTranspose2d):

    def __init__(self, in_channels=64):
        super().__init__(in_channels, in_channels // 4, 2, 2, groups=in_channels // 4, bias=False)
        w = torch.tensor(_HAAR, dtype=torch.get_default_dtype()).repeat(in_channels // 4, 1, 1, 1)
        self.weight.data.copy_(w)
        self.requires_grad_(False)

    def forward(self, x, output_size=None):
        return ops.to_nchw(self._nhwc(ops.to_nhwc(x)))

    def _nhwc(self, a):
        return ops.dwt_inverse(a, self)


class DWTForward_(nn.Module):

    def __init__(self):
        super().__init__()
        ll, lh, hl, hh = [[0.5, 0.5], [0.5, 0.5]], [[-0.5, -0.5], [0.5, 0.5]], [[-0.5, 0.5], [-0.5, 0.5]], [[0.5, -0.5], [-0.5, 0.5]]
        flip = lambda f: [row[::-1] for row in f[::-1]]
# ... 140 lines not shown
```

### realcamnet_amd/ops.py

```python
from __future__ import annotations

import ctypes as C
import math
from typing import Optional, Tuple

import numpy as np
import os
import torch
from torch._subclasses.fake_tensor import FakeTensor

from . import _lib
from . import torch_ops as _T
from ._lib import (RC_ACT_GELU, RC_ACT_LEAKY, RC_ACT_NONE, RC_ACT_RELU, RC_ACT_RELU_POST, RC_BF16, RC_F16, RC_F32, RC_OUT_NCHW, RC_OUT_NHWC, RC_OUT_NHWC_DWT,
                   RC_OUT_PIXEL_SHUFFLE2, RC_OUT_PIXEL_SHUFFLE2_NCHW, ConvDesc, ConvPairDesc, check)

_DT = {torch.float32: RC_F32, torch.bfloat16: RC_BF16, torch.float16: RC_F16}
_HALF = (torch.bfloat16, torch.float16)
_R = torch.ops.realcam


def _opt(t: torch.Tensor) -> Optional[torch.Tensor]:
    return t if t.numel() else None

FUSE_GATE = True


def lib():
    return _lib.load()


def _dt(t: torch.Tensor) -> int:
    try:
        return _DT[t.dtype]
    except KeyError:
        raise TypeError(f"realcamnet_amd: unsupported dtype {t.dtype} (fp32 / bf16 / fp16)") from None


def require_dtype(t: torch.Tensor, allowed, what: str) -> None:
    if t.dtype not in allowed:
        names = " / ".join({torch.float32: "fp32", torch.bfloat16: "bf16", torch.float16: "fp16"}.get(d, str(d)) for d in allowed)
        raise TypeError(f"realcamnet_amd: {what} supports {names} only, got {t.dtype}")


def _req(t: torch.Tensor, name: str) -> torch.Tensor:
    if not isinstance(t, torch.Tensor):
        raise TypeError(f"{name}: expected a tensor")
    if not t.is_cuda:
        raise RuntimeError(f"{name}: tensor is on {t.device}; the HIP path has no CPU fallback "
                           "(use oracle/ for CPU reference results)")
    return t if t.is_contiguous() else t.contiguous()


def _stream() -> int:
    return torch.cuda.current_stream().cuda_stream


def _ptr(t: Optional[torch.Tensor]) -> Optional[int]:
    return None if t is None else t.data_ptr()


def derived(mod, slot, params, build, extra=None):
    cache = mod.__dict__.get("_rc_cache")
    if cache is None:
        cache = mod.__dict__["_rc_cache"] = {}
    key = (tuple(None if p is None else (id(p), 0 if isinstance(p, FakeTensor) else p.data_ptr(), p._version, p.dtype, str(p.device)) for p in params), extra)
    hit = cache.get(slot)
    if hit is not None and hit[0] == key:
        return hit[2]
    cache.pop(slot, None)
    value = build()
    cache[slot] = (key, tuple(params), value)
    return value


def drop_derived(mod, *slots) -> None:
    if not slots:
        mod.__dict__.pop("_rc_cache", None)
    for slot in slots:
        mod.__dict__.get("_rc_cache", {}).pop(slot, None)


def invalidate_caches(module) -> None:
    for m in module.modules():
        for k in ("_rc_cache", "_f32_masters", "_f32_verdict", "_graphs"):
            m.__dict__.pop(k, None)


def f32_param(mod, name: str) -> torch.Tensor:
    p = getattr(mod, name)
    if p.dtype == torch.float32 and p.is_contiguous():
        return _req(p.detach(), name)
    return derived(mod, ("f32", name), (p,), lambda: _req(p.detach(), name).float().contiguous())


class PackedConv:
    __slots__ = ("wpacked", "bias", "cin", "cout", "ksize", "dtype", "out_mode")

# ... 543 lines not shown

def conv2d(x: torch.Tensor, mod, *, act: Optional[str] = None, slope: float = 0.0,
           residual: Optional[torch.Tensor] = None, mul_plus1: Optional[torch.Tensor] = None,
           film: Optional[Tuple[torch.Tensor, torch.Tensor]] = None,
           gate: Optional[torch.Tensor] = None, skip: Optional[torch.Tensor] = None, store_input: bool = False,
           out_mode: int = RC_OUT_NHWC, want_sums: bool = False,
           crop_hw: Optional[Tuple[int, int]] = None, out_dtype: Optional[torch.dtype] = None,
           out_scale: Optional[torch.Tensor] = None):
    if mod.weight.dim() == 4:
        check_conv_module(mod)
    x = _req(x, "conv input")
    b, H, W, cin = x.shape
    algo = 1 if mod.weight.dim() == 4 and winograd_ok(x, mod, act=act, gate=gate, skip=skip, mul_plus1=mul_plus1, out_mode=out_mode, store_input=store_input) else 0
    if algo:
        ct = 0
        pc = packed_wino(mod, x.dtype)
    else:
        ct = small_map_cout_tile(x, mod, out_mode)
        pc = packed_conv(mod, x.dtype, RC_OUT_NHWC if out_mode == RC_OUT_NHWC_DWT else out_mode, ct)
    if cin != pc.cin:
        raise ValueError(f"conv expects {pc.cin} input channels, got {cin}")
    if gate is not None:
        if skip is None:
            raise ValueError("gate needs skip")
        skip = _req(skip, "skip")
        gate = _req(gate, "gate")
        if skip.shape != x.shape or skip.dtype != x.dtype or gate.shape != (b, cin) or gate.dtype != torch.float32:
            raise ValueError("gate/skip shape or dtype mismatch")
    fs = ft = None
    if film is not None:
        fs, ft = (_req(t, "film") for t in film)
        if fs.shape != (b, pc.cout) or ft.shape != (b, pc.cout) or fs.dtype != torch.float32 or ft.dtype != torch.float32:
            raise ValueError("film tensors must be fp32 (B, cout)")
    if mul_plus1 is not None:
        mul_plus1 = _req(mul_plus1, "mul_plus1")
    if out_scale is not None:
        out_scale = _req(out_scale, "out_scale")
        if out_scale.shape != (b, pc.cout) or out_scale.dtype != torch.float32 or out_mode != RC_OUT_NHWC:
            raise ValueError("out_scale must be fp32 (B, cout) and needs the NHWC store")
    if residual is not None:
        residual = _req(residual, "residual")
    for name, t in (("mul_plus1", mul_plus1), ("residual", residual)):
        if t is not None and (t.shape != (b, H, W, pc.cout) or t.dtype != x.dtype):
            raise ValueError(f"{name} must be NHWC {(b, H, W, pc.cout)} {x.dtype}, got {tuple(t.shape)} {t.dtype}")
    planar = out_mode in (RC_OUT_NCHW, RC_OUT_PIXEL_SHUFFLE2_NCHW)
    ch, cw = (crop_hw if crop_hw is not None else (0, 0)) if planar else (0, 0)
    if out_dtype is not None:
        _DT[out_dtype]
    out, stored, sums = _R.conv2d(x, pc.wpacked, pc.bias, pc.cout, pc.ksize, _ACT[act], float(slope), residual, mul_plus1, fs, ft, gate, skip,
                                  bool(store_input), int(out_mode), bool(want_sums), int(ch), int(cw),
                                  out_dtype if planar else None, out_scale, ct, algo)
    extras = [t for t in (_opt(stored), _opt(sums)) if t is not None]
    return (out, *extras) if extras else out


FUSE_DWT = os.environ.get("RC_FUSE_DWT", "1") != "0"
_HAAR_TAPS = (0.5, 0.5, 0.5, 0.5, 0.5, 0.5, -0.5, -0.5, 0.5, -0.5, 0.5, -0.5, 0.5, -0.5, -0.5, 0.5)


def conv_dwt_ok(x: torch.Tensor, conv, dwt, act: Optional[str] = None, slope: float = 0.0, residual: bool = False) -> bool:
    if residual and act is not None:
        return False
    if not FUSE_DWT or x.dtype not in _HALF or x.dim() != 4 or conv.weight.dim() != 4:
        return False
    cout, cin, kh, kw = conv.weight.shape
    if not (kh == kw == 3 and cin == cout and cin in (32, 48) and x.shape[3] == cin and x.shape[1] % 2 == 0 and x.shape[2] % 2 == 0):
        return False
    if tuple(conv.stride) != (1, 1) or tuple(conv.padding) != (1, 1) or tuple(conv.dilation) != (1, 1) or conv.groups != 1:
        return False
    if act not in (None, "relu", "leaky") or (act == "leaky" and not (0.0 <= slope <= 1.0)):
        return False
    w = getattr(dwt, "weight", None)
    if w is None or tuple(w.shape) != (4 * cout, 1, 2, 2):
        return False
    if isinstance(w, FakeTensor):
        return True

    def taps_are_haar():
        want = torch.tensor(_HAAR_TAPS, dtype=torch.float32).reshape(4, 1, 2, 2).repeat(cout, 1, 1, 1)
        return bool(torch.equal(w.detach().float().cpu(), want))
    return derived(dwt, "haar_ok", (w,), taps_are_haar)


FUSE_SHUFFLE_STORE = True

FOLD_TAIL = True


def tail_fold_ok(x: torch.Tensor, conv1, conv2) -> bool:
    w1, w2 = conv1.weight, conv2.weight
    if not (FOLD_TAIL and x.dim() == 4 and x.dtype in _DT and x.shape[1] >= 2 and x.shape[2] >= 2 and w1.dim() == 4 and w2.dim() == 4):
        return False
    c = x.shape[-1]
    return (tuple(w1.shape) == (4 * c, c, 3, 3) and tuple(w2.shape[1:]) == (c, 3, 3) and 4 * w2.shape[0] <= 16 and
            _lib.load().rc_conv_packed_bytes(c, 4 * w2.shape[0], 5, _DT[x.dtype], RC_OUT_PIXEL_SHUFFLE2_NCHW) != 0)


def _folded_tail(conv1, conv2) -> "_ConvView":
    def fold():
        det = lambda t: None if t is None else t.detach()
        wc, bc = _R.tail_fold_weights(conv1.weight.detach(), det(conv1.bias), conv2.weight.detach(), det(conv2.bias))
        c = conv1.weight.shape[1]
        perm = (torch.arange(c, device=conv1.weight.device)[:, None] * 4 + torch.tensor([0, 2, 1, 3], device=conv1.weight.device)[None, :]).reshape(-1)
        v1t = _ConvView(conv1.weight.detach().transpose(2, 3)[perm].contiguous(), None if conv1.bias is None else conv1.bias.detach()[perm].contiguous())
        v2t = _ConvView(conv2.weight.detach().transpose(2, 3).contiguous(), det(conv2.bias))
        return _ConvView(wc, bc), v1t, v2t
    return derived(conv2, "tail_fold", (conv1.weight, conv1.bias, conv2.weight, conv2.bias), fold)


def tail_fold(x: torch.Tensor, conv1, conv2, crop_hw: Optional[Tuple[int, int]] = None, out_dtype: Optional[torch.dtype] = None) -> torch.Tensor:
    x = _req(x, "tail input")
    b, H, W, _ = x.shape
    odt = out_dtype or x.dtype

    folded, c1t, c2t = _folded_tail(conv1, conv2)

    def ring():
        rows, cols_t = _R.tail_ring_gather(x)
        return [conv2d(conv2d(t, m1, out_mode=RC_OUT_PIXEL_SHUFFLE2), m2, out_mode=RC_OUT_NCHW, out_dtype=odt) for t, m1, m2 in ((rows, conv1, conv2), (cols_t, c1t, c2t))]

    strips, out = fork_join(ring, lambda: conv2d(x, folded, out_mode=RC_OUT_PIXEL_SHUFFLE2_NCHW, crop_hw=crop_hw, out_dtype=odt), [x])
    _R.tail_ring_scatter(out, strips[0], strips[1], H, W)
    return out


FUSE_PAIR = False


def conv_pair_ok(x: torch.Tensor, m1, m2) -> bool:
    return (FUSE_PAIR and x.dtype == torch.bfloat16 and x.shape[-1] == 48 and
            all(m.weight.dim() == 4 and tuple(m.weight.shape) == (48, 48, 3, 3) for m in (m1, m2)))


def conv_pair(x: torch.Tensor, m1, m2, *, act: str = "relu", slope: float = 0.0,
              film: Optional[Tuple[torch.Tensor, torch.Tensor]] = None,
              gate: Optional[torch.Tensor] = None, skip: Optional[torch.Tensor] = None, store_input: bool = False,
              residual: Optional[torch.Tensor] = None, want_sums: bool = False):
    require_dtype(x, (torch.bfloat16,), "conv_pair (rc_conv_pair)")
    for m in (m1, m2):
        check_conv_module(m)
    x = _req(x, "conv_pair input")
    b, H, W, c = x.shape
    p1, p2 = packed_conv(m1, x.dtype, RC_OUT_NHWC), packed_conv(m2, x.dtype, RC_OUT_NHWC)
    if gate is not None:
        if skip is None:
            raise ValueError("gate needs skip")
        skip, gate = _req(skip, "skip"), _req(gate, "gate")
        if skip.shape != x.shape or skip.dtype != x.dtype or gate.shape != (b, c) or gate.dtype != torch.float32:
            raise ValueError("gate/skip shape or dtype mismatch")
    fs = ft = None
    if film is not None:
        fs, ft = (_req(t, "film") for t in film)
        if fs.shape != (b, c) or ft.shape != (b, c) or fs.dtype != torch.float32 or ft.dtype != torch.float32:
            raise ValueError("film tensors must be fp32 (B, C)")
    if residual is not None:
        residual = _req(residual, "residual")
        if residual.shape != x.shape or residual.dtype != x.dtype:
            raise ValueError("residual must match the input tensor")
    out, stored, sums = _R.conv_pair(x, p1.wpacked, p1.bias, p2.wpacked, p2.bias, _ACT[act], float(slope), fs, ft, gate, skip, bool(store_input),
                                     residual, bool(want_sums))
    extras = [t for t in (_opt(stored), _opt(sums)) if t is not None]
    return (out, *extras) if extras else out


FUSE_CHAIN = True

# ... 362 lines not shown
```

### realcamnet_amd/torch_ops.py

```python
from __future__ import annotations

import ctypes as C
from typing import List, Optional

import numpy as np
import torch
from torch import Tensor

from . import _lib
from ._lib import RC_BF16, RC_F16, RC_F32, RC_OUT_NCHW, RC_OUT_NHWC, RC_OUT_NHWC_DWT, RC_OUT_PIXEL_SHUFFLE2, RC_OUT_PIXEL_SHUFFLE2_NCHW, ConvDesc, ConvPairDesc, check

_DT = {torch.float32: RC_F32, torch.bfloat16: RC_BF16, torch.float16: RC_F16}
_LIB = torch.library.Library("realcam", "DEF")
SCHEMAS = {}


def lib():
    return _lib.load()


def _dt(t: Tensor) -> int:
    return _DT[t.dtype]


def _stream() -> int:
    return torch.cuda.current_stream().cuda_stream


def _p(t: Optional[Tensor]):
    return None if t is None else t.data_ptr()


def _none(x: Tensor) -> Tensor:
    return x.new_empty((0,))


def require_acts(op: str, dtype, *tensors) -> None:
    for t in tensors:
        if t is None:
            continue
        if t.dtype != dtype:
            raise TypeError(f"realcam::{op}: activation tensor of dtype {t.dtype}, expected {dtype}")
        if not t.is_contiguous():
            raise ValueError(f"realcam::{op}: non-contiguous activation tensor (shape {tuple(t.shape)}, strides {t.stride()})")


def define(schema: str, alloc, launch, acts=None):
    name = schema.split("(")[0]
    SCHEMAS[name] = schema
    _LIB.define(schema)

    def cuda_impl(*args):
        if acts is not None:
            require_acts(name, *acts(*args))
        outs = alloc(*args)
        launch(outs, *args)
        return outs

    def fake_impl(*args):
        return alloc(*args)

    _LIB.impl(name, cuda_impl, "CUDA")
    torch.library.register_fake(f"realcam::{name}", fake_impl, lib=_LIB)


def _bu_alloc(mosaic, dtype, pad_to):
    b, h2, w2 = mosaic.shape
    h, w = h2 // 2, w2 // 2
    return mosaic.new_empty((b, -(-h // pad_to) * pad_to, -(-w // pad_to) * pad_to, 4), dtype=dtype)


def _bu_launch(out, mosaic, dtype, pad_to):
    b, h2, w2 = mosaic.shape
    check(lib().rc_bayer_unshuffle(mosaic.data_ptr(), _dt(mosaic), out.data_ptr(), _DT[dtype], b, h2 // 2, w2 // 2, out.shape[1], out.shape[2],
                                   _stream()), "rc_bayer_unshuffle")


define("bayer_unshuffle(Tensor mosaic, ScalarType dtype, int pad_to) -> Tensor", _bu_alloc, _bu_launch)


def _ingest_alloc(mosaic, dtype, pad_to, black, white, cond_h, cond_w):
    b, h2, w2 = mosaic.shape
    h, w = h2 // 2, w2 // 2
    return (mosaic.new_empty((b, -(-h // pad_to) * pad_to, -(-w // pad_to) * pad_to, 4), dtype=dtype),
            mosaic.new_empty((b, 4, cond_h, cond_w), dtype=dtype))


def _ingest_launch(outs, mosaic, dtype, pad_to, black, white, cond_h, cond_w):
    packed, cond = outs
    b, h2, w2 = mosaic.shape
    in_dt = _lib.RC_U16 if mosaic.dtype == torch.uint16 else _dt(mosaic)
    check(lib().rc_raw_ingest(mosaic.data_ptr(), in_dt, packed.data_ptr(), cond.data_ptr(), _DT[dtype], b, h2 // 2, w2 // 2,
                              packed.shape[1], packed.shape[2], cond_h, cond_w, float(black), float(white), _stream()), "rc_raw_ingest")
# ... 79 lines not shown
            or mesh.shape[0] not in (1, y.shape[0])):
        raise ValueError(f"realcam::warp: the mesh must be a contiguous float32 tensor (1 or {y.shape[0]}, {gh}, {gw}, 2) on {y.device}, got {tuple(mesh.shape)} {mesh.dtype}")
    if cell not in (8, 16, 32, 64) or len(fill) != 3:
        raise ValueError(f"realcam::warp: cell must be 8, 16, 32 or 64 and fill three floats, got {cell!r}, {fill!r}")
    check(lib().rc_warp(y.data_ptr(), _dt(y), out.data_ptr(), _DT[dtype], mesh.data_ptr(), mesh.shape[0], cell.bit_length() - 1, interp, border,
                        float(fill[0]), float(fill[1]), float(fill[2]), y.shape[0], y.shape[2], y.shape[3], h, w, oh, ow, _stream()), "rc_warp")


define("warp(Tensor y, Tensor mesh, int cell, int interp, int border, float[] fill, int h, int w, int oh, int ow, ScalarType dtype) -> Tensor",
       lambda y, mesh, cell, interp, border, fill, h, w, oh, ow, dtype: y.new_empty((y.shape[0], 3, oh, ow), dtype=dtype), _warp_launch)

define("nchw_to_nhwc(Tensor x, ScalarType dtype, int hp, int wp) -> Tensor",
       lambda x, dtype, hp, wp: x.new_empty((x.shape[0], hp, wp, x.shape[1]), dtype=dtype),
       lambda out, x, dtype, hp, wp: check(lib().rc_nchw_to_nhwc(x.data_ptr(), _dt(x), out.data_ptr(), _DT[dtype], x.shape[0], x.shape[1],
                                                                 x.shape[2], x.shape[3], hp, wp, _stream()), "rc_nchw_to_nhwc"))

define("nhwc_to_nchw(Tensor a, ScalarType dtype, int h, int w) -> Tensor",
       lambda a, dtype, h, w: a.new_empty((a.shape[0], a.shape[3], h, w), dtype=dtype),
       lambda out, a, dtype, h, w: check(lib().rc_nhwc_to_nchw(a.data_ptr(), _dt(a), out.data_ptr(), _DT[dtype], a.shape[0], a.shape[3],
                                                               a.shape[1], a.shape[2], h, w, _stream()), "rc_nhwc_to_nchw"))


def _wshape(weight):
    if weight.dim() == 2:
        return weight.shape[0], weight.shape[1], 1
    return weight.shape[0], weight.shape[1], weight.shape[2]


def _pack_alloc(weight, bias, act_dtype, out_mode, cout_tile=0):
    cout, cin, k = _wshape(weight)
    L = lib()
    dt = _DT[act_dtype]
    nbytes = L.rc_conv_packed_bytes_ct(cin, cout, k, dt, out_mode, cout_tile)
    if nbytes == 0:
        raise _lib.HipError(f"rc_conv_packed_bytes: {L.rc_last_error().decode()}")
    n_packed = L.rc_conv_packed_cout_ct(cin, cout, k, dt, out_mode, cout_tile)
    return (weight.new_empty((nbytes,), dtype=torch.uint8),
            weight.new_empty((n_packed if bias is not None else 0,), dtype=torch.float32))


def _pack_launch(outs, weight, bias, act_dtype, out_mode, cout_tile=0):
    wp, bp = outs
    cout, cin, k = _wshape(weight)
    L = lib()
    dt = _DT[act_dtype]
    w_host = np.ascontiguousarray(weight.detach().float().cpu().numpy())
    dst = np.empty(wp.numel(), dtype=np.uint8)
    check(L.rc_conv_pack_weights_ct(w_host.ctypes.data, cin, cout, k, dt, out_mode, cout_tile, dst.ctypes.data), "rc_conv_pack_weights")
    wp.copy_(torch.from_numpy(dst))
    if bias is not None:
        b_host = np.ascontiguousarray(bias.detach().float().cpu().numpy())
        bdst = np.zeros(bp.numel(), dtype=np.float32)
        check(L.rc_conv_pack_bias_ct(b_host.ctypes.data, cin, cout, k, dt, out_mode, cout_tile, bdst.ctypes.data), "rc_conv_pack_bias")
        bp.copy_(torch.from_numpy(bdst))


define("conv_pack_weights(Tensor weight, Tensor? bias, ScalarType act_dtype, int out_mode, int cout_tile=0) -> (Tensor, Tensor)", _pack_alloc, _pack_launch)


def _wino_pack_alloc(weight, act_dtype):
    cout, cin, k = _wshape(weight)
    nbytes = lib().rc_wino_packed_bytes(cin, cout, _DT[act_dtype]) if k == 3 else 0
    if nbytes == 0:
        raise _lib.HipError(f"rc_wino_packed_bytes: {lib().rc_last_error().decode() if k == 3 else 'a 3x3 form'}")
    return weight.new_empty((nbytes,), dtype=torch.uint8)


def _wino_pack_launch(out, weight, act_dtype):
    cout, cin, _ = _wshape(weight)
    w_host = np.ascontiguousarray(weight.detach().float().cpu().numpy())
    dst = np.empty(out.numel(), dtype=np.uint8)
    check(lib().rc_wino_pack_weights(w_host.ctypes.data, cin, cout, _DT[act_dtype], dst.ctypes.data), "rc_wino_pack_weights")
    out.copy_(torch.from_numpy(dst))


define("wino_pack_weights(Tensor weight, ScalarType act_dtype) -> Tensor", _wino_pack_alloc, _wino_pack_launch)


def _conv_alloc(x, wpacked, bias, cout, ksize, act, slope, residual, mul_plus1, film_scale, film_shift, gate, skip, store_input, out_mode,
                want_sums, crop_h, crop_w, out_dtype, out_scale=None, cout_tile=0, algo=0):
    b, H, W, _ = x.shape
    if out_mode == RC_OUT_NHWC:
        out = x.new_empty((b, H, W, cout))
    elif out_mode == RC_OUT_PIXEL_SHUFFLE2:
        out = x.new_empty((b, 2 * H, 2 * W, cout // 4))
    elif out_mode == RC_OUT_NHWC_DWT:
        out = x.new_empty((b, H // 2, W // 2, 4 * cout))
    elif out_mode == RC_OUT_PIXEL_SHUFFLE2_NCHW:
        out = x.new_empty((b, cout // 4, crop_h if crop_h > 0 else 2 * H, crop_w if crop_w > 0 else 2 * W), dtype=out_dtype or x.dtype)
    else:
        out = x.new_empty((b, cout, crop_h if crop_h > 0 else H, crop_w if crop_w > 0 else W), dtype=out_dtype or x.dtype)
    stored = torch.empty_like(x) if (store_input and gate is not None) else _none(x)
    sums = x.new_empty((0,), dtype=torch.float32)
    if want_sums:
        d = ConvDesc()
        d.batch, d.height, d.width, d.cin, d.cout, d.ksize, d.dtype = b, H, W, x.shape[-1], cout, ksize, _DT[x.dtype]
        from torch._subclasses.fake_tensor import FakeTensor

        def stand_in(t):
            return 4096 + (0 if (t is None or isinstance(t, FakeTensor) or not t.is_cuda) else t.data_ptr() % 16)
        d.in0, d.wpacked, d.out, d.chan_sums = stand_in(x), stand_in(wpacked), stand_in(out), 4096
        if gate is not None:
            d.in1, d.in_gate = stand_in(skip), stand_in(gate)
            if store_input:
                d.in_store = 4096
        for name, t in (("bias", bias), ("film_scale", film_scale), ("film_shift", film_shift), ("mul_plus1", mul_plus1), ("residual", residual), ("out_scale", out_scale)):
            if t is not None:
                setattr(d, name, stand_in(t))
        d.act, d.act_slope, d.out_mode, d.out_dtype = act, float(slope), out_mode, _DT[out.dtype]
        d.cout_tile = cout_tile
        d.algo = algo
        if out_mode in (RC_OUT_NCHW, RC_OUT_PIXEL_SHUFFLE2_NCHW):
            d.out_h, d.out_w = out.shape[2], out.shape[3]
        if x.is_cuda and not isinstance(x, FakeTensor):
            with torch.cuda.device(x.device):
                n = lib().rc_conv_sum_slots(C.byref(d))
        else:
            n = lib().rc_conv_sum_slots(C.byref(d))
        if n <= 0:
            n = lib().rc_conv_sum_tiles(H, W)
        sums = x.new_empty((b, n, cout), dtype=torch.float32)
    return out, stored, sums


def _conv_launch(outs, x, wpacked, bias, cout, ksize, act, slope, residual, mul_plus1, film_scale, film_shift, gate, skip, store_input,
                 out_mode, want_sums, crop_h, crop_w, out_dtype, out_scale=None, cout_tile=0, algo=0):
    out, stored, sums = outs
    b, H, W, cin = x.shape
    d = ConvDesc()
    d.batch, d.height, d.width, d.cin, d.cout, d.ksize, d.dtype = b, H, W, cin, cout, ksize, _dt(x)
    d.in0 = x.data_ptr()
    if gate is not None:
        d.in1, d.in_gate = skip.data_ptr(), gate.data_ptr()
        if stored.numel():
            d.in_store = stored.data_ptr()
    d.wpacked, d.bias = wpacked.data_ptr(), _p(bias)
    d.film_scale, d.film_shift = _p(film_scale), _p(film_shift)
    d.act, d.act_slope = act, float(slope)
    d.mul_plus1, d.residual, d.out_scale = _p(mul_plus1), _p(residual), _p(out_scale)
    d.out, d.out_mode = out.data_ptr(), out_mode
    d.out_dtype = _dt(out)
    d.cout_tile = cout_tile
    d.algo = algo
    if out_mode in (RC_OUT_NCHW, RC_OUT_PIXEL_SHUFFLE2_NCHW):
        d.out_h, d.out_w = out.shape[2], out.shape[3]
    if want_sums:
        d.chan_sums = sums.data_ptr()
        d.chan_sums_slots = sums.shape[1]
    check(lib().rc_conv2d(C.byref(d), _stream()), "rc_conv2d")


define("conv2d(Tensor x, Tensor wpacked, Tensor? bias, int cout, int ksize, int act, float slope, Tensor? residual, Tensor? mul_plus1, "
       "Tensor? film_scale, Tensor? film_shift, Tensor? gate, Tensor? skip, bool store_input, int out_mode, bool want_sums, "
       "int crop_h, int crop_w, ScalarType? out_dtype, Tensor? out_scale=None, int cout_tile=0, int algo=0) -> (Tensor, Tensor, Tensor)", _conv_alloc, _conv_launch)


def _conv_fold2_launch(out, x, wpacked, bias, cout, act, slope):
    b, H, W, c = x.shape
    d = ConvDesc()
    d.batch, d.height, d.width, d.cin, d.cout, d.ksize, d.dtype = b, (H + 1) // 2, (W + 1) // 2, 4 * c, cout, 2, _dt(x)
    d.src_h, d.src_w = H, W
    d.in0, d.wpacked, d.bias = x.data_ptr(), wpacked.data_ptr(), _p(bias)
    d.act, d.act_slope = act, float(slope)
    d.out, d.out_mode, d.out_dtype = out.data_ptr(), RC_OUT_NHWC, _dt(out)
    check(lib().rc_conv2d(C.byref(d), _stream()), "rc_conv2d")


# ... 590 lines not shown
```

Baseline: 1323 MP/s.

## Fuse inverse Haar DWT into preceding 3x3 conv epilogue

Adds an RC_OUT_NHWC_IDWT output mode in which the last 3x3 conv of the middle/up3/up2 blocks applies the inverse Haar wavelet in its epilogue. The following up block then skips its DWTInverse module. This removes a separate IDWT launch and a full round trip of the intermediate tensor through memory at each decoder level. In exchange it needs a permuted weight/bias packing, cross-lane permlane swaps in the epilogue, and new kernel instantiations. It is limited to bf16/fp16 layers whose cin/cout fit the 48- or 64-wide cout tile forms.

```diff
diff --git a/include/realcam_hip.h b/include/realcam_hip.h
--- a/include/realcam_hip.h
+++ b/include/realcam_hip.h
@@ -29,7 +29,8 @@
     RC_OUT_PIXEL_SHUFFLE2 = 1,
     RC_OUT_NCHW = 2,
     RC_OUT_PIXEL_SHUFFLE2_NCHW = 3,
-    RC_OUT_NHWC_DWT = 4
+    RC_OUT_NHWC_DWT = 4,
+    RC_OUT_NHWC_IDWT = 5
 } rc_out_mode;
 
 int rc_abi_version(void);
@@ -167,6 +168,7 @@
 int rc_conv_packed_cout(int cin, int cout, int ksize, int dtype, int out_mode);
 int rc_conv_pack_bias(const float* bias_host, int cin, int cout, int ksize, int dtype, int out_mode,
                       float* dst_host);
+int rc_conv_idwt_ok(int dtype, int cin, int cout, int ksize);
 size_t rc_conv_packed_bytes_ct(int cin, int cout, int ksize, int dtype, int out_mode, int cout_tile);
 int rc_conv_packed_cout_ct(int cin, int cout, int ksize, int dtype, int out_mode, int cout_tile);
 int rc_conv_pack_weights_ct(const float* w_oihw_host, int cin, int cout, int ksize, int dtype, int out_mode, int cout_tile, void* dst_host);
diff --git a/realcamnet_amd/LiteISP.py b/realcamnet_amd/LiteISP.py
--- a/realcamnet_amd/LiteISP.py
+++ b/realcamnet_amd/LiteISP.py
@@ -362,10 +362,11 @@
         d1 = self._refine_d1(self.down1._nhwc(h))
         d2 = self.down2._nhwc(mod(2, d1))
         d3 = self.down3._nhwc(mod(3, d2))
-        m = self.middle._nhwc(mod(4, d3), residual=d3)
-        u3 = self.up3._nhwc(m, residual=d2)
-        u2 = self.up2._nhwc(u3, residual=d1)
-        u1 = self.up1._nhwc(u2, residual=h)
+        nxt = {s: (getattr(self, s)[0] if ops.FUSE_IDWT and isinstance(getattr(self, s)[0], N.DWTInverse) else None) for s in ("up3", "up2", "up1")}
+        m = self.middle._nhwc(mod(4, d3), residual=d3, idwt=nxt["up3"])
+        u3 = self.up3._nhwc(m, residual=d2, idwt=nxt["up2"], skip_first=nxt["up3"] is not None)
+        u2 = self.up2._nhwc(u3, residual=d1, idwt=nxt["up1"], skip_first=nxt["up2"] is not None)
+        u1 = self.up1._nhwc(u2, residual=h, skip_first=nxt["up1"] is not None)
         if ops.tail_fold_ok(u1, self.tail[0], self.tail[2]):
             return ops.tail_fold(u1, self.tail[0], self.tail[2], crop_hw=crop_hw, out_dtype=self.output_dtype)
         t = self.tail[0]._nhwc(u1, out_mode=RC_OUT_PIXEL_SHUFFLE2)
diff --git a/realcamnet_amd/_lib.py b/realcamnet_amd/_lib.py
--- a/realcamnet_amd/_lib.py
+++ b/realcamnet_amd/_lib.py
@@ -11,7 +11,7 @@
 
 RC_F32, RC_BF16, RC_U16, RC_F16 = 0, 1, 2, 3
 RC_ACT_NONE, RC_ACT_RELU, RC_ACT_LEAKY, RC_ACT_GELU, RC_ACT_RELU_POST = 0, 1, 2, 3, 4
-RC_OUT_NHWC, RC_OUT_PIXEL_SHUFFLE2, RC_OUT_NCHW, RC_OUT_PIXEL_SHUFFLE2_NCHW, RC_OUT_NHWC_DWT = 0, 1, 2, 3, 4
+RC_OUT_NHWC, RC_OUT_PIXEL_SHUFFLE2, RC_OUT_NCHW, RC_OUT_PIXEL_SHUFFLE2_NCHW, RC_OUT_NHWC_DWT, RC_OUT_NHWC_IDWT = 0, 1, 2, 3, 4, 5
 ABI_VERSION = 15
 RC_RAW_F32, RC_RAW_BF16, RC_RAW_U16, RC_RAW_F16, RC_RAW_U8, RC_RAW_MIPI10, RC_RAW_MIPI12 = 0, 1, 2, 3, 4, 5, 6
 RC_CFA_RGGB, RC_CFA_BGGR, RC_CFA_GRBG, RC_CFA_GBRG = 0, 1, 2, 3
@@ -104,6 +104,7 @@
     "rc_conv_pack_weights": (C.c_int, [_P, _I, _I, _I, _I, _I, _P]),
     "rc_conv_packed_cout": (C.c_int, [_I, _I, _I, _I, _I]),
     "rc_conv_pack_bias": (C.c_int, [_P, _I, _I, _I, _I, _I, _P]),
+    "rc_conv_idwt_ok": (C.c_int, [_I, _I, _I, _I]),
     "rc_conv_packed_bytes_ct": (_SZ, [_I, _I, _I, _I, _I, _I]),
     "rc_wino_packed_bytes": (_SZ, [_I, _I, _I]),
     "rc_wino_pack_weights": (C.c_int, [_P, _I, _I, _I, _P]),
diff --git a/realcamnet_amd/csrc/conv.hip b/realcamnet_amd/csrc/conv.hip
--- a/realcamnet_amd/csrc/conv.hip
+++ b/realcamnet_amd/csrc/conv.hip
@@ -59,11 +59,13 @@
     else if (h16 && ksize == 3 && p->ck == 32 && cout % 32 == 0) p->nt = 2;
     else p->nt = 1;
     if (cout_tile != 0) {
-        if (cout_tile < 16 || cout_tile > 80 || cout_tile % 16 != 0 || ksize == 5 || ksize == 2 || out_mode == RC_OUT_PIXEL_SHUFFLE2 || out_mode == RC_OUT_PIXEL_SHUFFLE2_NCHW) return false;
+        if (cout_tile < 16 || cout_tile > 80 || cout_tile % 16 != 0 || ksize == 5 || ksize == 2 || out_mode == RC_OUT_PIXEL_SHUFFLE2 || out_mode == RC_OUT_PIXEL_SHUFFLE2_NCHW ||
+            out_mode == RC_OUT_NHWC_IDWT) return false;
         p->nt = cout_tile / 16;
     }
     p->m32 = 0;
-    if (cout_tile == 0 && dtype == RC_BF16 && ksize == 3 && g_conv32 != 0 && cout <= kPersistMaxCout && out_mode != RC_OUT_NCHW && out_mode != RC_OUT_PIXEL_SHUFFLE2_NCHW) {
+    if (cout_tile == 0 && dtype == RC_BF16 && ksize == 3 && g_conv32 != 0 && cout <= kPersistMaxCout && out_mode != RC_OUT_NCHW && out_mode != RC_OUT_PIXEL_SHUFFLE2_NCHW &&
+        out_mode != RC_OUT_NHWC_IDWT) {
         const int cw = out_mode == RC_OUT_PIXEL_SHUFFLE2 ? cout / 4 : cout;
         const bool all = g_conv32 != 4;
         if (all && p->ck == 32 && cin % 32 == 0 && (out_mode == RC_OUT_PIXEL_SHUFFLE2 ? cw % 32 == 0 : cw % 64 == 0)) { p->m32 = 1; p->nt = 2; p->ck = (g_conv32 == 1 && out_mode == RC_OUT_NHWC) ? 16 : 32; }
@@ -98,6 +100,12 @@
     return j < cout ? j : -1;
 }
 
+static bool idwt_plan_ok(const ConvPlan& p, int cin, int cout, int ksize, int dtype) {
+    if (dtype == RC_F32 || ksize != 3 || p.m32 || cout % 64 != 0 || cout > kPersistMaxCout || p.cout_packed != cout || cin % p.ck != 0) return false;
+    return (p.ck == 48 && p.nt == 3 && p.n_chunks == 1) || (p.ck == 32 && p.nt == 4 && p.n_chunks > 1);
+}
+static int idwt_cout(int g, int k, int e) { return 4 * (16 * g + e) + k; }
+
 int wino_conv(const rc_conv_desc* d, hipStream_t stream);
 int wino_sum_slots(int H, int W, int cout);
 void wino_set_nnt(int v);
@@ -142,6 +150,7 @@
 size_t rc_conv_packed_bytes_ct(int cin, int cout, int ksize, int dtype, int out_mode, int cout_tile) {
     ConvPlan p;
     if (!make_plan(cin, cout, ksize, dtype, out_mode, &p, cout_tile)) { set_error("rc_conv_packed_bytes: bad shape"); return 0; }
+    if (out_mode == RC_OUT_NHWC_IDWT && !idwt_plan_ok(p, cin, cout, ksize, dtype)) { set_error("rc_conv_packed_bytes: RC_OUT_NHWC_IDWT has no form for this layer (rc_conv_idwt_ok)"); return 0; }
     return (size_t)p.n_ct * p.n_chunks * p.steps * p.nt * 1024;
 }
 size_t rc_conv_packed_bytes(int cin, int cout, int ksize, int dtype, int out_mode) { return rc_conv_packed_bytes_ct(cin, cout, ksize, dtype, out_mode, 0); }
@@ -151,6 +160,10 @@
     if (!make_plan(cin, cout, ksize, dtype, out_mode, &p, cout_tile)) return fail(RC_ERR_INVALID, "rc_conv_packed_cout: bad shape");
     return p.cout_packed;
 }
+int rc_conv_idwt_ok(int dtype, int cin, int cout, int ksize) {
+    ConvPlan p;
+    return make_plan(cin, cout, ksize, dtype, RC_OUT_NHWC_IDWT, &p, 0) && idwt_plan_ok(p, cin, cout, ksize, dtype) ? 1 : 0;
+}
 int rc_conv_packed_cout(int cin, int cout, int ksize, int dtype, int out_mode) { return rc_conv_packed_cout_ct(cin, cout, ksize, dtype, out_mode, 0); }
 
 int rc_conv_pack_weights(const float* w, int cin, int cout, int ksize, int dtype, int out_mode, void* dst) {
@@ -164,6 +177,8 @@
     ConvPlan p;
     RC_REQUIRE(w && dst, "rc_conv_pack_weights: null pointer");
     RC_REQUIRE(make_plan(cin, cout, ksize, dtype, out_mode, &p, cout_tile), "rc_conv_pack_weights: bad shape");
+    const bool idwt = out_mode == RC_OUT_NHWC_IDWT;
+    if (idwt && !idwt_plan_ok(p, cin, cout, ksize, dtype)) return fail(RC_ERR_UNSUPPORTED, "rc_conv_pack_weights: RC_OUT_NHWC_IDWT has no form for this layer (rc_conv_idwt_ok)");
     const int kk = ksize * ksize;
     char* out = static_cast<char*>(dst);
     if (p.m32) {
@@ -193,7 +208,7 @@
                         int tap = 0, cu = 0;
                         const bool live = unit_map(p.upt, kk, s, qk, tap, cu);
                         const int j = ct * 16 * p.nt + (m >> 2) * (4 * p.nt) + nt * 4 + (m & 3);
-                        const int co = packed_to_cout(p, cout, out_mode, j);
+                        const int co = (idwt && p.nt == 4) ? idwt_cout(ct, nt, m) : packed_to_cout(p, cout, out_mode, j);
                         for (int e = 0; e < p.unit; ++e) {
                             float val = 0.f;
                             if (live && co >= 0 && co < cout) {
@@ -214,8 +229,10 @@
     ConvPlan p;
     RC_REQUIRE(dst, "rc_conv_pack_bias: null pointer");
     RC_REQUIRE(make_plan(cin, cout, ksize, dtype, out_mode, &p, cout_tile), "rc_conv_pack_bias: bad shape");
+    const bool idwt = out_mode == RC_OUT_NHWC_IDWT;
+    if (idwt && !idwt_plan_ok(p, cin, cout, ksize, dtype)) return fail(RC_ERR_UNSUPPORTED, "rc_conv_pack_bias: RC_OUT_NHWC_IDWT has no form for this layer (rc_conv_idwt_ok)");
     for (int j = 0; j < p.cout_packed; ++j) {
-        const int co = packed_to_cout(p, cout, out_mode, j);
+        const int co = (idwt && p.nt == 4) ? idwt_cout(j / 64, (j % 64) / 16, j % 16) : packed_to_cout(p, cout, out_mode, j);
         dst[j] = (bias && co >= 0 && co < cout) ? bias[co] : 0.f;
     }
     return RC_OK;
@@ -339,11 +356,25 @@
 static int conv_build_args(const rc_conv_desc* d, ConvPlan& p, ConvArgs& a, size_t& es_out) {
     RC_REQUIRE(d != nullptr, "rc_conv2d: null desc");
     const bool dwt = d->out_mode == RC_OUT_NHWC_DWT;
-    RC_REQUIRE(make_plan(d->cin, d->cout, d->ksize, d->dtype, dwt ? (int)RC_OUT_NHWC : d->out_mode, &p, d->cout_tile), "rc_conv2d: unsupported cin/cout/ksize/dtype/cout_tile");
+    const bool idwt = d->out_mode == RC_OUT_NHWC_IDWT;
+    RC_REQUIRE(make_plan(d->cin, d->cout, d->ksize, d->dtype, dwt ? (int)RC_OUT_NHWC : d->out_mode, &p, idwt ? 0 : d->cout_tile), "rc_conv2d: unsupported cin/cout/ksize/dtype/cout_tile");
     RC_REQUIRE(d->batch >= 1 && d->height >= 1 && d->width >= 1, "rc_conv2d: empty tensor");
     RC_REQUIRE(d->batch <= 65535, "rc_conv2d: batch > 65535");
     RC_REQUIRE(d->in0 && d->wpacked && d->out, "rc_conv2d: null in0/wpacked/out");
-    RC_REQUIRE(d->out_mode >= RC_OUT_NHWC && d->out_mode <= RC_OUT_NHWC_DWT, "rc_conv2d: bad out_mode");
+    RC_REQUIRE(d->out_mode >= RC_OUT_NHWC && d->out_mode <= RC_OUT_NHWC_IDWT, "rc_conv2d: bad out_mode");
+    if (idwt) {
+        RC_REQUIRE(d->out_dtype == d->dtype && reinterpret_cast<uintptr_t>(d->out) % 16 == 0, "rc_conv2d: RC_OUT_NHWC_IDWT: out_dtype must equal dtype, out 16-byte aligned");
+        if (d->dtype == RC_F32) return fail(RC_ERR_UNSUPPORTED, "rc_conv2d: RC_OUT_NHWC_IDWT is a bf16 / fp16 form (fp32 keeps the two launches)");
+        if (d->ksize != 3) return fail(RC_ERR_UNSUPPORTED, "rc_conv2d: RC_OUT_NHWC_IDWT is a 3x3 form");
+        if (d->cout % 64 != 0) return fail(RC_ERR_UNSUPPORTED, "rc_conv2d: RC_OUT_NHWC_IDWT needs cout % 64 == 0");
+        if (d->act != RC_ACT_NONE) return fail(RC_ERR_UNSUPPORTED, "rc_conv2d: RC_OUT_NHWC_IDWT excludes an activation (act must be RC_ACT_NONE)");
+        if (d->chan_sums) return fail(RC_ERR_UNSUPPORTED, "rc_conv2d: RC_OUT_NHWC_IDWT excludes chan_sums");
+        if (d->mul_plus1 || d->film_scale || d->film_shift || d->out_scale) return fail(RC_ERR_UNSUPPORTED, "rc_conv2d: RC_OUT_NHWC_IDWT excludes mul_plus1 / film / out_scale");
+        if (d->in_gate || d->in1 || d->in_store) return fail(RC_ERR_UNSUPPORTED, "rc_conv2d: RC_OUT_NHWC_IDWT excludes the gated input");
+        if (d->src_h || d->src_w || d->cout_tile) return fail(RC_ERR_UNSUPPORTED, "rc_conv2d: RC_OUT_NHWC_IDWT excludes src_h / src_w / cout_tile");
+        if (!idwt_plan_ok(p, d->cin, d->cout, d->ksize, d->dtype))
+            return fail(RC_ERR_UNSUPPORTED, "rc_conv2d: RC_OUT_NHWC_IDWT has no form for this (cin, cout): cin == 48 with cout % 192 == 0, or cin = several 32-channel chunks, cout <= 512 (rc_conv_idwt_ok)");
+    }
     if (dwt) {
         RC_REQUIRE(d->height % 2 == 0 && d->width % 2 == 0, "rc_conv2d: RC_OUT_NHWC_DWT needs even height and width");
         RC_REQUIRE(d->out_dtype == d->dtype && reinterpret_cast<uintptr_t>(d->out) % 16 == 0, "rc_conv2d: RC_OUT_NHWC_DWT: out_dtype must equal dtype, out 16-byte aligned");
@@ -359,7 +390,7 @@
     RC_REQUIRE((d->film_scale == nullptr) == (d->film_shift == nullptr), "rc_conv2d: film_scale/film_shift must come together");
     const bool full_tiles = d->cout == p.cout_packed;
     if (d->mul_plus1 || d->residual)
-        RC_REQUIRE((full_tiles || d->cout % 4 == 0) && (d->out_mode == RC_OUT_NHWC || (dwt && !d->mul_plus1)), "rc_conv2d: mul_plus1/residual need cout % 4 == 0 and RC_OUT_NHWC (residual: or RC_OUT_NHWC_DWT)");
+        RC_REQUIRE((full_tiles || d->cout % 4 == 0) && (d->out_mode == RC_OUT_NHWC || ((dwt || idwt) && !d->mul_plus1)), "rc_conv2d: mul_plus1/residual need cout % 4 == 0 and RC_OUT_NHWC (residual: or RC_OUT_NHWC_DWT / RC_OUT_NHWC_IDWT)");
     if (d->chan_sums) RC_REQUIRE(d->out_mode == RC_OUT_NHWC, "rc_conv2d: chan_sums needs RC_OUT_NHWC");
     if (d->out_scale) {
         RC_REQUIRE(d->out_mode == RC_OUT_NHWC && !p.m32, "rc_conv2d: out_scale needs RC_OUT_NHWC and a layer outside the 32x32x16 forms");
@@ -367,7 +398,7 @@
     }
     const size_t es = dtype_size(d->dtype);
     const int planar16 = d->dtype == RC_F16 ? RC_F16 : RC_BF16;
-    if (dwt) {
+    if (dwt || idwt) {
     } else if (d->out_mode == RC_OUT_NHWC) {
         RC_REQUIRE(d->out_dtype == d->dtype, "rc_conv2d: out_dtype must equal dtype for RC_OUT_NHWC");
         RC_REQUIRE(!full_tiles || (d->cout * es) % 8 == 0, "rc_conv2d: cout*elem_size must be a multiple of 8 bytes for RC_OUT_NHWC");
diff --git a/realcamnet_amd/csrc/conv_dispatch.hip b/realcamnet_amd/csrc/conv_dispatch.hip
--- a/realcamnet_amd/csrc/conv_dispatch.hip
+++ b/realcamnet_amd/csrc/conv_dispatch.hip
@@ -31,8 +31,15 @@
 int conv_f16_k1_ck16(int nt, const ConvArgs& a, hipStream_t s);
 int conv_f16_k1_ck48(int nt, const ConvArgs& a, hipStream_t s);
 int conv_f16_k1_ck64(int nt, const ConvArgs& a, hipStream_t s);
+int conv_bf16_k3_idwt(int ck, int nt, const ConvArgs& a, hipStream_t s);
+int conv_f16_k3_idwt(int ck, int nt, const ConvArgs& a, hipStream_t s);
 
 int dispatch_conv(int dtype, int ksize, int ck, int nt, const ConvArgs& a, hipStream_t s) {
+    if (a.out_mode == RC_OUT_NHWC_IDWT) {
+        if (ksize == 3 && dtype == RC_BF16) return conv_bf16_k3_idwt(ck, nt, a, s);
+        if (ksize == 3 && dtype == RC_F16) return conv_f16_k3_idwt(ck, nt, a, s);
+        return fail(RC_ERR_UNSUPPORTED, "conv: RC_OUT_NHWC_IDWT is a bf16 / fp16 3x3 form");
+    }
     if (dtype == RC_F16) {
         if (ksize == 3 && ck == 8) return conv_f16_k3_ck8(nt, a, s);
         if (ksize == 3 && ck == 16) return conv_f16_k3_ck16(nt, a, s);
diff --git a/realcamnet_amd/csrc/conv_inst_bf16_k3_idwt.hip b/realcamnet_amd/csrc/conv_inst_bf16_k3_idwt.hip
--- /dev/null
+++ b/realcamnet_amd/csrc/conv_inst_bf16_k3_idwt.hip
@@ -0,0 +1,8 @@
+#include "conv_kernel.hpp"
+namespace rc {
+int conv_bf16_k3_idwt(int ck, int nt, const ConvArgs& a, hipStream_t s) {
+    if (ck == 48 && nt == 3) return launch_conv_idwt<ConvCfg<bf16_t, 48, 3, 3>>(a, s);
+    if (ck == 32 && nt == 4) return launch_conv_idwt<ConvCfg<bf16_t, 32, 4, 3>>(a, s);
+    return fail(RC_ERR_UNSUPPORTED, "conv: no RC_OUT_NHWC_IDWT kernel instantiation for this (chunk width, cout tile width)");
+}
+}
diff --git a/realcamnet_amd/csrc/conv_inst_f16_k3_idwt.hip b/realcamnet_amd/csrc/conv_inst_f16_k3_idwt.hip
--- /dev/null
+++ b/realcamnet_amd/csrc/conv_inst_f16_k3_idwt.hip
@@ -0,0 +1,8 @@
+#include "conv_kernel.hpp"
+namespace rc {
+int conv_f16_k3_idwt(int ck, int nt, const ConvArgs& a, hipStream_t s) {
+    if (ck == 48 && nt == 3) return launch_conv_idwt<ConvCfg<f16_t, 48, 3, 3>>(a, s);
+    if (ck == 32 && nt == 4) return launch_conv_idwt<ConvCfg<f16_t, 32, 4, 3>>(a, s);
+    return fail(RC_ERR_UNSUPPORTED, "conv: no RC_OUT_NHWC_IDWT kernel instantiation for this (chunk width, cout tile width)");
+}
+}
diff --git a/realcamnet_amd/csrc/conv_kernel.hpp b/realcamnet_amd/csrc/conv_kernel.hpp
--- a/realcamnet_amd/csrc/conv_kernel.hpp
+++ b/realcamnet_amd/csrc/conv_kernel.hpp
@@ -98,6 +98,7 @@
 
 typedef unsigned int u32x4_t __attribute__((ext_vector_type(4)));
 typedef unsigned int u32x2_t __attribute__((ext_vector_type(2)));
+typedef unsigned int u32x3_t __attribute__((ext_vector_type(3)));
 
 __device__ __forceinline__ __amdgpu_buffer_rsrc_t make_rsrc(const void* p, unsigned bytes) {
     return __builtin_amdgcn_make_buffer_rsrc(const_cast<void*>(p), 0, (int)bytes, 0x00020000);
@@ -926,6 +927,97 @@
 #pragma unroll
         for (int i = 0; i < NV / 2; ++i)
             __builtin_amdgcn_raw_buffer_store_b128(u32x4_t{o[4 * i], o[4 * i + 1], o[4 * i + 2], o[4 * i + 3]}, r_out, oo, 16 * i, 0);
+    }
+
+    __device__ static __forceinline__ void swap_rows16(unsigned& x, unsigned& y) {
+        asm volatile("s_nop 1\n\tv_permlane16_swap_b32 %0, %1\n\ts_nop 1" : "+v"(x), "+v"(y));
+    }
+    template <bool PRE>
+    __device__ static __forceinline__ void epilogue_idwt(const ConvArgs& a, int b, int y0, int x0, int ct, int tid, f32x4 (&acc)[4][NT],
+                                                         const unsigned (&rp)[PRE ? 4 : 1][PRE ? NV / 2 : 1], bool has_res) {
+        static_assert(ES == 2 && (NT == 3 || NT == 4), "16-bit storage; 48- or 64-wide cout tiles");
+        const int lane = tid & 63, wave = tid >> 6, q = lane >> 4, n = lane & 15;
+        const int jbase = ct * Cfg::COUT_TILE + q * NV;
+        const size_t img = (size_t)a.H * a.W * a.cout;
+        const unsigned img_bytes = (unsigned)(img * ES);
+        const __amdgpu_buffer_rsrc_t r_out = make_rsrc(static_cast<T*>(a.out) + (size_t)b * img, img_bytes);
+        const __amdgpu_buffer_rsrc_t r_res = make_rsrc(has_res ? static_cast<const T*>(a.residual) + (size_t)b * img : nullptr, has_res ? img_bytes : 0u);
+        const int gy = y0 + 2 * wave, gx = x0 + n;
+        const int row_b = a.W * a.cout * ES, col_b = 16 * a.cout * ES;
+        const int off0 = ((gy * a.W + gx) * a.cout + jbase) * ES;
+        const int cq = a.cout >> 2;
+        const int o_row = 2 * a.W * cq * ES;
+        const int o_off0 = ((4 * gy * a.W + 2 * gx + (q & 1)) * cq + NT * (4 * ct + (q & 2))) * ES;
+#pragma unroll
+        for (int pt = 0; pt < 4; ++pt) {
+            const int dy = pt >> 1, dx = pt & 1;
+            const bool valid = gy + dy < a.H && gx + 16 * dx < a.W;
+            float v[NV];
+#pragma unroll
+            for (int i = 0; i < NT; ++i)
+#pragma unroll
+                for (int k = 0; k < 4; ++k) {
+                    if constexpr (NT == 4) v[4 * i + k] = acc[pt][k][i];
+                    else v[4 * i + k] = acc[pt][i][k];
+                }
+            if (has_res) {
+                unsigned rw[NV / 2];
+                if constexpr (PRE) {
+#pragma unroll
+                    for (int i = 0; i < NV / 2; ++i) rw[i] = rp[pt][i];
+                } else {
+                    const int po = valid ? off0 + dy * row_b + dx * col_b : kOOB;
+#pragma unroll
+                    for (int i = 0; i < NV / 8; ++i) {
+                        const u32x4_t t = __builtin_amdgcn_raw_buffer_load_b128(r_res, po + 16 * i, 0, 0);
+                        rw[4 * i] = t.x; rw[4 * i + 1] = t.y; rw[4 * i + 2] = t.z; rw[4 * i + 3] = t.w;
+                    }
+                    if constexpr (NV % 8 != 0) {
+                        const u32x2_t t = __builtin_amdgcn_raw_buffer_load_b64(r_res, po + 16 * (NV / 8), 0, 0);
+                        rw[4 * (NV / 8)] = t.x; rw[4 * (NV / 8) + 1] = t.y;
+                    }
+                }
+#pragma unroll
+                for (int i = 0; i < NV / 2; ++i) {
+                    v[2 * i] += lo16<T>(rw[i]);
+                    v[2 * i + 1] += hi16<T>(rw[i]);
+                }
+            }
+            float h[NV];
+#pragma unroll
+            for (int i = 0; i < NV / 2; ++i) {
+                const unsigned w = pack16x2<T>(v[2 * i], v[2 * i + 1]);
+                h[2 * i] = lo16<T>(w) * 0.5f;
+                h[2 * i + 1] = hi16<T>(w) * 0.5f;
+            }
+            unsigned wd[4][2];
+            float o[4][4];
+#pragma unroll
+            for (int i = 0; i < NT; ++i) {
+                const float sab = h[4 * i] + h[4 * i + 1], dab = h[4 * i] - h[4 * i + 1];
+                o[0][i] = (sab + h[4 * i + 2]) + h[4 * i + 3];
+                o[1][i] = (sab - h[4 * i + 2]) - h[4 * i + 3];
+                o[2][i] = (dab + h[4 * i + 2]) - h[4 * i + 3];
+                o[3][i] = (dab - h[4 * i + 2]) + h[4 * i + 3];
+            }
+#pragma unroll
+            for (int t = 0; t < 4; ++t) {
+                wd[t][0] = pack16x2<T>(o[t][0], o[t][1]);
+                if constexpr (NT == 4) wd[t][1] = pack16x2<T>(o[t][2], o[t][3]);
+                else wd[t][1] = pack16x2<T>(o[t][2], 0.f);
+            }
+            const int oo = (valid && !(a.dbg_flags & 1)) ? o_off0 + dy * 2 * o_row + dx * 32 * cq * ES : kOOB;
+#pragma unroll
+            for (int r = 0; r < 2; ++r) {
+                unsigned x0w = wd[2 * r][0], x1w = wd[2 * r][1], y0w = wd[2 * r + 1][0], y1w = wd[2 * r + 1][1];
+                swap_rows16(x0w, y0w);
+                swap_rows16(x1w, y1w);
+                if constexpr (NT == 4)
+                    __builtin_amdgcn_raw_buffer_store_b128(u32x4_t{x0w, x1w, y0w, y1w}, r_out, oo, r * o_row, 0);
+                else
+                    __builtin_amdgcn_raw_buffer_store_b96(u32x3_t{x0w, (x1w & 0xffffu) | (y0w << 16), (y0w >> 16) | (y1w << 16)}, r_out, oo, r * o_row, 0);
+            }
+        }
     }
 
     __device__ static __forceinline__ void epilogue_generic(const ConvArgs& a, int b, int y0, int x0, int sp, int ct, int tid,
@@ -1152,7 +1244,7 @@
 template <class Cfg>
 constexpr int persist_blocks_per_cu() { return Cfg::NT <= 2 && persist_lds_bytes_c<Cfg>() * 3 <= 160 * 1024 ? 3 : 2; }
 
-template <class Cfg, bool GATED, bool FAST>
+template <class Cfg, bool GATED, bool FAST, bool IDWT = false>
 __global__ __launch_bounds__(kThreads, persist_blocks_per_cu<Cfg>()) void conv_mfma_persist_kernel(const ConvArgs a) {
     using D = ConvDev<Cfg>;
     constexpr int NT = Cfg::NT, STEPS = Cfg::STEPS, NV = 4 * NT;
@@ -1253,13 +1345,16 @@
             [[maybe_unused]] unsigned rpre[RESPRE ? 4 : 1][RESPRE ? D::NRH : 1];
             bool res_pre = false;
             if constexpr (RESPRE) {
-                if ((a.ep_key == D::EP_RES || a.ep_key == (D::EP_GATE | D::EP_RES)) && a.out_mode == RC_OUT_NHWC) {
+                if (IDWT ? a.ep_key == D::EP_RES : ((a.ep_key == D::EP_RES || a.ep_key == (D::EP_GATE | D::EP_RES)) && a.out_mode == RC_OUT_NHWC)) {
                     res_pre = true;
                     D::res_prefetch(a, cb, cy0, cx0, ct, tid, rpre);
                 }
             }
             D::template mma_steps<0, STEPS, 0, (!GATED && NT < 5)>(s_in, a.w_resident ? s_w + ct * (int)Cfg::CHUNK_W_BYTES : s_w, lane_x, lane_w, q, lo, acc);
-            if constexpr (FAST && sizeof(typename Cfg::elem) == 2) {
+            if constexpr (IDWT) {
+                static_assert(RESPRE, "the IDWT form of kernel 2: 16-bit, fast epilogue, <= 3 cout tiles of 16");
+                D::template epilogue_idwt<true>(a, cb, cy0, cx0, ct, tid, acc, rpre, res_pre);
+            } else if constexpr (FAST && sizeof(typename Cfg::elem) == 2) {
                 const int rslot = a.sums_compact ? 4 * D::compact_residue(pos, cb, sp_total, (int)gridDim.x) : -1;
                 if (RUN_SUMS && a.ep_key == D::EP_SUMS && n_ct == 1)
                     D::template epilogue_fast_impl<D::EP_SUMS, RUN_SUMS>(a, cb, cy0, cx0, csp, ct, tid, acc, run, tile < 0 || b != cb, rslot);
@@ -1554,7 +1649,7 @@
 constexpr bool wst_eligible() { return wst_form<Cfg>() != 0; }
 constexpr int waitcnt_vm(int n) { return (n & 15) | ((n >> 4) << 14) | 0x0F70; }
 
-template <class Cfg8, bool FAST>
+template <class Cfg8, bool FAST, bool IDWT = false>
 __global__ __launch_bounds__(kWsmThreads) void conv_mfma_wst_kernel(const ConvArgs a) {
 #if defined(__HIP_DEVICE_COMPILE__)
     using Cfg = WstCfg<Cfg8>;
@@ -1588,7 +1683,7 @@
     const int my_units = pos < n_units ? (n_units - pos + stride - 1) / stride : 0;
     const int my_stages = my_units * cts_per_unit * n_chunks;
 
-    for (int i = tid; i < a.cout_packed; i += kWsmThreads) s_bias[i] = a.bias ? a.bias[i] : 0.f;
+    for (int i = tid; i < a.cout_packed; i += kWsmThreads) s_bias[i] = a.bias ? a.bias[IDWT ? ((i & ~0x3c) | ((i & 0x0c) << 2) | ((i & 0x30) >> 2)) : i] : 0.f;
 
     auto decode = [&](int unit, int& b, int& ty, int& tx, int& ct0) {
         int tile = unit;
@@ -1757,8 +1852,13 @@
                 } else {
                     run_chunks(std::integral_constant<int, 3>{}, 0, n_chunks);
                 }
-                if (ty8 < a.tiles_y)
-                    D8::template epilogue<FAST>(a, b, ty8 * kTH, tx * kTW, ty8 * a.tiles_x + tx, ct, tid & 255, acc);
+                if (ty8 < a.tiles_y) {
+                    if constexpr (IDWT) {
+                        static_assert(NT == 4 && FAST, "the IDWT form of kernel 4b: 64-wide cout tiles");
+                        const unsigned none[1][1] = {{0u}};
+                        D8::template epilogue_idwt<false>(a, b, ty8 * kTH, tx * kTW, ct, tid & 255, acc, none, a.residual != nullptr);
+                    } else D8::template epilogue<FAST>(a, b, ty8 * kTH, tx * kTW, ty8 * a.tiles_x + tx, ct, tid & 255, acc);
+                }
                 __syncthreads();
             }
             kb3 = kb3 == NBUF - 1 ? 0 : kb3 + 1;
@@ -1766,6 +1866,7 @@
     }
 #endif
 }
+
 
 template <class Cfg>
 constexpr int pss_lds_bytes() { return (int)Cfg::CHUNK_W_BYTES + kPersistMaxCout * 4 + WsmCfg<Cfg>::IN_BYTES + kWsmTH * kTW * Cfg::COUT_TILE * 2; }
@@ -2310,6 +2411,26 @@
 template <class Cfg, bool FAST>
 int launch_wst(const ConvArgs& a, int grid, hipStream_t stream) {
     return launch_lds<&conv_mfma_wst_kernel<Cfg, FAST>>(dim3((unsigned)grid), dim3(kWsmThreads), wst_lds_bytes<Cfg>(), stream, a);
+}
+
+template <class Cfg>
+int launch_conv_idwt(const ConvArgs& a, hipStream_t stream) {
+    using DD = ConvDev<Cfg>;
+    static_assert(sizeof(typename Cfg::elem) == 2 && Cfg::KS == 3 && ((Cfg::CK == 48 && Cfg::NT == 3) || (Cfg::CK == 32 && Cfg::NT == 4)), "the IDWT forms");
+    const int n_tiles = a.tiles_x * a.tiles_y * a.batch;
+    if (!((a.ep_key == 0 || a.ep_key == DD::EP_RES) && a.cin_vec_ok && a.cin_chunk_ok && a.cout_packed == a.cout && a.cout_packed <= kPersistMaxCout && n_tiles < (1 << 24)))
+        return fail(RC_ERR_UNSUPPORTED, "rc_conv2d: RC_OUT_NHWC_IDWT needs 16-byte aligned operands, cin a whole number of chunks, cout <= 512 and fewer than 2^24 tiles");
+    if constexpr (Cfg::NT == 3) {
+        constexpr int P_LDS = persist_lds_bytes_c<Cfg>();
+        static_assert(P_LDS <= 80 * 1024, "two persistent blocks per CU");
+        if (a.n_chunks != 1) return fail(RC_ERR_UNSUPPORTED, "rc_conv2d: RC_OUT_NHWC_IDWT on 48-wide cout tiles is a one-chunk form (cin == 48)");
+        const int grid = persistent_grid(persist_blocks_per_cu<Cfg>() * a.num_cus, n_tiles);
+        return launch_lds<&conv_mfma_persist_kernel<Cfg, false, true, true>>(dim3((unsigned)grid), dim3(kThreads), P_LDS, stream, a);
+    } else {
+        static_assert(wst_form<Cfg>() == 2, "kernel 4b, two tile buffers");
+        const int n_items = a.tiles_x * ((a.H + kWsmTH - 1) / kWsmTH) * a.batch * (a.n_chunks > 1 ? a.n_ct : 1);
+        return launch_lds<&conv_mfma_wst_kernel<Cfg, true, true>>(dim3((unsigned)persistent_grid(a.num_cus, n_items)), dim3(kWsmThreads), wst_lds_bytes<Cfg>(), stream, a);
+    }
 }
 
 template <class Cfg, bool GATED, bool FAST>
diff --git a/realcamnet_amd/networks.py b/realcamnet_amd/networks.py
--- a/realcamnet_amd/networks.py
+++ b/realcamnet_amd/networks.py
@@ -53,9 +53,9 @@
             return (ops.to_nchw(y[0]), *y[1:])
         return ops.to_nchw(self._nhwc(ops.to_nhwc(x)))
 
-    def _nhwc(self, a, residual=None):
+    def _nhwc(self, a, residual=None, idwt=None, skip_first=False):
         mods = list(self)
-        i, n = 0, len(mods)
+        i, n = (1 if skip_first else 0), len(mods)
         while i < n:
             m = mods[i]
             if isinstance(m, Conv2d):
@@ -79,6 +79,9 @@
                     j += 1
                 if j == n and residual is not None and kw.get("out_mode", RC_OUT_NHWC) == RC_OUT_NHWC and not shuffle_after:
                     kw["residual"], residual = residual, None
+                if (j == n and idwt is not None and residual is None and "out_mode" not in kw and "act" not in kw and not shuffle_after and
+                        ops.conv_idwt_ok(a, m, idwt, kw.get("residual"))):
+                    kw["out_mode"], idwt = ops.RC_OUT_NHWC_IDWT, None
                 a = m._nhwc(a, **kw)
                 if shuffle_after:
                     a = ops.pixel_shuffle2(a)
@@ -97,7 +100,7 @@
             i += 1
         if residual is not None:
             raise NotImplementedError("trailing residual could not be fused (sequence does not end in a conv)")
-        return a
+        return a if idwt is None else idwt._nhwc(a)
 
 
 def seq(*args):
diff --git a/realcamnet_amd/ops.py b/realcamnet_amd/ops.py
--- a/realcamnet_amd/ops.py
+++ b/realcamnet_amd/ops.py
@@ -12,7 +12,7 @@
 from . import _lib
 from . import torch_ops as _T
 from ._lib import (RC_ACT_GELU, RC_ACT_LEAKY, RC_ACT_NONE, RC_ACT_RELU, RC_ACT_RELU_POST, RC_BF16, RC_F16, RC_F32, RC_OUT_NCHW, RC_OUT_NHWC, RC_OUT_NHWC_DWT,
-                   RC_OUT_PIXEL_SHUFFLE2, RC_OUT_PIXEL_SHUFFLE2_NCHW, ConvDesc, ConvPairDesc, check)
+                   RC_OUT_NHWC_IDWT, RC_OUT_PIXEL_SHUFFLE2, RC_OUT_PIXEL_SHUFFLE2_NCHW, ConvDesc, ConvPairDesc, check)
 
 _DT = {torch.float32: RC_F32, torch.bfloat16: RC_BF16, torch.float16: RC_F16}
 _HALF = (torch.bfloat16, torch.float16)
@@ -722,6 +722,33 @@
     return derived(dwt, "haar_ok", (w,), taps_are_haar)
 
 
+FUSE_IDWT = os.environ.get("RC_FUSE_IDWT", "1") != "0"
+
+
+def conv_idwt_ok(x: torch.Tensor, conv, idwt, residual: Optional[torch.Tensor] = None) -> bool:
+    if not FUSE_IDWT or x.dtype not in _HALF or x.dim() != 4 or conv.weight.dim() != 4:
+        return False
+    cout, cin, kh, kw = conv.weight.shape
+    if not (kh == kw == 3 and x.shape[3] == cin and cout % 4 == 0):
+        return False
+    if tuple(conv.stride) != (1, 1) or tuple(conv.padding) != (1, 1) or tuple(conv.dilation) != (1, 1) or conv.groups != 1:
+        return False
+    if residual is not None and (tuple(residual.shape) != (*x.shape[:3], cout) or residual.dtype != x.dtype):
+        return False
+    w = getattr(idwt, "weight", None)
+    if w is None or tuple(w.shape) != (cout, 1, 2, 2):
+        return False
+    if not _lib.load().rc_conv_idwt_ok(_DT[x.dtype], cin, cout, 3):
+        return False
+    if isinstance(w, FakeTensor):
+        return True
+
+    def taps_are_haar():
+        want = torch.tensor(_HAAR_TAPS, dtype=torch.float32).reshape(4, 1, 2, 2).repeat(cout // 4, 1, 1, 1)
+        return bool(torch.equal(w.detach().float().cpu(), want))
+    return derived(idwt, "haar_ok", (w,), taps_are_haar)
+
+
 FUSE_SHUFFLE_STORE = True
 
 FOLD_TAIL = True
diff --git a/realcamnet_amd/torch_ops.py b/realcamnet_amd/torch_ops.py
--- a/realcamnet_amd/torch_ops.py
+++ b/realcamnet_amd/torch_ops.py
@@ -8,7 +8,7 @@
 from torch import Tensor
 
 from . import _lib
-from ._lib import RC_BF16, RC_F16, RC_F32, RC_OUT_NCHW, RC_OUT_NHWC, RC_OUT_NHWC_DWT, RC_OUT_PIXEL_SHUFFLE2, RC_OUT_PIXEL_SHUFFLE2_NCHW, ConvDesc, ConvPairDesc, check
+from ._lib import RC_BF16, RC_F16, RC_F32, RC_OUT_NCHW, RC_OUT_NHWC, RC_OUT_NHWC_DWT, RC_OUT_NHWC_IDWT, RC_OUT_PIXEL_SHUFFLE2, RC_OUT_PIXEL_SHUFFLE2_NCHW, ConvDesc, ConvPairDesc, check
 
 _DT = {torch.float32: RC_F32, torch.bfloat16: RC_BF16, torch.float16: RC_F16}
 _LIB = torch.library.Library("realcam", "DEF")
@@ -254,7 +254,7 @@
     b, H, W, _ = x.shape
     if out_mode == RC_OUT_NHWC:
         out = x.new_empty((b, H, W, cout))
-    elif out_mode == RC_OUT_PIXEL_SHUFFLE2:
+    elif out_mode in (RC_OUT_PIXEL_SHUFFLE2, RC_OUT_NHWC_IDWT):
         out = x.new_empty((b, 2 * H, 2 * W, cout // 4))
     elif out_mode == RC_OUT_NHWC_DWT:
         out = x.new_empty((b, H // 2, W // 2, 4 * cout))
```

Result: no change. 1334 MP/s (median of 6 runs) (+0.8%).
